# VictoriaMetrics/VictoriaLogs

Measured on NVIDIA H100. Metric: log rows scanned/sec (LogsQL phrase+regex), higher is better.
Workload: dtype u8

## Files before the change

### victorialogs_b200/csrc/vl_engine.cu

```cuda
#include <dlfcn.h>
#include <algorithm>
#include <atomic>
#include <chrono>
#include <thread>
#include <cstdio>
#include <cstdlib>
#include <cstring>
#include <functional>
#include <map>
#include <memory>
#include <mutex>
#include "vl_copier.h"
#include "vl_engine.h"
#include "vl_program.h"
#include "vl_part.h"
#include "vl_mathnum.cuh"

using namespace vl;

namespace vl {
static thread_local std::string g_thread_err;
void set_thread_error(const std::string& s) { g_thread_err = s; }
}

struct vlscan_program {
    Program p;
    struct Image { DevBuf leaves, prepass, regexes, blob, u64s, u32s; DevProgram view; };
    std::map<int, std::unique_ptr<Image>> images;
    std::mutex mu;
    const DevProgram& image(int device, cudaStream_t st) {
        std::lock_guard<std::mutex> g(mu);
        auto it = images.find(device);
        if (it != images.end()) return it->second->view;
        auto im = std::make_unique<Image>();
        auto up = [&](DevBuf& b, const void* src, size_t n) { b.ensure(std::max<size_t>(n, 16)); if (n) VL_CUDA(cudaMemcpyAsync(b.p, src, n, cudaMemcpyHostToDevice, st)); };
        up(im->leaves, p.leaves.data(), p.leaves.size() * sizeof(DevLeaf));
        up(im->prepass, p.prepass.data(), p.prepass.size() * sizeof(DevPrepass));
        up(im->regexes, p.regexes.data(), p.regexes.size() * sizeof(DevRegex));
        up(im->blob, p.blob.data(), p.blob.size());
        up(im->u64s, p.u64s.data(), p.u64s.size() * 8);
        up(im->u32s, p.u32s.data(), p.u32s.size() * 4);
        VL_CUDA(cudaStreamSynchronize(st));
        im->view = DevProgram{im->leaves.as<DevLeaf>(), im->prepass.as<DevPrepass>(), im->regexes.as<DevRegex>(), im->blob.as<uint8_t>(), im->u64s.as<uint64_t>(), im->u32s.as<uint32_t>()};
        auto& ref = *im;
        images[device] = std::move(im);
        return ref.view;
    }
    ~vlscan_program() { for (auto& kv : images) { cudaSetDevice(kv.first); kv.second->leaves.release(); kv.second->prepass.release(); kv.second->regexes.release(); kv.second->blob.release(); kv.second->u64s.release(); kv.second->u32s.release(); } }
};

struct vlscan_host_blocks {
    void* pinned = nullptr; size_t bytes = 0;
    std::vector<vlscan_block> blocks;
    std::vector<vlscan_column> cols;
    std::vector<std::string> fields;
    std::vector<std::vector<uint32_t>> dict_offsets;
    std::vector<std::unique_ptr<std::vector<uint8_t>>> owned;
    std::vector<uint64_t> source;
};
struct vlscan_part { vl::part::PartReader r; };

void* vlscan_ctx::ensure_pinned(size_t n) {
    if (n <= pinned_cap) return pinned;
    if (pinned) cudaFreeHost(pinned);
    pinned = nullptr; pinned_cap = 0;
    VL_CUDA(cudaMallocHost(&pinned, n));
    pinned_cap = n;
    return pinned;
}

namespace {

template <class F> int guarded(vlscan_ctx* ctx, F&& f) {
    try { f(); return 0; }
    catch (const CudaFail& e) { set_thread_error(e.msg); if (ctx) ctx->err = e.msg; return e.code > 0 ? e.code : 1; }
    catch (const BadInput& e) { set_thread_error(e.msg); if (ctx) ctx->err = e.msg; return -1; }
    catch (const ProgError& e) { set_thread_error(e.what()); if (ctx) ctx->err = e.what(); return -2; }
    catch (const std::exception& e) { set_thread_error(e.what()); if (ctx) ctx->err = e.what(); return -3; }
}

struct ZstdWriter {
    size_t (*compress)(void*, size_t, const void*, size_t, int) = nullptr;
    size_t (*bound)(size_t) = nullptr;
    unsigned (*is_error)(size_t) = nullptr;
    bool ok = false;
    ZstdWriter() {
        void* h = dlopen("libzstd.so.1", RTLD_NOW | RTLD_GLOBAL);
        if (!h) return;
        compress = (decltype(compress))dlsym(h, "ZSTD_compress");
        bound = (decltype(bound))dlsym(h, "ZSTD_compressBound");
        is_error = (decltype(is_error))dlsym(h, "ZSTD_isError");
        ok = compress && bound && is_error;
    }
};
ZstdWriter& zstd_writer() { static ZstdWriter z; return z; }

void launch_check(vlscan_ctx* ctx) { ctx->launches++; VL_CUDA(cudaGetLastError()); }
inline unsigned cdiv(uint64_t a, uint64_t b) { return (unsigned)((a + b - 1) / b); }

struct Carve {
    size_t off = 0;
    std::vector<std::function<void(uint8_t*)>> set;
    template <class T> Carve& take(T*& p, uint64_t n) { const size_t o = off; off += (n * sizeof(T) + 15) & ~(size_t)15; set.push_back([&p, o](uint8_t* base) { p = (T*)(base + o); }); return *this; }
    size_t place(DevBuf& buf) { buf.ensure(std::max<size_t>(off, 16)); for (auto& f : set) f(buf.as<uint8_t>()); return off; }
};

}

namespace vl {
void finish_batch_layout(vlscan_ctx* ctx, vlscan_batch* b, const std::vector<uint32_t>& rows) {
    b->nblocks = rows.size();
    b->h_rows = rows;
    b->h_word_off.assign(rows.size() + 1, 0);
    b->rows = 0;
    for (size_t i = 0; i < rows.size(); i++) { b->h_word_off[i + 1] = b->h_word_off[i] + (rows[i] + 63) / 64; b->rows += rows[i]; }
    b->nwords = b->h_word_off.back();
    std::vector<uint32_t> wb(b->nwords);
    std::vector<uint64_t> init(b->nwords);
    for (size_t i = 0; i < rows.size(); i++) {
        for (uint64_t w = b->h_word_off[i]; w < b->h_word_off[i + 1]; w++) { wb[w] = (uint32_t)i; init[w] = ~0ull; }
        uint32_t tail = rows[i] & 63;
        if (tail) init[b->h_word_off[i + 1] - 1] = (~0ull) >> (64 - tail);
    }
    b->blk_rows.ensure(std::max<size_t>(rows.size() * 4, 16));
    b->blk_word_off.ensure((rows.size() + 1) * 8);
    b->word_block.ensure(std::max<size_t>(b->nwords * 4, 16));
    b->init_bitmap.ensure(std::max<size_t>(b->nwords * 8, 16));
    if (!rows.empty()) VL_CUDA(cudaMemcpyAsync(b->blk_rows.p, rows.data(), rows.size() * 4, cudaMemcpyHostToDevice, ctx->stream));
    VL_CUDA(cudaMemcpyAsync(b->blk_word_off.p, b->h_word_off.data(), (rows.size() + 1) * 8, cudaMemcpyHostToDevice, ctx->stream));
    if (b->nwords) {
        VL_CUDA(cudaMemcpyAsync(b->word_block.p, wb.data(), b->nwords * 4, cudaMemcpyHostToDevice, ctx->stream));
        VL_CUDA(cudaMemcpyAsync(b->init_bitmap.p, init.data(), b->nwords * 8, cudaMemcpyHostToDevice, ctx->stream));
    }
    VL_CUDA(cudaStreamSynchronize(ctx->stream));
}
}

static uint64_t collect_values_blocks(const vlscan_block* blocks, uint64_t nblocks, std::vector<ZValuesBlock>& zv, const uint8_t* need = nullptr, uint32_t nfields = 0, std::vector<size_t>* at = nullptr) {
    uint64_t zc = 512;
    if (at) at->assign((size_t)nblocks * nfields, SIZE_MAX);
    for (uint64_t b = 0; b < nblocks; b++)
        for (uint32_t k = 0; k < blocks[b].ncols; k++) {
            const vlscan_column& c = blocks[b].cols[k];
            if (c.kind != VLSCAN_COL_VALUES || c.stage != VLSCAN_STAGE_ONDISK) continue;
            if (need && (c.field >= nfields || !need[b * nfields + c.field])) continue;
            if (at && c.field < nfields && (*at)[b * nfields + c.field] == SIZE_MAX) (*at)[b * nfields + c.field] = zv.size();
            zv.push_back({c.values, (size_t)c.values_len, zc});
            zc += c.values_len;
        }
    return zc;
}
static double now_s() { return std::chrono::duration<double>(std::chrono::steady_clock::now().time_since_epoch()).count(); }

namespace {
struct Upload {
    vlscan_ctx* ctx; vlscan_batch* out; const vlscan_block* blocks; uint64_t nblocks; uint32_t nfields; vlscan_stats* stats;
    const std::vector<char>* need_bloom;
    std::vector<DevColumn>& cols = out->h_cols;
    const bool dbg = getenv("VLSCAN_DEBUG_TIMING") != nullptr; const double t_start = now_s();
    Copier io{ctx};
    std::vector<uint32_t> rows = std::vector<uint32_t>(nblocks);
    std::vector<Piece> pieces;
    std::vector<std::unique_ptr<std::vector<uint8_t>>> owned;
    uint64_t cursor = 16;
    ZstdJob zjob;
    uint64_t regen_cursor = 0;
    struct Ondisk { uint64_t col; uint32_t lens_frame, data_frame; uint64_t lens_rel, data_rel; };
    std::vector<Ondisk> ondisk;
    std::vector<OndiskCol> ocols;
    struct TsFrame { uint64_t block; uint32_t frame; uint64_t rel; };
    std::vector<TsFrame> ts_frames;
    std::vector<DevTimestamps> tsv;
    std::vector<ZValuesBlock> zv; std::vector<ZValuesInfo> zinfo; std::vector<size_t> zv_of; std::vector<uint64_t> ts_zoff; size_t zbad = SIZE_MAX; std::string zmsg;
    uint64_t add_piece(const uint8_t* src, uint64_t len) { uint64_t off = arena_reserve(cursor, len); if (len) pieces.push_back({src, len, off}); return off; }
    template <class F> void walk(bool ts, F&& f) {
        for (uint64_t b = 0; b < nblocks; b++) {
            const vlscan_block& blk = blocks[b];
            if (blk.rows > (8u << 20)) throw BadInput("block rows exceed maxRowsPerBlock (8Mi)");
            rows[b] = (uint32_t)blk.rows;
            if (ts) timestamps(blk, b);
            for (uint32_t k = 0; k < blk.ncols; k++) {
                if (blk.cols[k].field >= nfields) throw BadInput("column refers to a field outside the batch field table");
                f(blk, blk.cols[k], (size_t)b * nfields + blk.cols[k].field);
            }
        }
    }
    void sources(const uint8_t* need, bool ts) {
        uint64_t zc = collect_values_blocks(blocks, nblocks, zv, need, nfields, &zv_of);
        for (const ZValuesBlock& v : zv) if (v.n) io.src.push_back({v.p, v.n, v.zoff});
        ts_zoff.resize(ts ? nblocks : 0);
        for (uint64_t b = 0; b < nblocks && ts; b++) {
            const vlscan_block& blk = blocks[b];
            if (blk.ts_marshal_type != MT_ZSTD_NEAREST_DELTA2 && blk.ts_marshal_type != MT_ZSTD_NEAREST_DELTA) continue;
            if (blk.timestamps_len > vl::part::kMaxTimestampsBlockSize) throw BadInput("timestamps block size cannot exceed 8 MiB");
            ts_zoff[b] = zc;
            if (blk.timestamps_len) io.src.push_back({blk.timestamps, blk.timestamps_len, zc});
            zc += blk.timestamps_len;
        }
        if (!io.src.empty()) { ctx->zsrc.ensure(zc + 512); io.send_sources(ctx->zsrc.as<uint8_t>()); }
        zinfo.resize(zv.size());
        const double t_w = now_s();
        if (!zv.empty()) zjob.add_values_blocks(zv.data(), zv.size(), host_threads(), zinfo.data(), &zbad, &zmsg);
        if (dbg) fprintf(stderr, "[vlscan upload] header walk of %zu values blocks on %d host threads: %.1f ms (after %.1f ms of collecting and enqueueing the copies)\n",
                         zv.size(), host_threads(), 1e3 * (now_s() - t_w), 1e3 * (t_w - t_start));
    }
    template <class F> void header(const vlscan_column& c, size_t i, F&& payload) {
        DevColumn& d = cols[i];
        if (d.kind != COL_MISSING) throw BadInput("duplicate column for one field in a block");
        if (c.kind == VLSCAN_COL_CONST) {
            d.kind = COL_CONST; d.meta_len = (uint32_t)c.const_len; d.meta_off = add_piece(c.const_value, c.const_len);
            return;
        }
        if (c.kind != VLSCAN_COL_VALUES) throw BadInput("unknown column kind");
        if (c.value_type < VT_STRING || c.value_type >= VT_MAX) throw BadInput("unknown valueType");
        d.kind = COL_VALUES; d.vt = c.value_type; d.min_value = c.min_value; d.max_value = c.max_value;
        payload();
        if (c.bloom_len % 8) throw BadInput("cannot unmarshal bloomFilter from src with size not multiple by 8");
        if (need_bloom && !(*need_bloom)[c.field]) { d.bloom_words = 0; d.bloom_off = add_piece(c.bloom, 0); }
        else { d.bloom_words = (uint32_t)(c.bloom_len / 8); d.bloom_off = add_piece(c.bloom, c.bloom_len); }
        if (c.value_type == VT_DICT) {
            if (c.dict_len > 8) throw BadInput("valuesDict may contain max 8 items");
            d.dict_len = c.dict_len;
            uint32_t total = c.dict_len ? c.dict_offsets[c.dict_len] : 0;
            d.meta_len = total;
            if (c.dict_len && c.dict_blob == (const uint8_t*)c.dict_offsets + 4 * (c.dict_len + 1)) {
                d.meta_off = add_piece((const uint8_t*)c.dict_offsets, 4 * (c.dict_len + 1) + total);
            } else {
                auto meta = std::make_unique<std::vector<uint8_t>>();
                meta->resize(4 * (c.dict_len + 1) + total);
                if (c.dict_len) memcpy(meta->data(), c.dict_offsets, 4 * (c.dict_len + 1)); else memset(meta->data(), 0, 4);
                if (total) memcpy(meta->data() + 4 * (c.dict_len + 1), c.dict_blob, total);
                d.meta_off = add_piece(meta->data(), meta->size());
                owned.push_back(std::move(meta));
            }
        }
    }
    void values(const vlscan_block& blk, const vlscan_column& c, size_t ci) {
        DevColumn& d = cols[ci];
        if (c.stage == VLSCAN_STAGE_ONDISK) {
            const size_t z = zv_of[ci];
            if (z >= zbad) throw BadInput(zmsg);
            const uint64_t lens_len = zinfo[z].lens_len, data_len = zinfo[z].data_len;
            if (data_len > 0xFFFFFFFFull) throw BadInput("values block too large");
            const uint64_t lr = arena_reserve(regen_cursor, lens_len + 15), dr = arena_reserve(regen_cursor, data_len);
            d.lens_off = lr + 16; d.data_off = dr; d.data_len = data_len;
            ondisk.push_back({ci, (uint32_t)(2 * z), (uint32_t)(2 * z + 1), lr + 15, dr});
            ocols.push_back({ci, lens_len, blk.rows});
        } else if (c.stage == VLSCAN_STAGE_DECODED) {
            const uint8_t* lens_items = c.lens_items; const uint64_t lens_len = c.lens_items_len, data_len = c.data_len;
            if (lens_len < 1) throw BadInput("cannot unmarshal uint64 block type from empty src");
            uint8_t lt = lens_items[0];
            if (lt > 7) throw BadInput("unexpected uint64 block type");
            uint64_t want = lt < 4 ? (blk.rows << lt) : (1ull << (lt - 4));
            if (lens_len - 1 != want) throw BadInput("unexpected block length for uint items");
            d.lens_type = lt;
            if (lt >= 4) { uint64_t v = 0; for (uint64_t i = 0; i < want; i++) v = (v << 8) | lens_items[1 + i]; if (v > 0xFFFFFFFFull) throw BadInput("row length does not fit 32 bits"); d.lens_const = (uint32_t)v; }
            if (data_len > 0xFFFFFFFFull) throw BadInput("values block too large");
            d.lens_off = add_piece(lens_items + 1, lens_len - 1);
            d.data_off = add_piece(c.data, data_len); d.data_len = data_len;
            d.data_const = (blk.rows >= 2 && lt >= 4 && data_len == d.lens_const) ? 1 : 0;
        } else throw BadInput("unknown values stage");
    }
    void timestamps(const vlscan_block& blk, uint64_t b) {
        if (!blk.ts_marshal_type) return;
        if (blk.ts_marshal_type > MT_NEAREST_DELTA) throw BadInput("unknown MarshalType of a timestamps block");
        if (blk.timestamps_len > vl::part::kMaxTimestampsBlockSize) throw BadInput("timestamps block size cannot exceed 8 MiB");
        if (tsv.empty()) { tsv.resize(nblocks); memset(tsv.data(), 0, nblocks * sizeof(DevTimestamps)); }
        DevTimestamps& t = tsv[b];
        t.first = blk.min_timestamp; t.max = blk.max_timestamp;
        if (blk.ts_marshal_type == MT_ZSTD_NEAREST_DELTA2 || blk.ts_marshal_type == MT_ZSTD_NEAREST_DELTA) {
            uint64_t regen = 0; uint32_t id = 0;
            zjob.add_frame(blk.timestamps, blk.timestamps_len, ts_zoff[b], &regen, &id);
            if (regen > 10ull * blk.rows + 16) throw BadInput("cannot unmarshal timestamps: the decompressed block is larger than its varints can be");
            t.mt = blk.ts_marshal_type == MT_ZSTD_NEAREST_DELTA2 ? MT_NEAREST_DELTA2 : MT_NEAREST_DELTA;
            t.len = (uint32_t)regen;
            ts_frames.push_back({b, id, arena_reserve(regen_cursor, regen)});
        } else {
            t.mt = (uint8_t)blk.ts_marshal_type; t.len = (uint32_t)blk.timestamps_len;
            t.off = add_piece(blk.timestamps, blk.timestamps_len);
        }
    }

    uint64_t commit(DevBuf& region, const std::vector<uint64_t>* patch, bool layout) {
        const uint64_t regen_base = (cursor + kArenaAlign - 1) / kArenaAlign * kArenaAlign;
        for (const Ondisk& o : ondisk) {
            DevColumn& d = cols[o.col];
            d.lens_off += regen_base; d.data_off += regen_base;
            zjob.set_dst(o.lens_frame, regen_base + o.lens_rel); zjob.set_dst(o.data_frame, regen_base + o.data_rel);
        }
        for (const TsFrame& tf : ts_frames) { tsv[tf.block].off = regen_base + tf.rel; zjob.set_dst(tf.frame, regen_base + tf.rel); }
        const bool have_z = !ondisk.empty() || !ts_frames.empty();
        if (have_z) cursor = regen_base + regen_cursor;
        const uint64_t bytes = cursor + kArenaPad;
        const double t_desc = now_s();
        region.ensure(bytes);
        const double t_alloc = now_s();
        uint8_t* cols_base = region.as<uint8_t>();
        std::vector<ColPatch> patches;
        if (patch) {
            const uint64_t delta = (uint64_t)(uintptr_t)region.p - (uint64_t)(uintptr_t)out->arena.p;
            cols_base = out->arena.as<uint8_t>();
            patches.resize(patch->size());
            for (size_t i = 0; i < patch->size(); i++) {
                DevColumn& d = cols[(*patch)[i]];
                d.lens_off += delta; d.data_off += delta;
                patches[i].col = (*patch)[i]; patches[i].c = d;
            }
        }
        cudaStream_t cs = ctx->copy_stream;
        cudaEvent_t ev_cleared = io.events.make(), ev_copied = io.events.make();
        VL_CUDA(cudaMemsetAsync(region.p, 0, bytes, ctx->stream));
        VL_CUDA(cudaEventRecord(ev_cleared, ctx->stream));
        VL_CUDA(cudaStreamWaitEvent(cs, ev_cleared, 0));
        const double t_h2d = dbg ? now_s() : 0;
        double t_zrun = 0;
        if (have_z) {
            zjob.set_group_hook([&](uint64_t src_end) { io.wait_sources(ctx->stream, src_end); });
            zjob.run(ctx, ctx->zsrc.as<uint8_t>(), region.as<uint8_t>());
            io.ship_sources(UINT64_MAX);
            if (dbg) t_zrun = now_s();
        }
        io.copy(pieces, region.as<uint8_t>());
        DevBuf& table = patch ? ctx->patch : out->cols;
        const void* entries = patch ? (const void*)patches.data() : (const void*)cols.data();
        const size_t table_bytes = patch ? patches.size() * sizeof(ColPatch) : cols.size() * sizeof(DevColumn);
        table.ensure(std::max<size_t>(table_bytes, 16));
        if (table_bytes) VL_CUDA(cudaMemcpyAsync(table.p, entries, table_bytes, cudaMemcpyHostToDevice, cs));
        io.h2d += table_bytes;
        if (!patch) out->has_ts = !tsv.empty();
        if (!tsv.empty()) {
            out->ts.ensure(nblocks * sizeof(DevTimestamps));
            VL_CUDA(cudaMemcpyAsync(out->ts.p, tsv.data(), nblocks * sizeof(DevTimestamps), cudaMemcpyHostToDevice, cs));
            io.h2d += nblocks * sizeof(DevTimestamps);
        }
        VL_CUDA(cudaEventRecord(ev_copied, cs));
        if (!patches.empty()) {
            VL_CUDA(cudaStreamWaitEvent(ctx->stream, ev_copied, 0));
            k_patch_cols<<<cdiv(patches.size(), 128), 128, 0, ctx->stream>>>(out->cols.as<DevColumn>(), ctx->patch.as<ColPatch>(), (uint32_t)patches.size());
            launch_check(ctx);
        }
        const double t_enq = dbg ? now_s() : 0;
        if (have_z) {
            VL_CUDA(cudaStreamWaitEvent(ctx->stream, ev_copied, 0));
            ctx->zcols.ensure(16 + ocols.size() * sizeof(OndiskCol));
            VL_CUDA(cudaMemsetAsync(ctx->zcols.p, 0, 16, ctx->stream));
            VL_CUDA(cudaMemcpyAsync(ctx->zcols.as<uint8_t>() + 16, ocols.data(), ocols.size() * sizeof(OndiskCol), cudaMemcpyHostToDevice, ctx->stream));
            if (!ocols.empty()) {
                k_finish_ondisk_cols<<<cdiv(ocols.size(), 128), 128, 0, ctx->stream>>>(cols_base, out->cols.as<DevColumn>(), (const OndiskCol*)(ctx->zcols.as<uint8_t>() + 16),
                                                                                         (uint32_t)ocols.size(), ctx->zcols.as<unsigned long long>());
                launch_check(ctx);
            }
            io.h2d += ocols.size() * sizeof(OndiskCol);
            zjob.check(ctx);
            unsigned long long cst[2] = {0, 0};
            VL_CUDA(cudaMemcpy(cst, ctx->zcols.p, 16, cudaMemcpyDeviceToHost));
            static const char* what[] = {"", "cannot unmarshal uint64 block type from empty src", "unexpected uint64 block type", "unexpected block length for uint items", "row length does not fit 32 bits"};
            if (cst[0]) throw BadInput(what[std::min<unsigned long long>(cst[0], 4)]);
        }
        VL_CUDA(cudaStreamWaitEvent(ctx->stream, ev_copied, 0));
        double t_copy = 0;
        if (dbg) { VL_CUDA(cudaStreamSynchronize(ctx->stream)); t_copy = now_s(); }
        if (nfields) out->note_columns(cols);
        if (layout) finish_batch_layout(ctx, out, rows);
        else VL_CUDA(cudaStreamSynchronize(ctx->stream));
        if (dbg) fprintf(stderr, "[vlscan upload] blocks=%llu arena=%.1f MB h2d=%.1f MB pieces=%zu+%zu pinned=%d: describe %.1f ms, alloc %.1f ms, copy %.1f ms (%.1f GB/s), "
                                 "zstd %llu frames / %llu blocks / %llu sequences: enqueue %.1f ms, decode %.1f ms; layout %.1f ms\n", (unsigned long long)nblocks,
                         bytes / 1e6, io.h2d / 1e6, pieces.size(), io.src.size(), (int)io.all_pinned, 1e3 * (t_desc - t_start), 1e3 * (t_alloc - t_desc), 1e3 * (t_enq - (t_zrun > 0 ? t_zrun : t_h2d)), io.h2d / 1e9 / std::max(t_copy - t_start, 1e-9),
                         (unsigned long long)zjob.frames(), (unsigned long long)zjob.compressed_blocks(), (unsigned long long)zjob.sequences(), 1e3 * (t_zrun > 0 ? t_zrun - t_h2d : 0), 1e3 * (t_copy - t_enq), 1e3 * (now_s() - t_copy));
        if (layout) io.h2d += out->nwords * 12 + nblocks * 12;
        if (stats) stats->h2d_bytes += io.h2d;
        return bytes;
    }
};
}

enum UploadMode { UP_FULL = 0, UP_HEADERS = 1, UP_VALUES = 2, UP_LATE = 3 };
static void do_upload(vlscan_ctx* ctx, const char* const* field_names, const size_t* field_name_lens, uint32_t nfields, const vlscan_block* blocks,
                      uint64_t nblocks, vlscan_batch* out, vlscan_stats* stats, const std::vector<char>* need_bloom = nullptr, UploadMode mode = UP_FULL,
                      const uint8_t* need = nullptr, uint64_t* zframes = nullptr) {
    VL_CUDA(cudaSetDevice(ctx->device));
    if (nblocks > 0xFFFFFFF0ull) throw BadInput("too many blocks in one batch");
    out->device = ctx->device; out->nfields = nfields;
    Upload u{ctx, out, blocks, nblocks, nfields, stats, need_bloom};
    if (mode == UP_FULL || mode == UP_HEADERS) {
        for (uint32_t f = 0; f < nfields; f++) out->field_names.emplace_back(field_names[f], field_name_lens[f]);
        u.cols.assign((size_t)nblocks * std::max<uint32_t>(nfields, 1), DevColumn{});
        memset(u.cols.data(), 0, u.cols.size() * sizeof(DevColumn));
        out->late_used = 0; out->split_hdr = mode == UP_HEADERS;
    } else if (u.cols.size() != (size_t)nblocks * std::max<uint32_t>(nfields, 1) || !need) throw BadInput("internal: values phase of a bloom-first upload without its header phase");
    try {
        switch (mode) {
        case UP_FULL:
            u.sources(nullptr, true);
            u.walk(true, [&](const vlscan_block& blk, const vlscan_column& c, size_t i) { u.header(c, i, [&] { u.values(blk, c, i); }); });
            out->arena_bytes = u.commit(out->arena, nullptr, true);
            out->harena_bytes = 0;
            std::vector<DevColumn>().swap(out->h_cols);
            break;
        case UP_HEADERS:
            u.walk(false, [&](const vlscan_block&, const vlscan_column& c, size_t i) {
                u.header(c, i, [&] {
                    if (c.stage != VLSCAN_STAGE_ONDISK && c.stage != VLSCAN_STAGE_DECODED) throw BadInput("unknown values stage");
                    u.cols[i].values_state = VALUES_DEFERRED;
                });
            });
            out->harena_bytes = u.commit(out->harena, nullptr, true);
            break;
        case UP_VALUES:
            u.sources(need, true);
            u.walk(true, [&](const vlscan_block& blk, const vlscan_column& c, size_t i) {
                if (c.kind != VLSCAN_COL_VALUES) return;
                u.cols[i].values_state = need[i] ? VALUES_STAGED : VALUES_ABSENT;
                if (need[i]) u.values(blk, c, i);
            });
            out->arena_bytes = u.commit(out->arena, nullptr, false);
            break;
        case UP_LATE: {
            std::vector<uint64_t> staged;
            u.sources(need, false);
            u.walk(false, [&](const vlscan_block& blk, const vlscan_column& c, size_t i) {
                if (c.kind != VLSCAN_COL_VALUES || !need[i]) return;
                if (u.cols[i].values_state == VALUES_STAGED) throw BadInput("duplicate column for one field in a block");
                u.cols[i].values_state = VALUES_STAGED;
                u.values(blk, c, i);
                staged.push_back(i);
            });
            if (out->late_used == out->late.size()) out->late.emplace_back();
            u.commit(out->late[out->late_used], &staged, false);
            out->late_used++;
            *zframes += u.zjob.frames();
            break;
        }
        }
    } catch (...) {
        cudaStreamSynchronize(ctx->copy_stream); cudaStreamSynchronize(ctx->stream);
        throw;
    }
}

namespace {
struct ScanRun {
    vlscan_ctx* ctx; const vlscan_program* prog; const vlscan_batch* batch;
    DevProgram P; BatchView B; std::vector<int> field_slot;
    unsigned long long* stats;
    size_t regs_used = 0;

    uint64_t* new_reg() {
        if (regs_used == ctx->regs.size()) ctx->regs.emplace_back();
        DevBuf& r = ctx->regs[regs_used++];
        r.ensure(std::max<size_t>(B.nwords * 8, 16));
        return r.as<uint64_t>();
    }
    void free_reg() { regs_used--; }
    void copy_reg(uint64_t* dst, const uint64_t* src) { if (B.nwords) VL_CUDA(cudaMemcpyAsync(dst, src, B.nwords * 8, cudaMemcpyDeviceToDevice, ctx->stream)); }
    void andnot(uint64_t* a, const uint64_t* b) { if (!B.nwords) return; k_andnot<<<cdiv(B.nwords, 256), 256, 0, ctx->stream>>>(a, b, B.nwords); launch_check(ctx); }
    void prepass(const PNode& nd, uint64_t* reg) {
        if (nd.prepass_count == 0) return;
        std::vector<int> slots(nd.prepass_count);
        for (int e = 0; e < nd.prepass_count; e++) slots[e] = field_slot[prog->p.prepass[nd.prepass_begin + e].field];
        size_t off = slots_cursor; slots_cursor += slots.size();
        ctx->slots.ensure(std::max<size_t>(slots_total * 4, 16));
        VL_CUDA(cudaMemcpyAsync(ctx->slots.as<int>() + off, slots.data(), slots.size() * 4, cudaMemcpyHostToDevice, ctx->stream));
        k_prepass<<<cdiv((uint64_t)B.nblocks * 32, 128), 128, 0, ctx->stream>>>(P, B, (uint32_t)nd.prepass_begin, (uint32_t)nd.prepass_count, ctx->slots.as<int>() + off,
                                                                             nd.kind == F_OR, reg, stats);
        launch_check(ctx);
    }
    size_t slots_cursor = 0, slots_total = 0;

    void leaf(int leaf_idx, uint64_t* reg) {
        const DevLeaf& L = prog->p.leaves[leaf_idx];
        if (L.kind == F_NOOP) return;
        int slot = L.field >= 0 ? field_slot[L.field] : -1;
        uint8_t* action = ctx->action.as<uint8_t>(); uint64_t* payload = ctx->payload.as<uint64_t>(); uint64_t* leaf_bm = ctx->leaf_bm.as<uint64_t>();
        uint32_t* lens_blocks = ctx->lens_blocks.as<uint32_t>(); uint32_t* row_blocks = ctx->row_blocks.as<uint32_t>(); uint32_t* wc = ctx->work_count.as<uint32_t>();
        ScanTile* tiles = ctx->tiles.as<ScanTile>();
        VL_CUDA(cudaMemsetAsync(wc, 0, WC_COUNT * 4, ctx->stream));
        if (L.kind == F_EQ_FIELD || L.kind == F_LE_FIELD) {
            const int slot_b = field_slot[L.field2];
            uint32_t* lens_b = ctx->lens_blocks2.as<uint32_t>();
            k_plan_pair<<<cdiv((uint64_t)B.nblocks * 32, 256), 256, 0, ctx->stream>>>(P, B, (uint32_t)leaf_idx, slot, slot_b, reg, action, payload, lens_blocks, lens_b, row_blocks, wc, stats);
            launch_check(ctx);
            if (B.nwords) {
                const int persistent = ctx->sm_count * 8;
                const uint32_t *ro_a = nullptr, *ro_b = nullptr;
                for (int side = 0; side < 2; side++) {
                    const int sl = side ? slot_b : slot;
                    if (sl < 0) continue;
                    uint8_t* ready = ctx->ready[sl].as<uint8_t>();
                    if (!ctx->ready_cleared[sl]) { VL_CUDA(cudaMemsetAsync(ready, 0, B.nblocks, ctx->stream)); ctx->ready_cleared[sl] = 1; }
                    k_lens_offsets<<<persistent, 256, 0, ctx->stream>>>(B, sl, side ? lens_b : lens_blocks, wc, ctx->row_off8[sl].as<uint32_t>(), ready, stats, side ? WC_LENS2 : WC_LENS); launch_check(ctx);
                    (side ? ro_b : ro_a) = ctx->row_off8[sl].as<uint32_t>();
                }
                k_row_pair<<<persistent, 256, 0, ctx->stream>>>(P, B, (uint32_t)leaf_idx, slot, slot_b, row_blocks, wc, payload, reg, ro_a, ro_b, leaf_bm, stats); launch_check(ctx);
                k_apply_leaf<<<cdiv(B.nwords, 256), 256, 0, ctx->stream>>>(B, action, leaf_bm, reg); launch_check(ctx);
            }
            return;
        }
        k_plan_leaf<<<cdiv(B.nblocks, VL_PLAN_WARPS), VL_PLAN_WARPS * 32, 0, ctx->stream>>>(P, B, (uint32_t)leaf_idx, slot, reg, action, payload, lens_blocks, row_blocks, tiles, wc, stats);
        launch_check(ctx);
        if (slot >= 0 && B.nwords) {
            uint32_t* ro = ctx->row_off8[slot].as<uint32_t>(); uint8_t* ready = ctx->ready[slot].as<uint8_t>();
            if (!ctx->ready_cleared[slot]) { VL_CUDA(cudaMemsetAsync(ready, 0, B.nblocks, ctx->stream)); ctx->ready_cleared[slot] = 1; }
            const int persistent = ctx->sm_count * 8;
            const uint32_t vts = batch->slot_vt_mask.empty() ? ~0u : batch->slot_vt_mask[slot];
            const bool has_string = vts >> VT_STRING & 1, has_dict = vts >> VT_DICT & 1;
            const bool has_numeric = (vts & ~((1u << VT_STRING) | (1u << VT_DICT))) != 0;
            const bool may_scan = L.str_strategy == STR_SCAN && has_string;
            const bool may_row = (has_string && L.str_strategy != STR_ALL) || has_numeric;
            if (may_scan || may_row) { k_lens_offsets<<<persistent, 256, 0, ctx->stream>>>(B, slot, lens_blocks, wc, ro, ready, stats); launch_check(ctx); }
            if (may_scan) {
                VL_CUDA(cudaMemsetAsync(leaf_bm, 0, B.nwords * 8, ctx->stream));
                ScanParams sp; memset(&sp, 0, sizeof sp);
                sp.mode = L.scan_mode; sp.needle_off = L.scan_needle_off; sp.needle_len = L.scan_needle_len; sp.starts_tok = L.starts_tok; sp.ends_tok = L.ends_tok; sp.regex = L.regex;
                const bool masked = fill_scan_patterns(prog->p.blob.data() + L.scan_needle_off, L.scan_needle_len, sp.pat, sp.msk, sp.delta, sp.nd16);
                if (L.scan_mode == SCAN_CONTAINS || L.scan_mode >= SCAN_RX_DOTPLUS) { sp.starts_tok = sp.ends_tok = 0; }
                auto& evp = next_scan_events();
                VL_CUDA(cudaEventRecord(evp.first, ctx->stream));
                if (masked) k_substr_scan<true><<<ctx->sm_count * ctx->scan_occ[1], VL_SCAN_THREADS, 0, ctx->stream>>>(P, B, slot, sp, tiles, wc, ro, leaf_bm);
                else k_substr_scan<false><<<ctx->sm_count * ctx->scan_occ[0], VL_SCAN_THREADS, 0, ctx->stream>>>(P, B, slot, sp, tiles, wc, ro, leaf_bm);
                launch_check(ctx);
                VL_CUDA(cudaEventRecord(evp.second, ctx->stream));
            }
            if (may_row) { k_row_match<<<ctx->sm_count * ctx->row_occ, 256, 0, ctx->stream>>>(P, B, (uint32_t)leaf_idx, slot, row_blocks, wc, action, payload, reg, ro, leaf_bm); launch_check(ctx); }
            if (has_dict || has_numeric) { k_word_match<<<cdiv(B.nwords, 128), 128, 0, ctx->stream>>>(P, B, (uint32_t)leaf_idx, slot, action, payload, reg, leaf_bm, stats); launch_check(ctx); }
        }
        if (L.kind == F_TIME && B.nwords) {
            ctx->ts_vals.ensure(B.nwords * 64 * 8);
            k_time_match<<<ctx->sm_count * 4, 256, 0, ctx->stream>>>(B, (long long)L.aux0, (long long)L.aux1, row_blocks, wc, ctx->ts_vals.as<unsigned long long>(), leaf_bm, stats);
            launch_check(ctx);
        }
        if (B.nwords) { k_apply_leaf<<<cdiv(B.nwords, 256), 256, 0, ctx->stream>>>(B, action, leaf_bm, reg); launch_check(ctx); }
    }
    std::pair<cudaEvent_t, cudaEvent_t>& next_scan_events() {
        if (ctx->scan_events_used == ctx->scan_events.size()) { cudaEvent_t a, b; VL_CUDA(cudaEventCreate(&a)); VL_CUDA(cudaEventCreate(&b)); ctx->scan_events.emplace_back(a, b); }
        return ctx->scan_events[ctx->scan_events_used++];
    }
    void probe_leaf(int leaf_idx, const uint64_t* reg, uint8_t* need) {
        const DevLeaf& L = prog->p.leaves[leaf_idx];
        if (L.kind == F_NOOP || L.kind == F_TIME) return;
        const int slot = L.field >= 0 ? field_slot[L.field] : -1;
        if (L.kind == F_EQ_FIELD || L.kind == F_LE_FIELD) {
            k_plan_pair<<<cdiv((uint64_t)B.nblocks * 32, 256), 256, 0, ctx->stream>>>(P, B, (uint32_t)leaf_idx, slot, field_slot[L.field2], reg, nullptr, nullptr, nullptr, nullptr, nullptr, nullptr, stats, need);
        } else {
            if (slot < 0) return;
            k_plan_leaf<<<cdiv(B.nblocks, VL_PLAN_WARPS), VL_PLAN_WARPS * 32, 0, ctx->stream>>>(P, B, (uint32_t)leaf_idx, slot, reg, nullptr, nullptr, nullptr, nullptr, nullptr, nullptr, stats, need);
        }
        launch_check(ctx);
    }
    void probe_node(int id, uint64_t* reg, uint8_t* need) {
        const PNode& nd = prog->p.nodes[id];
        switch (nd.kind) {
        case F_NOOP: break;
        case F_AND: case F_OR: {
            uint64_t* r = reg;
            if (nd.prepass_count) { r = new_reg(); copy_reg(r, reg); prepass(nd, r); }
            for (int k : nd.kids) probe_node(k, r, need);
            if (nd.prepass_count) free_reg();
            break;
        }
        case F_NOT: probe_node(nd.kids[0], reg, need); break;
        default: probe_leaf(nd.leaf, reg, need);
        }
    }
    void node(int id, uint64_t* reg) {
        const PNode& nd = prog->p.nodes[id];
        switch (nd.kind) {
        case F_NOOP: break;
        case F_AND: prepass(nd, reg); for (int k : nd.kids) node(k, reg); break;
        case F_OR: {
            prepass(nd, reg);
            uint64_t* res = new_reg(); uint64_t* tmp = new_reg();
            copy_reg(res, reg);
            for (int k : nd.kids) { copy_reg(tmp, res); node(k, tmp); andnot(res, tmp); }
            andnot(reg, res);
            free_reg(); free_reg();
            break;
        }
        case F_NOT: { uint64_t* tmp = new_reg(); copy_reg(tmp, reg); node(nd.kids[0], tmp); andnot(reg, tmp); free_reg(); break; }
        default: leaf(nd.leaf, reg);
        }
    }
};
}

static void read_stats(vlscan_ctx* ctx, vlscan_stats* st, bool check_error) {
    unsigned long long h[ST_COUNT];
    VL_CUDA(cudaMemcpyAsync(h, ctx->stats.p, sizeof h, cudaMemcpyDeviceToHost, ctx->stream));
    VL_CUDA(cudaStreamSynchronize(ctx->stream));
    if (check_error && h[ST_ERROR]) {
        static const char* const msg[] = {"", "cannot unmarshal strings: row lengths do not add up to the data length", "too big index for dict value",
                                          "unexpected length for binary representation of a number", "", "", "the filter needs the timestamps of a block that was handed over without them", "cannot unmarshal timestamps",
                                          "internal: a filter reached the values of a column that the bloom-first probe pass had left on the host"};
        throw BadInput(msg[std::min<unsigned long long>(h[ST_ERROR], 8)]);
    }
    if (!st) return;
    st->values_bytes += h[ST_VALUES_BYTES]; st->bloom_probe_bytes += h[ST_BLOOM_BYTES]; st->columns_read += h[ST_COLUMNS_READ];
    st->bitmap_bytes += h[ST_BITMAP_BYTES]; st->rows_matched += h[ST_ROWS_MATCHED]; st->blocks_matched += h[ST_BLOCKS_MATCHED];
    st->scan_kernel_bytes += h[ST_SCAN_BYTES];
    float ms = 0;
    VL_CUDA(cudaEventElapsedTime(&ms, ctx->ev_begin, ctx->ev_end)); st->gpu_ms += ms;
    for (size_t i = 0; i < ctx->scan_events_used; i++) { VL_CUDA(cudaEventElapsedTime(&ms, ctx->scan_events[i].first, ctx->scan_events[i].second)); st->scan_kernel_ms += ms; }
}

static void do_scan(vlscan_ctx* ctx, const vlscan_program* prog, const vlscan_batch* batch, vlscan_stats* stats) {
    VL_CUDA(cudaSetDevice(ctx->device));
    if (batch->device != ctx->device) throw BadInput("batch lives on another device than the ctx");
    ScanRun run{ctx, prog, batch};
    run.P = const_cast<vlscan_program*>(prog)->image(ctx->device, ctx->stream);
    run.B = batch->view();
    const Program& pr = prog->p;
    run.field_slot.assign(pr.fields.size(), -1);
    for (size_t f = 0; f < pr.fields.size(); f++) for (uint32_t s = 0; s < batch->nfields; s++) if (batch->field_names[s] == pr.fields[f]) run.field_slot[f] = (int)s;
    for (auto& nd : pr.nodes) run.slots_total += nd.prepass_count;
    uint64_t nb = std::max<uint64_t>(batch->nblocks, 1), nw = std::max<uint64_t>(batch->nwords, 1);
    ctx->action.ensure(nb); ctx->payload.ensure(nb * 8); ctx->leaf_bm.ensure(nw * 8);
    ctx->lens_blocks.ensure(nb * 4); ctx->lens_blocks2.ensure(nb * 4); ctx->row_blocks.ensure(nb * 4); ctx->work_count.ensure(WC_COUNT * 4);
    {
        uint64_t max_tiles = batch->arena_bytes / VL_TILE_BYTES + nb + 16;
        ctx->tiles.ensure(max_tiles * sizeof(ScanTile));
    }
    ctx->stats.ensure(ST_COUNT * 8); ctx->totals.ensure(32); ctx->counts.ensure(nb * 4);
    if (ctx->row_off8.size() < batch->nfields) { ctx->row_off8.resize(batch->nfields); ctx->ready.resize(batch->nfields); }
    ctx->ready_cleared.assign(batch->nfields, 0);
    for (uint32_t s = 0; s < batch->nfields; s++) { ctx->row_off8[s].ensure(nw * 32); ctx->ready[s].ensure(nb); }
    uint64_t launches0 = ctx->launches;
    ctx->scan_events_used = 0;
    run.stats = ctx->stats.as<unsigned long long>();
    VL_CUDA(cudaEventRecord(ctx->ev_begin, ctx->stream));
    VL_CUDA(cudaMemsetAsync(ctx->stats.p, 0, ST_COUNT * 8, ctx->stream));
    VL_CUDA(cudaMemsetAsync(ctx->totals.p, 0, 32, ctx->stream));
    uint64_t* reg = run.new_reg();
    run.copy_reg(reg, batch->init_bitmap.as<uint64_t>());
    if (batch->nblocks) {
        run.node(pr.root, reg);
        k_finalize<<<cdiv(batch->nblocks, 8), 256, 0, ctx->stream>>>(run.B, reg, ctx->counts.as<uint32_t>(), run.stats, ctx->totals.as<unsigned long long>());
        launch_check(ctx);
    }
    VL_CUDA(cudaEventRecord(ctx->ev_end, ctx->stream));
    ctx->last_batch = batch; ctx->has_result = true; ctx->kept = false; ctx->last_launches = ctx->launches - launches0;
    ctx->last_nblocks = batch->nblocks; ctx->last_nwords = batch->nwords; ctx->last_rows = batch->rows;
    if (stats) {
        read_stats(ctx, stats, true);
        stats->blocks += batch->nblocks; stats->rows += batch->rows; stats->gpu_launches += ctx->launches - launches0;
    }
}

static void do_probe(vlscan_ctx* ctx, const vlscan_program* prog, const vlscan_batch* batch, std::vector<uint8_t>& need) {
    VL_CUDA(cudaSetDevice(ctx->device));
    ScanRun run{ctx, prog, batch};
    run.P = const_cast<vlscan_program*>(prog)->image(ctx->device, ctx->stream);
    run.B = batch->view();
    const Program& pr = prog->p;
    run.field_slot.assign(pr.fields.size(), -1);
    for (size_t f = 0; f < pr.fields.size(); f++) for (uint32_t s = 0; s < batch->nfields; s++) if (batch->field_names[s] == pr.fields[f]) run.field_slot[f] = (int)s;
    for (auto& nd : pr.nodes) run.slots_total += nd.prepass_count;
    const size_t cells = (size_t)batch->nblocks * batch->nfields;
    need.assign(cells, 0);
    if (!cells || !batch->nwords) return;
    ctx->need.ensure(std::max<size_t>(cells, 16)); ctx->stats.ensure(ST_COUNT * 8);
    VL_CUDA(cudaMemsetAsync(ctx->need.p, 0, cells, ctx->stream));
    VL_CUDA(cudaMemsetAsync(ctx->stats.p, 0, ST_COUNT * 8, ctx->stream));
    run.stats = ctx->stats.as<unsigned long long>();
    uint64_t* reg = run.new_reg();
    run.copy_reg(reg, batch->init_bitmap.as<uint64_t>());
    run.probe_node(pr.root, reg, ctx->need.as<uint8_t>());
    VL_CUDA(cudaMemcpyAsync(need.data(), ctx->need.p, cells, cudaMemcpyDeviceToHost, ctx->stream));
    VL_CUDA(cudaStreamSynchronize(ctx->stream));
}

extern "C" {

int vlscan_device_count(void) {
    int n = 0;
    if (cudaGetDeviceCount(&n) != cudaSuccess) { cudaGetLastError(); return 0; }
    return n;
}

vlscan_ctx* vlscan_ctx_create(int device) {
    vlscan_ctx* ctx = new vlscan_ctx();
    int rc = guarded(nullptr, [&] {
        int n = vlscan_device_count();
        if (n <= 0) throw CudaFail("no CUDA device is available: libvlscan has no CPU fallback", 100);
        ctx->device = ((device % n) + n) % n;
        VL_CUDA(cudaSetDevice(ctx->device));
        VL_CUDA(cudaStreamCreateWithFlags(&ctx->stream, cudaStreamNonBlocking));
        VL_CUDA(cudaStreamCreateWithFlags(&ctx->copy_stream, cudaStreamNonBlocking));
        VL_CUDA(cudaEventCreate(&ctx->ev_begin)); VL_CUDA(cudaEventCreate(&ctx->ev_end));
        cudaDeviceProp prop; VL_CUDA(cudaGetDeviceProperties(&prop, ctx->device)); ctx->sm_count = prop.multiProcessorCount;
        VL_CUDA(cudaOccupancyMaxActiveBlocksPerMultiprocessor(&ctx->scan_occ[0], k_substr_scan<false>, VL_SCAN_THREADS, 0));
        VL_CUDA(cudaOccupancyMaxActiveBlocksPerMultiprocessor(&ctx->scan_occ[1], k_substr_scan<true>, VL_SCAN_THREADS, 0));
        for (int& o : ctx->scan_occ) o = std::max(o, 1);
        VL_CUDA(cudaOccupancyMaxActiveBlocksPerMultiprocessor(&ctx->row_occ, k_row_match, 256, 0));
        ctx->row_occ = std::max(ctx->row_occ, 1);
    });
    if (rc) { delete ctx; return nullptr; }
    return ctx;
}
void vlscan_ctx_free(vlscan_ctx* ctx) {
    if (!ctx) return;
    cudaSetDevice(ctx->device);
    if (ctx->copy_stream) cudaStreamSynchronize(ctx->copy_stream);
    if (ctx->stream) cudaStreamSynchronize(ctx->stream);
    for (DevBuf* b : {&ctx->action, &ctx->payload, &ctx->leaf_bm, &ctx->lens_blocks, &ctx->row_blocks, &ctx->work_count, &ctx->stats, &ctx->totals, &ctx->counts, &ctx->slots, &ctx->hit_offs, &ctx->hits, &ctx->tiles, &ctx->lens_blocks2}) b->release();
    for (auto& r : ctx->regs) r.release();
    for (auto& r : ctx->row_off8) r.release();
    for (auto& r : ctx->ready) r.release();
    ctx->zsrc.release(); ctx->zcols.release(); ctx->ztest.release(); ctx->ts_vals.release();
    for (DevBuf* b : {&ctx->hit_block, &ctx->glens, &ctx->goffs, &ctx->gtiles, &ctx->gout, &ctx->gstat, &ctx->hblk, &ctx->htab, &ctx->hgrp, &ctx->lcand, &ctx->ftab, &ctx->patch, &ctx->unstaged}) b->release();
    for (DevBuf& b : ctx->ftxt) b.release();
    zstd_dev_free(ctx->zdev);
    delete ctx->pool;
    if (ctx->pinned) cudaFreeHost(ctx->pinned);
    delete ctx->recycle;
    for (auto& e : ctx->scan_events) { cudaEventDestroy(e.first); cudaEventDestroy(e.second); }
    if (ctx->ev_begin) cudaEventDestroy(ctx->ev_begin);
    if (ctx->ev_end) cudaEventDestroy(ctx->ev_end);
    if (ctx->copy_stream) cudaStreamDestroy(ctx->copy_stream);
    if (ctx->stream) cudaStreamDestroy(ctx->stream);
    delete ctx;
}
const char* vlscan_last_error(const vlscan_ctx* ctx) { return ctx ? ctx->err.c_str() : g_thread_err.c_str(); }
void* vlscan_ctx_stream(const vlscan_ctx* ctx) { return (void*)ctx->stream; }
int vlscan_ctx_sync(vlscan_ctx* ctx) { return guarded(ctx, [&] { VL_CUDA(cudaSetDevice(ctx->device)); VL_CUDA(cudaStreamSynchronize(ctx->stream)); }); }

int vlscan_program_create(const void* tree, size_t tree_len, vlscan_program** out) {
    *out = nullptr;
    auto* pg = new vlscan_program();
    int rc = guarded(nullptr, [&] { ProgramBuilder(tree, tree_len, pg->p).build(); });
    if (rc) { delete pg; return rc; }
    *out = pg;
    return 0;
}
void vlscan_program_free(vlscan_program* prog) { delete prog; }
uint32_t vlscan_program_nfields(const vlscan_program* prog) { return (uint32_t)prog->p.fields.size(); }
const char* vlscan_program_field(const vlscan_program* prog, uint32_t i, size_t* len) { if (i >= prog->p.fields.size()) { *len = 0; return nullptr; } *len = prog->p.fields[i].size(); return prog->p.fields[i].data(); }
int64_t vlscan_program_leaf_tokens(const vlscan_program* prog, uint32_t leaf, char* buf, size_t cap) {
    if (leaf >= prog->p.leaf_tokens.size()) return -1;
    std::string s; for (size_t i = 0; i < prog->p.leaf_tokens[leaf].size(); i++) { if (i) s.push_back('\n'); s += prog->p.leaf_tokens[leaf][i]; }
    if (s.size() > cap) return -1;
    memcpy(buf, s.data(), s.size());
    return (int64_t)s.size();
}

int vlscan_eval_predicate(int kind, const void* value, size_t value_len, const void* arg1, size_t arg1_len, const void* arg2, size_t arg2_len, uint64_t aux0, uint64_t aux1) {
    if (value_len > 0xFFFFFFFFull || arg1_len > 0xFFFFFFFFull || arg2_len > 0xFFFFFFFFull) return -1;
    const uint8_t* v = (const uint8_t*)value; const uint32_t vn = (uint32_t)value_len;
    const uint8_t* a = (const uint8_t*)arg1; const uint32_t an = (uint32_t)arg1_len;
    switch (kind) {
    case F_REGEXP: {
        try { return vl::compile_regex(std::string((const char*)a, an)).match(v, vn) ? 1 : 0; } catch (const vl::RxError& e) { vl::set_thread_error(e.what()); return -2; }
    }
    case 14: return vl::any_case_match(v, vn, a, an, false) ? 1 : 0;
    case 15: return vl::any_case_match(v, vn, a, an, true) ? 1 : 0;
    case 16: return vl::match_sequence(v, vn, vl::PhraseList{a, an}) ? 1 : 0;
    case 17: return vl::match_all_phrases(v, vn, vl::PhraseList{a, an}) ? 1 : 0;
    case 18: return vl::match_any_phrase(v, vn, vl::PhraseList{a, an}) ? 1 : 0;
    }
    if (kind < F_EXACT_PREFIX || kind > F_IPV4_RANGE) return -1;
    return vl::range_predicate(kind, (const uint8_t*)value, (uint32_t)value_len, (const uint8_t*)arg1, (uint32_t)arg1_len, (const uint8_t*)arg2, (uint32_t)arg2_len, aux0, aux1) ? 1 : 0;
}

int64_t vlscan_program_prepass_tokens(const vlscan_program* prog, char* buf, size_t cap) {
    const Program& P = prog->p;
    std::string s;
    for (const PNode& nd : P.nodes) {
        if (nd.kind != F_AND && nd.kind != F_OR) continue;
        s += nd.kind == F_AND ? "A" : "O";
        for (int k = 0; k < nd.prepass_count; k++) {
            const DevPrepass& pp = P.prepass[(size_t)nd.prepass_begin + k];
            s += "\t" + P.fields[pp.field];
            const uint32_t* offs = (const uint32_t*)(P.blob.data() + pp.tok_offs_off);
            for (uint32_t t = 0; t < pp.ntokens; t++) { s += "\x1f"; s.append((const char*)P.blob.data() + pp.tok_blob_off + offs[t], offs[t + 1] - offs[t]); }
        }
        s += "\n";
    }
    if (s.size() > cap) return -1;
    memcpy(buf, s.data(), s.size());
    return (int64_t)s.size();
}

int64_t vlscan_program_in_hashes(const vlscan_program* prog, uint32_t leaf, uint64_t* out, size_t cap) {
    const Program& P = prog->p;
    if (leaf >= P.leaves.size() || P.leaves[leaf].kind != F_IN) return -1;
    const DevLeaf& L = P.leaves[leaf];
    std::vector<uint64_t> v;
    v.push_back(L.nhashes); v.insert(v.end(), P.u64s.begin() + L.hashes_off, P.u64s.begin() + L.hashes_off + L.nhashes);
    if (L.in_skip_sets) v.push_back(UINT64_MAX);
    else {
        v.push_back(L.in_nsets);
        for (uint32_t k = 0; k < L.in_nsets; k++) {
            const uint32_t off = P.u32s[L.in_sets_off + 2 * k], n = P.u32s[L.in_sets_off + 2 * k + 1];
            v.push_back(n); v.insert(v.end(), P.u64s.begin() + off, P.u64s.begin() + off + n);
        }
    }
    if (v.size() > cap) return -1;
    memcpy(out, v.data(), v.size() * 8);
    return (int64_t)v.size();
}

int64_t vlscan_program_in_typed(const vlscan_program* prog, uint32_t leaf, int value_type, uint64_t* out, size_t cap) {
    const Program& P = prog->p;
    if (leaf >= P.leaves.size() || P.leaves[leaf].kind != F_IN || value_type < VT_UINT8 || value_type >= VT_MAX) return -1;
    const DevLeaf& L = P.leaves[leaf];
    const uint32_t n = L.in_typed_cnt[value_type];
    if (n > cap) return -1;
    if (n) memcpy(out, P.u64s.data() + L.in_typed_off[value_type], (size_t)n * 8);
    return (int64_t)n;
}

int vlscan_parse_typed(int value_type, const void* s, size_t len, uint64_t* out) {
    const std::string v((const char*)s, len);
    uint64_t u = 0; int64_t i = 0; double f = 0; uint32_t ip = 0;
    switch (value_type) {
    case VT_UINT8: case VT_UINT16: case VT_UINT32: case VT_UINT64: if (!vl::parse_u64(v, &u)) return 0; *out = u; return 1;
    case VT_INT64: if (!vl::parse_i64(v, &i)) return 0; *out = (uint64_t)i; return 1;
    case VT_FLOAT64: if (!vl::parse_f64_exact(v, &f)) return 0; memcpy(out, &f, 8); return 1;
    case VT_IPV4: if (!vl::parse_ipv4(v, &ip)) return 0; *out = ip; return 1;
    case VT_ISO8601: if (!vl::parse_iso8601(v, &i)) return 0; *out = (uint64_t)i; return 1;
    }
    return -1;
}

double vlscan_parse_math_number(const void* s, size_t len) {
    if (len > 0xFFFFFFFFull) return NAN;
    return vl::mn::parse_math_number((const uint8_t*)s, (uint32_t)len);
}

int vlscan_format_float64(uint64_t ieee_bits, char* buf, size_t cap) {
    uint8_t tmp[VL_FMT_F64_MAX];
    int n = vl::fmt_f64(tmp, ieee_bits);
    if ((size_t)n > cap) return -1;
    memcpy(buf, tmp, (size_t)n);
    return n;
}

int vlscan_batch_upload(vlscan_ctx* ctx, const char* const* field_names, const size_t* field_name_lens, uint32_t nfields, const vlscan_block* blocks,
                        uint64_t nblocks, vlscan_batch** out, vlscan_stats* stats) {
    *out = nullptr;
    auto* b = new vlscan_batch();
    int rc = guarded(ctx, [&] { do_upload(ctx, field_names, field_name_lens, nfields, blocks, nblocks, b, stats); });
    if (rc) { delete b; return rc; }
    *out = b;
    return 0;
}
void vlscan_batch_free(vlscan_batch* batch) { delete batch; }
uint64_t vlscan_batch_nblocks(const vlscan_batch* b) { return b->nblocks; }
uint64_t vlscan_batch_rows(const vlscan_batch* b) { return b->rows; }
uint64_t vlscan_batch_words(const vlscan_batch* b) { return b->nwords; }
uint64_t vlscan_batch_device_bytes(const vlscan_batch* b) { return b->device_bytes(); }

int vlscan_batch_download(vlscan_ctx* ctx, const vlscan_batch* batch, vlscan_host_blocks** out) {
    *out = nullptr;
    auto* hb = new vlscan_host_blocks();
    int rc = guarded(ctx, [&] {
        VL_CUDA(cudaSetDevice(ctx->device));
        if (batch->split_hdr) throw BadInput("a batch staged bloom-first cannot be downloaded");
        hb->bytes = batch->arena_bytes;
        VL_CUDA(cudaMallocHost(&hb->pinned, std::max<size_t>(hb->bytes, 16)));
        std::vector<DevColumn> cols((size_t)batch->nblocks * batch->nfields);
        VL_CUDA(cudaMemcpyAsync(hb->pinned, batch->arena.p, hb->bytes, cudaMemcpyDeviceToHost, ctx->stream));
        if (!cols.empty()) VL_CUDA(cudaMemcpyAsync(cols.data(), batch->cols.p, cols.size() * sizeof(DevColumn), cudaMemcpyDeviceToHost, ctx->stream));
        VL_CUDA(cudaStreamSynchronize(ctx->stream));
        hb->fields = batch->field_names;
        const uint8_t* base = (const uint8_t*)hb->pinned;
        hb->blocks.resize(batch->nblocks);
        hb->cols.reserve(cols.size());
        std::vector<size_t> first(batch->nblocks + 1, 0);
        for (uint64_t b = 0; b < batch->nblocks; b++) {
            first[b] = hb->cols.size();
            for (uint32_t f = 0; f < batch->nfields; f++) {
                const DevColumn& d = cols[(size_t)b * batch->nfields + f];
                if (d.kind == COL_MISSING) continue;
                vlscan_column c; memset(&c, 0, sizeof c);
                c.field = f;
                if (d.kind == COL_CONST) { c.kind = VLSCAN_COL_CONST; c.const_value = base + d.meta_off; c.const_len = d.meta_len; hb->cols.push_back(c); continue; }
                c.kind = VLSCAN_COL_VALUES; c.value_type = d.vt; c.stage = VLSCAN_STAGE_DECODED; c.dict_len = d.dict_len; c.min_value = d.min_value; c.max_value = d.max_value;
                uint64_t items = d.lens_type < 4 ? ((uint64_t)batch->h_rows[b] << d.lens_type) : (1ull << (d.lens_type - 4));
                uint8_t* tb = (uint8_t*)hb->pinned + d.lens_off - 1;
                *tb = d.lens_type;
                c.lens_items = tb; c.lens_items_len = items + 1;
                c.data = base + d.data_off; c.data_len = d.data_len;
                c.bloom = base + d.bloom_off; c.bloom_len = (uint64_t)d.bloom_words * 8;
                if (d.vt == VT_DICT) { c.dict_offsets = (const uint32_t*)(base + d.meta_off); c.dict_blob = base + d.meta_off + 4 * (d.dict_len + 1); }
                hb->cols.push_back(c);
            }
        }
        first[batch->nblocks] = hb->cols.size();
        for (uint64_t b = 0; b < batch->nblocks; b++) { hb->blocks[b].rows = batch->h_rows[b]; hb->blocks[b].ncols = (uint32_t)(first[b + 1] - first[b]); hb->blocks[b].cols = hb->cols.data() + first[b]; }
        if (batch->has_ts && batch->nblocks) {
            std::vector<DevTimestamps> ts(batch->nblocks);
            VL_CUDA(cudaMemcpy(ts.data(), batch->ts.p, ts.size() * sizeof(DevTimestamps), cudaMemcpyDeviceToHost));
            for (uint64_t b = 0; b < batch->nblocks; b++) {
                if (!ts[b].mt) continue;
                vlscan_block& blk = hb->blocks[b];
                blk.ts_marshal_type = ts[b].mt; blk.timestamps = base + ts[b].off; blk.timestamps_len = ts[b].len;
                blk.min_timestamp = ts[b].first; blk.max_timestamp = ts[b].max;
            }
        }
    });
    if (rc) { if (hb->pinned) cudaFreeHost(hb->pinned); delete hb; return rc; }
    *out = hb;
    return 0;
}
static void marshal_bytes_block(std::vector<uint8_t>& dst, const uint8_t* src, size_t n) {
    if (n < 128) { dst.push_back(0); dst.push_back((uint8_t)n); dst.insert(dst.end(), src, src + n); return; }
    ZstdWriter& z = zstd_writer();
    if (!z.ok) throw BadInput("libzstd.so.1 is not available for compressing values blocks");
    int level = n <= 512 ? 1 : n <= 4096 ? 2 : 3;
    size_t cap = z.bound(n), old = dst.size();
    dst.push_back(1);
    dst.resize(old + 1 + 10 + cap);
    size_t got = z.compress(dst.data() + old + 11, cap, src, n, level);
    if (z.is_error(got)) throw BadInput("ZSTD_compress failed");
    uint8_t vu[10]; int k = 0; uint64_t v = got; while (v >= 0x80) { vu[k++] = (uint8_t)(v | 0x80); v >>= 7; } vu[k++] = (uint8_t)v;
    memcpy(dst.data() + old + 1, vu, k);
    memmove(dst.data() + old + 1 + k, dst.data() + old + 11, got);
    dst.resize(old + 1 + k + got);
}

int vlscan_host_blocks_compress(const vlscan_host_blocks* in, int threads, vlscan_host_blocks** out) {
    *out = nullptr;
    auto* hb = new vlscan_host_blocks();
    int rc = guarded(nullptr, [&] {
        const size_t ncols = in->cols.size();
        std::vector<std::vector<uint8_t>> packed(ncols);
        std::atomic<size_t> next{0}; std::atomic<bool> failed{false}; std::string fail_msg; std::mutex mu;
        auto work = [&] {
            for (;;) {
                size_t i0 = next.fetch_add(64); if (i0 >= ncols || failed) return;
                for (size_t i = i0; i < std::min(ncols, i0 + 64); i++) {
                    const vlscan_column& c = in->cols[i];
                    if (c.kind != VLSCAN_COL_VALUES) continue;
                    try {
                        if (c.stage == VLSCAN_STAGE_ONDISK) packed[i].assign(c.values, c.values + c.values_len);
                        else { marshal_bytes_block(packed[i], c.lens_items, c.lens_items_len); marshal_bytes_block(packed[i], c.data, c.data_len); }
                    } catch (const BadInput& e) { std::lock_guard<std::mutex> g(mu); fail_msg = e.msg; failed = true; return; }
                }
            }
        };
        int nt = threads > 0 ? threads : (int)std::max(1u, std::thread::hardware_concurrency());
        std::vector<std::thread> pool; for (int t = 1; t < nt; t++) pool.emplace_back(work);
        work(); for (auto& t : pool) t.join();
        if (failed) throw BadInput(fail_msg);
        uint64_t cursor = 16, vbytes = 0;
        std::vector<uint64_t> off_a(ncols, 0), off_b(ncols, 0), off_v(ncols, 0);
        for (size_t i = 0; i < ncols; i++) {
            const vlscan_column& c = in->cols[i];
            if (c.kind == VLSCAN_COL_CONST) { off_a[i] = arena_reserve(cursor, c.const_len); continue; }
            off_a[i] = arena_reserve(cursor, c.bloom_len);
            if (c.value_type == VT_DICT) off_b[i] = arena_reserve(cursor, 4 * (c.dict_len + 1) + (c.dict_len ? c.dict_offsets[c.dict_len] : 0));
            off_v[i] = vbytes; vbytes += packed[i].size();
        }
        const uint64_t vbase = (cursor + kArenaPad + 63) / 64 * 64;
        hb->bytes = vbase + vbytes + 64;
        VL_CUDA(cudaMallocHost(&hb->pinned, hb->bytes));
        uint8_t* base = (uint8_t*)hb->pinned;
        memset(base, 0, vbase);
        hb->fields = in->fields; hb->cols = in->cols; hb->blocks = in->blocks;
        for (size_t i = 0; i < ncols; i++) {
            vlscan_column& c = hb->cols[i];
            if (c.kind == VLSCAN_COL_CONST) { if (c.const_len) memcpy(base + off_a[i], c.const_value, c.const_len); c.const_value = base + off_a[i]; continue; }
            if (c.bloom_len) memcpy(base + off_a[i], c.bloom, c.bloom_len);
            c.bloom = base + off_a[i];
            if (c.value_type == VT_DICT) {
                uint32_t total = c.dict_len ? c.dict_offsets[c.dict_len] : 0;
                uint8_t* m = base + off_b[i];
                if (c.dict_len) memcpy(m, c.dict_offsets, 4 * (c.dict_len + 1)); else memset(m, 0, 4);
                if (total) memcpy(m + 4 * (c.dict_len + 1), c.dict_blob, total);
                c.dict_offsets = (const uint32_t*)m; c.dict_blob = m + 4 * (c.dict_len + 1);
            }
            memcpy(base + vbase + off_v[i], packed[i].data(), packed[i].size());
            c.stage = VLSCAN_STAGE_ONDISK; c.values = base + vbase + off_v[i]; c.values_len = packed[i].size();
            c.lens_items = nullptr; c.lens_items_len = 0; c.data = nullptr; c.data_len = 0;
            std::vector<uint8_t>().swap(packed[i]);
        }
        size_t k = 0;
        for (size_t b = 0; b < hb->blocks.size(); b++) { hb->blocks[b].cols = hb->cols.data() + k; k += hb->blocks[b].ncols; }
    });
    if (rc) { if (hb->pinned) cudaFreeHost(hb->pinned); delete hb; return rc; }
    *out = hb;
    return 0;
}

int vlscan_zstd_inspect(const void* bytes_block, size_t len, uint64_t out[5]) {
    return guarded(nullptr, [&] {
        ZstdJob job;
        uint64_t regen = 0; uint32_t id = 0;
        size_t used = job.add_bytes_block((const uint8_t*)bytes_block, len, 512, &regen, &id);
        out[0] = used; out[1] = regen; out[2] = job.blocks(); out[3] = job.compressed_blocks(); out[4] = job.sequences();
    });
}

int vlscan_zstd_walk_digest(const vlscan_block* blocks, uint64_t nblocks, int threads, uint64_t out[12]) {
    return guarded(nullptr, [&] {
        std::vector<ZValuesBlock> zv;
        collect_values_blocks(blocks, nblocks, zv);
        std::vector<ZValuesInfo> info(zv.size());
        ZstdJob job; size_t bad = SIZE_MAX; std::string msg;
        const double t0 = now_s();
        if (!zv.empty()) job.add_values_blocks(zv.data(), zv.size(), threads, info.data(), &bad, &msg);
        const double t1 = now_s();
        if (bad != SIZE_MAX) throw BadInput("values block " + std::to_string(bad) + ": " + msg);
        job.prepare();
        const double t2 = now_s();
        job.digest(out);
        uint64_t h = 5; for (const ZValuesInfo& x : info) { h = (h ^ x.lens_len) * 0x9E3779B97F4A7C15ull; h = (h ^ x.data_len) * 0x9E3779B97F4A7C15ull; h ^= h >> 29; }
        out[0] ^= h;
        out[4] = job.frames(); out[5] = job.blocks(); out[6] = job.groups(); out[7] = job.compressed_blocks(); out[8] = job.sequences();
        out[9] = (uint64_t)((t1 - t0) * 1e9); out[10] = (uint64_t)((t2 - t1) * 1e9); out[11] = 0;
    });
}

static void zstd_decompress_frames(vlscan_ctx* ctx, uint32_t nframes, const void* const* frames, const size_t* frame_lens, void* dst, const uint64_t* dst_offsets) {
    {
        VL_CUDA(cudaSetDevice(ctx->device));
        ZstdJob job;
        std::vector<uint8_t> packed(512, 0);
// ... 857 lines not shown
```

### victorialogs_b200/csrc/vl_engine.h

```cpp
#pragma once
#include <cuda_runtime.h>
#include <stdint.h>
#include <algorithm>
#include <string>
#include <vector>
#include "../../include/vlscan.h"
#include "vl_kernels.cuh"
#include "vl_zstd.h"
#include "vl_zstd_walk.h"
#include "vl_hostpool.h"

namespace vl {

void set_thread_error(const std::string& s);
#define VL_CUDA(call)                                                                                                   \
    do {                                                                                                                \
        cudaError_t e__ = (call);                                                                                       \
        if (e__ != cudaSuccess) throw CudaFail(std::string(#call) + ": " + cudaGetErrorString(e__), (int)e__);        \
    } while (0)
struct CudaFail { std::string msg; int code; CudaFail(std::string m, int c) : msg(std::move(m)), code(c) {} };

struct DevBuf {
    void* p = nullptr; size_t cap = 0;
    void ensure(size_t n) {
        if (n <= cap) return;
        if (p) VL_CUDA(cudaFree(p));
        p = nullptr; cap = 0;
        size_t want = n + std::min<size_t>(n / 8, (size_t)256 << 20) + 256;
        VL_CUDA(cudaMalloc(&p, want)); cap = want;
    }
    void release() { if (p) cudaFree(p); p = nullptr; cap = 0; }
    template <class T> T* as() const { return (T*)p; }
};



static const size_t kArenaAlign = 16;
static const size_t kArenaPad = 32;
inline uint64_t arena_reserve(uint64_t& cursor, uint64_t len) {
    uint64_t off = (cursor + kArenaAlign - 1) / kArenaAlign * kArenaAlign;
    cursor = off + len + kArenaPad;
    return off;
}

}

struct vlscan_batch {
    int device = 0;
    uint32_t nfields = 0;
    std::vector<std::string> field_names;
    uint64_t nblocks = 0, nwords = 0, rows = 0;
    uint64_t arena_bytes = 0, harena_bytes = 0;
    vl::DevBuf arena, cols, blk_rows, blk_word_off, word_block, init_bitmap, ts;
    vl::DevBuf harena;
    bool split_hdr = false;
    std::vector<vl::DevColumn> h_cols;
    bool has_ts = false;
    std::vector<uint32_t> h_rows;
    std::vector<uint64_t> h_word_off;
    std::vector<uint32_t> slot_vt_mask;
    std::vector<vl::DevBuf> late;
    size_t late_used = 0;
    struct CellSig { uint64_t len0 = 0, len1 = 0; uint32_t stage = 0; };
    std::vector<CellSig> h_sig;
    std::vector<uint32_t> h_ncols;
    void note_columns(const std::vector<vl::DevColumn>& cols) {
        slot_vt_mask.assign(nfields, 0);
        for (size_t i = 0; i < cols.size(); i++) if (cols[i].kind == vl::COL_VALUES) slot_vt_mask[i % nfields] |= 1u << cols[i].vt;
    }
    vl::BatchView view() const {
        vl::BatchView v;
        v.arena = arena.as<uint8_t>(); v.hdr = split_hdr ? harena.as<uint8_t>() : arena.as<uint8_t>(); v.cols = cols.as<vl::DevColumn>(); v.blk_rows = blk_rows.as<uint32_t>();
        v.blk_word_off = blk_word_off.as<uint64_t>(); v.word_block = word_block.as<uint32_t>();
        v.ts = has_ts ? ts.as<vl::DevTimestamps>() : nullptr;
        v.nblocks = (uint32_t)nblocks; v.nfields = nfields; v.nwords = nwords;
        return v;
    }
    uint64_t device_bytes() const {
        uint64_t n = arena.cap + harena.cap + cols.cap + blk_rows.cap + blk_word_off.cap + word_block.cap + init_bitmap.cap + ts.cap;
        for (const vl::DevBuf& r : late) n += r.cap;
        return n;
    }
    ~vlscan_batch() {
        cudaSetDevice(device); arena.release(); harena.release(); cols.release(); blk_rows.release(); blk_word_off.release(); word_block.release(); init_bitmap.release(); ts.release();
        for (vl::DevBuf& r : late) r.release();
    }
};

struct vlscan_ctx {
    int device = 0;
    cudaStream_t stream = nullptr;
    cudaStream_t copy_stream = nullptr;
    std::string err;
    uint64_t launches = 0;
    vl::DevBuf action, payload, leaf_bm, lens_blocks, work_count, stats, totals, counts, slots, tiles;
    vl::DevBuf lens_blocks2;
    vl::DevBuf row_blocks;
    vl::DevBuf hit_offs, hits;
    std::vector<vl::DevBuf> regs;
    std::vector<vl::DevBuf> row_off8;
    std::vector<vl::DevBuf> ready;
    std::vector<char> ready_cleared;
    vl::DevBuf hit_block, glens, goffs, gtiles, gout, gstat;
    vl::DevBuf ts_vals;
    vl::DevBuf hblk, htab, hgrp;
    vl::DevBuf lcand;
    vl::DevBuf ftab;
    std::vector<vl::DevBuf> ftxt;
    vl::DevBuf need;
    const void* bf_prog = nullptr; int bf_skip = 0;
    vl::DevBuf zsrc, zcols, ztest;
    vl::ZstdDev* zdev = nullptr;
    void* pinned = nullptr; size_t pinned_cap = 0;
    vl::HostPool* pool = nullptr;
    cudaEvent_t ev_begin = nullptr, ev_end = nullptr;
    std::vector<std::pair<cudaEvent_t, cudaEvent_t>> scan_events; size_t scan_events_used = 0;
    const vlscan_batch* last_batch = nullptr;
    uint64_t last_nblocks = 0, last_nwords = 0, last_rows = 0;
    vlscan_batch* recycle = nullptr;
    bool kept = false;
    vl::DevBuf patch, unstaged;
    bool has_result = false;
    uint64_t last_launches = 0;
    int sm_count = 132;
    int scan_occ[2] = {1, 1};
    int row_occ = 1;
    void* ensure_pinned(size_t n);
};

namespace vl {
void finish_batch_layout(vlscan_ctx* ctx, vlscan_batch* b, const std::vector<uint32_t>& rows);
}
```

### victorialogs_b200/csrc/vl_kernels.cuh

```cuda
#pragma once
#include <cuda_runtime.h>
#include <stdint.h>
#include "vl_hd.cuh"
#include "vl_anycase.cuh"
#include "vl_mathnum.cuh"
#include "vl_types.h"

namespace vl {

struct DevProgram {
    const DevLeaf* leaves; const DevPrepass* prepass; const DevRegex* regexes;
    const uint8_t* blob; const uint64_t* u64s; const uint32_t* u32s;
};

enum { ST_VALUES_BYTES = 0, ST_BLOOM_BYTES, ST_COLUMNS_READ, ST_BITMAP_BYTES, ST_ROWS_MATCHED, ST_BLOCKS_MATCHED, ST_ERROR, ST_SCAN_BYTES, ST_COUNT };
enum { ERR_NONE = 0, ERR_LENS_MISMATCH = 1, ERR_DICT_INDEX = 2, ERR_BAD_WIDTH = 3, ERR_NO_TIMESTAMPS = 6, ERR_BAD_TIMESTAMPS = 7, ERR_VALUES_ABSENT = 8,
       ERR_TS_HEADER = 9 };

struct BatchView {
    const uint8_t* arena;
    const uint8_t* hdr;
    const DevColumn* cols;
    const uint32_t* blk_rows;
    const uint64_t* blk_word_off;
    const uint32_t* word_block;
    const DevTimestamps* ts;
    uint32_t nblocks, nfields;
    uint64_t nwords;
};

static __device__ __forceinline__ uint32_t lane_id() { return threadIdx.x & 31; }
#define VL_SHORT_ROW_BYTES 48u
static __device__ __forceinline__ uint32_t width_of_vt(uint32_t vt) {
    switch (vt) { case VT_DICT: case VT_UINT8: return 1; case VT_UINT16: return 2; case VT_UINT32: case VT_IPV4: return 4; case VT_UINT64: case VT_FLOAT64: case VT_ISO8601: case VT_INT64: return 8; }
    return 0;
}
static __device__ __forceinline__ uint64_t lens_stored_bytes(const DevColumn& c, uint32_t rows) {
    return 1 + (c.lens_type < 4 ? ((uint64_t)rows << c.lens_type) : (1ull << (c.lens_type - 4)));
}
static __device__ __forceinline__ bool cell_needs_offsets(const DevColumn& c) { return c.kind == COL_VALUES && c.lens_type < 4 && !c.data_const; }
static __device__ __forceinline__ uint32_t row_len(const DevColumn& c, const uint8_t* lens, uint32_t r) {
    switch (c.lens_type) {
    case 0: return lens[r];
    case 1: return ld_be16(lens + 2 * (uint64_t)r);
    case 2: return ld_be32(lens + 4 * (uint64_t)r);
    case 3: return (uint32_t)ld_be64(lens + 8 * (uint64_t)r);
    default: return c.lens_const;
    }
}
static __device__ __forceinline__ uint64_t load_fixed_be(const uint8_t* p, uint32_t w) {
    switch (w) { case 1: return p[0]; case 2: return ld_be16(p); case 4: return ld_be32(p); default: return ld_be64(p); }
}
static __device__ __forceinline__ int64_t unzigzag64(uint64_t u) { return (int64_t)(u >> 1) ^ -(int64_t)(u & 1); }

static __device__ __forceinline__ uint32_t rx_class(const DevRegex& R, const uint8_t* blob, int32_t r) {
    if (r < 128) return blob[R.ascii_off + r];
    const int32_t* b = (const int32_t*)(blob + R.bounds_off);
    int lo = 0, hi = (int)R.nclasses - 1;
    while (lo < hi) { int mid = (lo + hi + 1) >> 1; if (b[mid] <= r) lo = mid; else hi = mid - 1; }
    return (uint32_t)lo;
}
static __device__ bool dfa_run(const DevRegex& R, const uint8_t* blob, const uint8_t* s, uint32_t n) {
    const uint16_t* T = (const uint16_t*)(blob + R.trans_off);
    uint32_t st = 0;
    for (uint32_t i = 0; i < n;) {
        int w; int32_t r = s[i];
        if (r < 0x80) w = 1; else r = decode_rune(s + i, n - i, &w);
        i += w;
        uint32_t e = T[st * R.nclasses + rx_class(R, blob, r)];
        if (e & 0x8000) return true;
        st = e & 0x7FFF;
        if (st == 0x7FFF) return false;
    }
    return blob[R.accept_off + st] != 0;
}
static __device__ bool regex_match(const DevRegex& R, const uint8_t* blob, const uint8_t* s, uint32_t n) {
    const uint8_t* pre = blob + R.prefix_off; uint32_t pl = R.prefix_len;
    const uint8_t* sub = blob + R.sub_off; uint32_t sl = R.sub_len;
    if (R.only_prefix) return pl == 0 || find_bytes(s, n, pre, pl, 0) >= 0;
    if (pl == 0) {
        if (R.dot_star) return true;
        if (R.dot_plus) return n > 0;
        if (R.sub_kind == 1) return find_bytes(s, n, sub, sl, 0) >= 0;
        if (R.sub_kind == 2) { int k = find_bytes(s, n, sub, sl, 0); return k > 0 && (uint32_t)k + sl < n; }
        return dfa_run(R, blob, s, n);
    }
    int k = find_bytes(s, n, pre, pl, 0);
    if (k < 0) return false;
    uint32_t rem = (uint32_t)k + pl;
    if (R.dot_star) return true;
    if (R.dot_plus) return n > rem;
    if (R.sub_kind == 1) return find_bytes(s + rem, n - rem, sub, sl, 0) >= 0;
    if (R.sub_kind == 2) { int m = find_bytes(s + rem, n - rem, sub, sl, 0); return m > 0 && (uint32_t)m + sl < n - rem; }
    if (R.tail_len) return find_bytes(s + rem, n - rem, blob + R.tail_off, R.tail_len, 0) >= 0;
    for (;;) {
        if (dfa_run(R, blob, s + rem, n - rem)) return true;
        k = find_bytes(s, n, pre, pl, (uint32_t)k + 1);
        if (k < 0) return false;
        rem = (uint32_t)k + pl;
    }
}

static __device__ bool in_contains_string(const DevLeaf& L, const uint8_t* blob, const uint8_t* s, uint32_t n) {
    const uint32_t* offs = (const uint32_t*)(blob + L.in_offs_off);
    const uint8_t* base = blob + L.in_blob_off;
    for (uint32_t i = 0; i < L.in_count; i++) { uint32_t a = offs[i], b = offs[i + 1]; if (b - a == n && bytes_equal(base + a, n, s, n)) return true; }
    return false;
}
static __device__ __forceinline__ bool in_contains_typed(const DevLeaf& L, const uint64_t* u64s, uint32_t vt, uint64_t v) {
    const uint64_t* set = u64s + L.in_typed_off[vt];
    int lo = 0, hi = (int)L.in_typed_cnt[vt] - 1;
    while (lo <= hi) { int mid = (lo + hi) >> 1; uint64_t x = set[mid]; if (x == v) return true; if (x < v) lo = mid + 1; else hi = mid - 1; }
    return false;
}

static __device__ bool leaf_match_string(const DevProgram& P, const DevLeaf& L, const uint8_t* s, uint32_t n) {
    const uint8_t* nd = P.blob + L.needle_off;
    switch (L.kind) {
    case F_PHRASE: return match_phrase(s, n, nd, L.needle_len);
    case F_PREFIX: return match_prefix(s, n, nd, L.needle_len);
    case F_EXACT: return bytes_equal(s, n, nd, L.needle_len);
    case F_IN: return in_contains_string(L, P.blob, s, n);
    case F_REGEXP: return regex_match(P.regexes[L.regex], P.blob, s, n);
    case F_EXACT_PREFIX: case F_LEN_RANGE: case F_STRING_RANGE: case F_IPV4_RANGE:
        return range_predicate(L.kind, s, n, nd, L.needle_len, P.blob + L.needle2_off, L.needle2_len, L.aux0, L.aux1);
    case F_VALUE_TYPE: return false;
    case F_ANY_CASE_PHRASE: return any_case_match(s, n, nd, L.needle_len, false);
    case F_ANY_CASE_PREFIX: return any_case_match(s, n, nd, L.needle_len, true);
    case F_SEQUENCE: return match_sequence(s, n, PhraseList{P.blob + L.list_off, L.list_len});
    case F_CONTAINS_ALL: return match_all_phrases(s, n, PhraseList{P.blob + L.list_off, L.list_len});
    case F_CONTAINS_ANY: return match_any_phrase(s, n, PhraseList{P.blob + L.list_off, L.list_len});
    case F_RANGE: {
        const double f = mn::parse_math_number(s, n);
        return f >= __longlong_as_double((long long)L.rng_fmin) && f <= __longlong_as_double((long long)L.rng_fmax);
    }
    }
    return true;
}
static __device__ bool leaf_match_typed_text(const DevProgram& P, const DevLeaf& L, uint32_t vt, const uint8_t* s, uint32_t n) {
    if (L.kind == F_ANY_CASE_PHRASE || L.kind == F_ANY_CASE_PREFIX) {
        const uint8_t* nd = P.blob + (vt == VT_ISO8601 ? L.needle2_off : L.needle_off); const uint32_t nl = vt == VT_ISO8601 ? L.needle2_len : L.needle_len;
        return L.kind == F_ANY_CASE_PHRASE ? match_phrase(s, n, nd, nl) : match_prefix(s, n, nd, nl);
    }
    return leaf_match_string(P, L, s, n);
}

static __device__ int encoded_to_string(uint32_t vt, uint64_t raw, uint8_t* buf) {
    switch (vt) {
    case VT_UINT8: case VT_UINT16: case VT_UINT32: case VT_UINT64: return fmt_u64(buf, raw);
    case VT_INT64: return fmt_i64(buf, unzigzag64(raw));
    case VT_IPV4: return fmt_ipv4(buf, (uint32_t)raw);
    case VT_ISO8601: return fmt_iso8601(buf, (int64_t)raw);
    }
    return -1;
}

static __device__ __noinline__ bool leaf_match_f64(const DevProgram& P, const DevLeaf& L, uint64_t raw) {
    uint8_t buf[VL_FMT_F64_MAX];
    int n = fmt_f64(buf, raw);
    return leaf_match_typed_text(P, L, VT_FLOAT64, buf, (uint32_t)n);
}

static __device__ bool bloom_contains_all_warp(const uint8_t* bloom_be, uint32_t nwords, const uint64_t* hashes, uint32_t nh) {
    if (nwords == 0) return true;
    uint64_t maxbits = (uint64_t)nwords * 64;
    bool ok = true;
    for (uint32_t i = lane_id(); i < nh; i += 32) {
        uint64_t idx = hashes[i] % maxbits;
        uint64_t w = ld_be64(bloom_be + (idx >> 6) * 8);
        if (!((w >> (idx & 63)) & 1)) ok = false;
    }
    return __all_sync(0xffffffffu, ok);
}

static __device__ __forceinline__ bool block_alive_warp(const uint64_t* __restrict__ reg, const BatchView& B, uint32_t b) {
    const uint64_t lo = B.blk_word_off[b], hi = B.blk_word_off[b + 1];
    bool any = false;
    for (uint64_t w = lo + lane_id(); w < hi; w += 32) any |= reg[w] != 0;
    return __any_sync(0xffffffffu, any);
}
static __device__ __forceinline__ uint32_t block_ones_warp(const uint64_t* __restrict__ reg, const BatchView& B, uint32_t b) {
    const uint64_t lo = B.blk_word_off[b], hi = B.blk_word_off[b + 1];
    uint32_t n = 0;
    for (uint64_t w = lo + lane_id(); w < hi; w += 32) n += __popcll(reg[w]);
#pragma unroll
    for (int d = 16; d; d >>= 1) n += __shfl_xor_sync(0xffffffffu, n, d);
    return n;
}
static __global__ void k_andnot(uint64_t* __restrict__ a, const uint64_t* __restrict__ b, uint64_t n) {
    uint64_t i = (uint64_t)blockIdx.x * blockDim.x + threadIdx.x;
    if (i < n) a[i] &= ~b[i];
}

static __global__ void k_prepass(DevProgram P, BatchView B, uint32_t pp_begin, uint32_t pp_count, const int* __restrict__ slots ,
                          int is_or, uint64_t* __restrict__ reg, unsigned long long* __restrict__ stats) {
    uint32_t b = (blockIdx.x * blockDim.x + threadIdx.x) >> 5;
    if (b >= B.nblocks || !block_alive_warp(reg, B, b)) return;
    bool pass = is_or ? false : true;
    unsigned long long bloom_bytes = 0;
    for (uint32_t e = 0; e < pp_count; e++) {
        const DevPrepass& pp = P.prepass[pp_begin + e];
        int slot = slots[e];
        const DevColumn* c = slot >= 0 ? &B.cols[(uint64_t)b * B.nfields + slot] : nullptr;
        bool ok;
        bool skip = false;
        if (c && c->kind == COL_CONST) {
            const uint32_t* to = (const uint32_t*)(P.blob + pp.tok_offs_off);
            const uint8_t* v = B.hdr + c->meta_off;
            ok = true;
            for (uint32_t t = 0; t < pp.ntokens && ok; t++) ok = match_phrase(v, c->meta_len, P.blob + pp.tok_blob_off + to[t], to[t + 1] - to[t]);
        } else if (!c || c->kind == COL_MISSING) {
            ok = false; skip = true;
        } else if (c->vt == VT_DICT) {
            const uint32_t* dof = (const uint32_t*)(B.hdr + c->meta_off);
            const uint8_t* dv = B.hdr + c->meta_off + 4 * (c->dict_len + 1);
            const uint32_t* to = (const uint32_t*)(P.blob + pp.tok_offs_off);
            ok = true;
            for (uint32_t t = 0; t < pp.ntokens && ok; t++) {
                bool found = false;
                for (uint32_t d = 0; d < c->dict_len && !found; d++) found = match_phrase(dv + dof[d], dof[d + 1] - dof[d], P.blob + pp.tok_blob_off + to[t], to[t + 1] - to[t]);
                ok = found;
            }
        } else {
            bloom_bytes += 8ull * pp.nhashes;
            ok = bloom_contains_all_warp(B.hdr + c->bloom_off, c->bloom_words, P.u64s + pp.hashes_off, pp.nhashes);
        }
        if (is_or) { if (!skip && ok) { pass = true; break; } }
        else if (!ok) { pass = false; break; }
    }
    if (is_or && pp_count == 0) pass = true;
    if (lane_id() == 0 && bloom_bytes) atomicAdd(&stats[ST_BLOOM_BYTES], bloom_bytes);
    if (!pass) for (uint64_t w = B.blk_word_off[b] + lane_id(); w < B.blk_word_off[b + 1]; w += 32) reg[w] = 0;
}

#define VL_PLAN_WARPS 8
enum { WC_LENS = 0, WC_TILES = 1, WC_ROW = 2, WC_LENS2 = 3, WC_COUNT = 4 };
#define VL_TILE_BYTES 65536u
struct __align__(16) ScanTile {
    uint64_t off;
    uint32_t bytes;
    uint32_t block;
};
static __global__ void __launch_bounds__(VL_PLAN_WARPS * 32) k_plan_leaf(DevProgram P, BatchView B, uint32_t leaf_idx, int slot, const uint64_t* __restrict__ reg,
                            uint8_t* __restrict__ action, uint64_t* __restrict__ payload, uint32_t* __restrict__ lens_blocks, uint32_t* __restrict__ row_blocks,
                            ScanTile* __restrict__ tiles, uint32_t* __restrict__ work_count,
                            unsigned long long* __restrict__ stats, uint8_t* __restrict__ need = nullptr) {
    __shared__ uint32_t s_cnt[VL_PLAN_WARPS][3], s_off[VL_PLAN_WARPS][3];
    __shared__ unsigned long long s_stat[VL_PLAN_WARPS][4];
    const uint32_t warp = threadIdx.x >> 5;
    const uint32_t b = blockIdx.x * VL_PLAN_WARPS + warp;
    const DevLeaf& L = P.leaves[leaf_idx];
    uint8_t act = ACT_NONE; uint64_t pay = 0;
    unsigned long long bloom_bytes = 0, values_bytes = 0, scan_bytes = 0, scan_off = 0; int err = 0;
    uint32_t need_lens = 0, need_row = 0, ntiles = 0;
    const bool valid = b < B.nblocks;
    const uint32_t ones = valid ? block_ones_warp(reg, B, b) : 0;
    const bool alive = ones != 0;
    if (alive && L.kind == F_NOOP) act = ACT_ALL;
    else if (alive) {
    act = ACT_ALL;
    uint32_t rows = B.blk_rows[b];
    const DevColumn* c = slot >= 0 ? &B.cols[(uint64_t)b * B.nfields + slot] : nullptr;
    const uint8_t* nd = P.blob + L.needle_off; uint32_t nl = L.needle_len;
    if ((L.kind == F_IN && L.in_count == 0) || L.always_none) act = ACT_NONE;
    else if (L.kind == F_TIME) {
        const int64_t mn = (int64_t)L.aux0, mx = (int64_t)L.aux1;
        if (!B.ts || B.ts[b].mt == 0) { act = ACT_NONE; err = ERR_NO_TIMESTAMPS; }
        else if (mn > B.ts[b].max || mx < B.ts[b].first) act = ACT_NONE;
        else if (mn <= B.ts[b].first && mx >= B.ts[b].max) act = ACT_ALL;
        else { act = ACT_TIME; need_row = 1; }
    }
    else if (c && c->kind == COL_CONST) {
        if (L.kind == F_VALUE_TYPE) act = L.aux0 == VTYPE_CONST ? ACT_ALL : ACT_NONE;
        else act = leaf_match_string(P, L, B.hdr + c->meta_off, c->meta_len) ? ACT_ALL : ACT_NONE;
    } else if (!c || c->kind == COL_MISSING) {
        switch (L.kind) {
        case F_PHRASE: case F_EXACT: case F_EXACT_PREFIX: act = nl == 0 ? ACT_ALL : ACT_NONE; break;
        case F_PREFIX: act = ACT_NONE; break;
        case F_IN: act = L.in_has_empty ? ACT_ALL : ACT_NONE; break;
        case F_REGEXP: act = regex_match(P.regexes[L.regex], P.blob, nullptr, 0) ? ACT_ALL : ACT_NONE; break;
        case F_LEN_RANGE: act = L.aux0 == 0 ? ACT_ALL : ACT_NONE; break;
        case F_STRING_RANGE: act = (nl == 0 && L.needle2_len > 0) ? ACT_ALL : ACT_NONE; break;
        case F_IPV4_RANGE: case F_VALUE_TYPE: case F_RANGE: act = ACT_NONE; break;
        case F_ANY_CASE_PHRASE: act = nl == 0 ? ACT_ALL : ACT_NONE; break;
        case F_ANY_CASE_PREFIX: act = ACT_NONE; break;
        case F_SEQUENCE: case F_CONTAINS_ALL: case F_CONTAINS_ANY: act = leaf_match_string(P, L, nullptr, 0) ? ACT_ALL : ACT_NONE; break;
        }
    } else if (L.kind == F_VALUE_TYPE) {
        act = L.aux0 == c->vt ? ACT_ALL : ACT_NONE;
    } else if (c->vt == VT_DICT) {
        const uint32_t* dof = (const uint32_t*)(B.hdr + c->meta_off);
        const uint8_t* dv = B.hdr + c->meta_off + 4 * (c->dict_len + 1);
        uint32_t mask = 0;
        for (uint32_t d = 0; d < c->dict_len; d++) if (leaf_match_string(P, L, dv + dof[d], dof[d + 1] - dof[d])) mask |= 1u << d;
        if (mask == 0) act = ACT_NONE; else { act = ACT_DICT; pay = mask; }
    } else {
        uint32_t vt = c->vt;
        const uint8_t* bloom = B.hdr + c->bloom_off;
        auto probe = [&](const uint64_t* h, uint32_t nh) -> bool {
            if (nh == 0) return true;
            bloom_bytes += 8ull * nh;
            return bloom_contains_all_warp(bloom, c->bloom_words, h, nh);
        };
        const uint64_t* H = P.u64s + L.hashes_off; uint32_t nH = L.nhashes;
        if (vt == VT_STRING) {
            bool ok = true;
            if (L.kind == F_IN) {
                ok = probe(H, L.nhashes);
                if (ok && !(L.in_skip_sets || (uint64_t)L.in_nsets > 10ull * rows)) {
                    bool any = false;
                    const uint32_t* sets = P.u32s + L.in_sets_off;
                    for (uint32_t s = 0; s < L.in_nsets && !any; s++) { bloom_bytes += 8ull * sets[2 * s + 1]; any = bloom_contains_all_warp(bloom, c->bloom_words, P.u64s + sets[2 * s], sets[2 * s + 1]); }
                    ok = any;
                }
            } else if (L.kind == F_CONTAINS_ANY) {
                ok = probe(H, L.nhashes);
                if (ok) {
                    bool any = false;
                    const uint32_t* sets = P.u32s + L.in_sets_off;
                    for (uint32_t s = 0; s < L.in_nsets; s++) { bloom_bytes += 8ull * sets[2 * s + 1]; any |= bloom_contains_all_warp(bloom, c->bloom_words, P.u64s + sets[2 * s], sets[2 * s + 1]); }
                    ok = any;
                }
            } else if (L.kind == F_ANY_CASE_PHRASE || L.kind == F_ANY_CASE_PREFIX || L.kind == F_RANGE) ok = true;
            else ok = probe(H, L.nhashes);
            if (!ok) act = ACT_NONE;
            else if (need) { act = ACT_ROW; values_bytes = 1; }
            else if (c->data_const) act = leaf_match_string(P, L, B.arena + c->data_off, (uint32_t)c->data_len) ? ACT_ALL : ACT_NONE, values_bytes = 1;
            else {
                act = L.str_strategy == STR_SCAN ? ACT_SCAN : L.str_strategy == STR_ALL ? ACT_ALL : ACT_ROW; values_bytes = 1;
                if (act == ACT_SCAN && c->data_len < (uint64_t)VL_SHORT_ROW_BYTES * rows) act = ACT_ROW;
                if (act == ACT_SCAN && (uint64_t)ones * 16 < rows) act = ACT_ROW;
            }
        } else {
            uint32_t w = width_of_vt(vt);
            bool fixed_ok = c->lens_type >= 4 && c->lens_const == w && c->data_len == (uint64_t)rows * w && !c->data_const;
            const TypedNeedle& tn = L.typed[vt];
            uint32_t kind = L.kind;
            if (kind == F_ANY_CASE_PHRASE || kind == F_ANY_CASE_PREFIX) {
                kind = kind == F_ANY_CASE_PHRASE ? F_PHRASE : F_PREFIX;
                if (vt == VT_ISO8601) { H = P.u64s + L.hashes2_off; nH = L.nhashes2; nd = P.blob + L.needle2_off; nl = L.needle2_len; }
            }
            auto in_range = [&]() -> bool {
                switch (vt) {
                case VT_UINT8: case VT_UINT16: case VT_UINT32: case VT_UINT64: case VT_IPV4: return tn.val >= c->min_value && tn.val <= c->max_value;
                case VT_INT64: case VT_ISO8601: return tn.sval >= (int64_t)c->min_value && tn.sval <= (int64_t)c->max_value;
                case VT_FLOAT64: { double f = __longlong_as_double((long long)tn.val), mn = __longlong_as_double((long long)c->min_value), mx = __longlong_as_double((long long)c->max_value); return !(f < mn) && !(f > mx); }
                }
                return false;
            };
            auto exact_path = [&]() {
                if (!tn.ok || !in_range()) { act = ACT_NONE; return; }
                if (!probe(H, nH)) { act = ACT_NONE; return; }
                act = fixed_ok ? ACT_FIXED_EQ : ACT_ROW_EQ; pay = tn.val;
            };
            auto tostring_path = [&](bool use_bloom) {
                if (use_bloom && !probe(H, nH)) { act = ACT_NONE; return; }
                act = ACT_ROW;
            };
            const bool is_uintN = vt == VT_UINT8 || vt == VT_UINT16 || vt == VT_UINT32 || vt == VT_UINT64;
            switch (kind) {
            case F_EXACT: exact_path(); break;
            case F_PHRASE:
                if (vt == VT_FLOAT64) { if (!L.f64_phrase_gate) act = ACT_NONE; else if (L.f64_exact_form) exact_path(); else tostring_path(true); }
                else if (vt == VT_IPV4 || vt == VT_ISO8601) { if (tn.ok) exact_path(); else tostring_path(true); }
                else exact_path();
                break;
            case F_PREFIX:
                if (nl == 0) act = ACT_ALL;
                else if (vt == VT_UINT8 || vt == VT_UINT16 || vt == VT_UINT32 || vt == VT_UINT64) { if (!tn.ok || tn.val > c->max_value) act = ACT_NONE; else tostring_path(false); }
                else if (vt == VT_INT64) { bool dash = nl == 1 && nd[0] == '-'; if (!dash && (!tn.ok || !in_range())) act = ACT_NONE; else tostring_path(false); }
                else if (vt == VT_FLOAT64) { if (!L.f64_prefix_gate) act = ACT_NONE; else tostring_path(true); }
                else tostring_path(true);
                break;
            case F_REGEXP: tostring_path(true); break;
            case F_IN:
                if (L.in_typed_cnt[vt] == 0) act = ACT_NONE;
                else {
                    bool ok = probe(H, L.nhashes);
                    if (ok && !(L.in_skip_sets || (uint64_t)L.in_nsets > 10ull * rows)) {
                        bool any = false;
                        const uint32_t* sets = P.u32s + L.in_sets_off;
                        for (uint32_t s = 0; s < L.in_nsets && !any; s++) { bloom_bytes += 8ull * sets[2 * s + 1]; any = bloom_contains_all_warp(bloom, c->bloom_words, P.u64s + sets[2 * s], sets[2 * s + 1]); }
                        ok = any;
                    }
                    act = !ok ? ACT_NONE : fixed_ok ? ACT_FIXED_IN : ACT_ROW_IN;
                }
                break;
            case F_SEQUENCE:
                if (is_uintN || vt == VT_INT64) { if (L.in_count > 1) act = ACT_NONE; else exact_path(); }
                else if (vt == VT_FLOAT64) tostring_path(true);
                else if (L.in_count == 1 && tn.ok) exact_path();
                else tostring_path(true);
                break;
            case F_CONTAINS_ALL:
                if (is_uintN) {
                    const uint32_t n_values = (uint32_t)L.aux0;
                    if (n_values == 0) act = ACT_ALL;
                    else if (n_values != 1 || L.in_typed_cnt[vt] != 1) act = ACT_NONE;
                    else if (!probe(H, nH)) act = ACT_NONE;
                    else { act = fixed_ok ? ACT_FIXED_EQ : ACT_ROW_EQ; pay = P.u64s[L.in_typed_off[vt]]; }
                } else tostring_path(true);
                break;
            case F_CONTAINS_ANY:
                if (is_uintN) {
                    if (L.in_typed_cnt[vt] == 0) act = ACT_NONE;
                    else {
                        bool ok = probe(H, nH);
                        if (ok && !(L.in_skip_sets || (uint64_t)L.in_nsets > 10ull * rows)) {
                            bool any = false;
                            const uint32_t* sets = P.u32s + L.in_sets_off;
                            for (uint32_t s = 0; s < L.in_nsets && !any; s++) { bloom_bytes += 8ull * sets[2 * s + 1]; any = bloom_contains_all_warp(bloom, c->bloom_words, P.u64s + sets[2 * s], sets[2 * s + 1]); }
                            ok = any;
                        }
                        act = !ok ? ACT_NONE : fixed_ok ? ACT_FIXED_IN : ACT_ROW_IN;
                    }
                } else {
                    bool ok = probe(H, nH);
                    if (ok) {
                        bool any = false;
                        const uint32_t* sets = P.u32s + L.in_sets_off;
                        for (uint32_t s = 0; s < L.in_nsets; s++) { bloom_bytes += 8ull * sets[2 * s + 1]; any |= bloom_contains_all_warp(bloom, c->bloom_words, P.u64s + sets[2 * s], sets[2 * s + 1]); }
                        ok = any;
                    }
                    act = ok ? ACT_ROW : ACT_NONE;
                }
                break;
            case F_RANGE: {
                const double fmn = __longlong_as_double((long long)L.rng_fmin), fmx = __longlong_as_double((long long)L.rng_fmax);
                if (is_uintN) act = (fmx < 0 || L.rng_ulo > c->max_value || L.rng_uhi < c->min_value) ? ACT_NONE : ACT_ROW;
                else if (vt == VT_INT64) act = (L.rng_ilo > (int64_t)c->max_value || L.rng_ihi < (int64_t)c->min_value) ? ACT_NONE : ACT_ROW;
                else if (vt == VT_FLOAT64) act = (fmn > __longlong_as_double((long long)c->max_value) || fmx < __longlong_as_double((long long)c->min_value)) ? ACT_NONE : ACT_ROW;
                else if (vt == VT_IPV4) act = (c->min_value > (uint64_t)L.rng_iphi || c->max_value < (uint64_t)L.rng_iplo) ? ACT_NONE : ACT_ROW;
                else act = (fmx < 0 || L.rng_ilo > (int64_t)c->max_value || L.rng_ihi < (int64_t)c->min_value) ? ACT_NONE : ACT_ROW;
                break;
            }
            case F_EXACT_PREFIX: {
                const bool is_uint = vt == VT_UINT8 || vt == VT_UINT16 || vt == VT_UINT32 || vt == VT_UINT64;
                if (nl == 0) act = ACT_ALL;
                else if (is_uint) act = (L.nhashes > 0 || !tn.ok || tn.val > c->max_value) ? ACT_NONE : ACT_ROW;
                else if (vt == VT_INT64) {
                    bool dash = nl == 1 && nd[0] == '-';
                    if (L.nhashes > 0) act = ACT_NONE;
                    else if (!dash && (!tn.ok || tn.sval > (int64_t)c->max_value || tn.sval < (int64_t)c->min_value)) act = ACT_NONE;
                    else act = ACT_ROW;
                }
                else if (vt == VT_FLOAT64) act = (L.nhashes > 2 * 6 || !probe(H, L.nhashes)) ? ACT_NONE : ACT_ROW;
                else if (vt == VT_IPV4) act = (!(L.gates & GATE_DIGIT_PREFIX) || L.nhashes > 3 * 6 || !probe(H, L.nhashes)) ? ACT_NONE : ACT_ROW;
                else act = (!(L.gates & GATE_DIGIT_PREFIX) || !probe(H, L.nhashes)) ? ACT_NONE : ACT_ROW;
                break;
            }
            case F_LEN_RANGE: {
                const uint64_t mn = L.aux0, mx = L.aux1;
                uint8_t tmp[24];
                if (vt == VT_UINT8 || vt == VT_UINT16 || vt == VT_UINT32 || vt == VT_UINT64) {
                    const uint64_t maxd = vt == VT_UINT8 ? 3 : vt == VT_UINT16 ? 5 : vt == VT_UINT32 ? 10 : 20;
                    if (mn > maxd || mx == 0) act = ACT_NONE;
                    else if (mx < (uint64_t)fmt_u64(tmp, c->min_value) || mn > (uint64_t)fmt_u64(tmp, c->max_value)) act = ACT_NONE;
                    else act = ACT_ROW;
                } else if (vt == VT_INT64) {
                    if (mn > 21 || mx == 0) act = ACT_NONE;
                    else { int a = fmt_i64(tmp, (int64_t)c->min_value), b2 = fmt_i64(tmp, (int64_t)c->max_value); act = (uint64_t)(a > b2 ? a : b2) < mn ? ACT_NONE : ACT_ROW; }
                } else if (vt == VT_FLOAT64) act = (mn > 24 || mx == 0) ? ACT_NONE : ACT_ROW;
                else if (vt == VT_IPV4) act = (mn > 15 || mx < 7) ? ACT_NONE : ACT_ROW;
                else act = (mn > 24 || mx < 24) ? ACT_NONE : ACT_ALL;
                break;
            }
            case F_STRING_RANGE:
                if (vt == VT_INT64) act = (L.gates & GATE_SR_INT) ? ACT_ROW : ACT_NONE;
                else if (vt == VT_FLOAT64) act = (L.gates & GATE_SR_FLOAT) ? ACT_ROW : ACT_NONE;
                else act = (L.gates & GATE_SR_UINT) ? ACT_ROW : ACT_NONE;
                break;
            case F_IPV4_RANGE:
                if (vt != VT_IPV4) act = ACT_NONE;
                else act = (c->min_value > L.aux1 || c->max_value < L.aux0) ? ACT_NONE : ACT_ROW;
                break;
            }
        }
        if (act >= ACT_DICT || values_bytes) values_bytes = lens_stored_bytes(*c, rows) + c->data_len;
    }
    if (c && c->kind == COL_VALUES && c->vt == VT_DICT && act == ACT_DICT) values_bytes = lens_stored_bytes(*c, rows) + c->data_len;
    if (need) {
        if (c && c->kind == COL_VALUES && (values_bytes || act >= ACT_DICT) && lane_id() == 0) need[(uint64_t)b * B.nfields + slot] = 1;
        act = ACT_NONE; values_bytes = 0; bloom_bytes = 0; err = 0;
    } else if (c && c->kind == COL_VALUES && c->values_state != VALUES_STAGED && (values_bytes || act >= ACT_DICT)) {
        act = ACT_NONE; values_bytes = 0; err = ERR_VALUES_ABSENT;
    }
    if (c && c->kind == COL_VALUES && (act == ACT_SCAN || act >= ACT_ROW)) {
        need_lens = 1;
        if (act == ACT_SCAN) { ntiles = (uint32_t)((c->data_len + VL_TILE_BYTES - 1) / VL_TILE_BYTES); scan_bytes = c->data_len; scan_off = c->data_off; }
        else need_row = 1;
    }
    }
    if (need) return;
    if (lane_id() == 0) {
        if (valid) { action[b] = act; payload[b] = pay; }
        if (err) atomicMax(&stats[ST_ERROR], (unsigned long long)err);
        s_cnt[warp][0] = need_lens; s_cnt[warp][1] = ntiles; s_cnt[warp][2] = need_row;
        s_stat[warp][0] = bloom_bytes; s_stat[warp][1] = values_bytes; s_stat[warp][2] = values_bytes ? 1 : 0; s_stat[warp][3] = scan_bytes;
    }
    __syncthreads();
    if (threadIdx.x < 3) {
        uint32_t tot = 0;
        for (int w = 0; w < VL_PLAN_WARPS; w++) { s_off[w][threadIdx.x] = tot; tot += s_cnt[w][threadIdx.x]; }
        const uint32_t base = tot ? atomicAdd(&work_count[threadIdx.x], tot) : 0;
        for (int w = 0; w < VL_PLAN_WARPS; w++) s_off[w][threadIdx.x] += base;
    } else if (threadIdx.x >= 32 && threadIdx.x < 36) {
        const int k = threadIdx.x - 32;
        unsigned long long tot = 0;
        for (int w = 0; w < VL_PLAN_WARPS; w++) tot += s_stat[w][k];
        if (tot) atomicAdd(&stats[k == 0 ? ST_BLOOM_BYTES : k == 1 ? ST_VALUES_BYTES : k == 2 ? ST_COLUMNS_READ : ST_SCAN_BYTES], tot);
    }
    __syncthreads();
    if (need_lens && lane_id() == 0) lens_blocks[s_off[warp][0]] = b;
    if (need_row && lane_id() == 0) row_blocks[s_off[warp][2]] = b;
    for (uint32_t k = lane_id(); k < ntiles; k += 32) {
        const uint32_t t0 = k * VL_TILE_BYTES;
        tiles[s_off[warp][1] + k] = ScanTile{scan_off + t0, (uint32_t)min(scan_bytes - t0, (unsigned long long)VL_TILE_BYTES), b};
    }
}

struct OndiskCol { uint64_t col; uint64_t lens_total; uint64_t rows; };
static __global__ void k_finish_ondisk_cols(const uint8_t* __restrict__ arena, DevColumn* __restrict__ cols, const OndiskCol* __restrict__ oc, uint32_t n,
                                            unsigned long long* __restrict__ status) {
    uint32_t i = blockIdx.x * blockDim.x + threadIdx.x;
    if (i >= n) return;
    DevColumn& c = cols[oc[i].col];
    const uint64_t total = oc[i].lens_total, rows = oc[i].rows;
    unsigned err = 0;
    if (total < 1) err = 1;
    else {
        const uint8_t* p = arena + c.lens_off - 1;
        uint32_t lt = p[0];
        if (lt > 7) err = 2;
        else {
            uint64_t want = lt < 4 ? (rows << lt) : (1ull << (lt - 4));
            if (total - 1 != want) err = 3;
            else {
                c.lens_type = (uint8_t)lt;
                if (lt >= 4) {
                    uint64_t v = 0; for (uint64_t k = 0; k < want; k++) v = (v << 8) | p[1 + k];
                    if (v > 0xFFFFFFFFull) err = 4;
                    else { c.lens_const = (uint32_t)v; c.data_const = (rows >= 2 && c.data_len == v) ? 1 : 0; }
                }
            }
        }
    }
    if (err) atomicMax(&status[0], (unsigned long long)err);
}
struct ColPatch { uint64_t col; DevColumn c; };
static __global__ void k_patch_cols(DevColumn* __restrict__ cols, const ColPatch* __restrict__ p, uint32_t n) {
    const uint32_t i = blockIdx.x * blockDim.x + threadIdx.x;
    if (i < n) cols[p[i].col] = p[i].c;
}
static __global__ void k_unstaged_count(BatchView B, const uint32_t* __restrict__ marks, int slot, unsigned long long* __restrict__ count) {
    const uint32_t b = blockIdx.x * blockDim.x + threadIdx.x;
    if (b >= B.nblocks || marks[b] == 0) return;
    const DevColumn& c = B.cols[(uint64_t)b * B.nfields + slot];
    if (c.kind == COL_VALUES && c.values_state != VALUES_STAGED) atomicAdd(count, 1ull);
}

static __global__ void k_lens_offsets(BatchView B, int slot, const uint32_t* __restrict__ lens_blocks, const uint32_t* __restrict__ work_count,
                               uint32_t* __restrict__ row_off8, uint8_t* __restrict__ ready, unsigned long long* __restrict__ stats, int wc_idx = WC_LENS) {
    const uint32_t nwork = work_count[wc_idx];
    const uint32_t warps = (gridDim.x * blockDim.x) >> 5, lane = lane_id();
    for (uint32_t j = (blockIdx.x * blockDim.x + threadIdx.x) >> 5; j < nwork; j += warps) {
        const uint32_t b = lens_blocks[j];
        if (ready[b]) continue;
        const DevColumn& c = B.cols[(uint64_t)b * B.nfields + slot];
        if (c.values_state != VALUES_STAGED) {
            if (lane == 0) atomicMax(&stats[ST_ERROR], (unsigned long long)ERR_VALUES_ABSENT);
            continue;
        }
        const uint32_t rows = B.blk_rows[b];
        const uint64_t w0 = B.blk_word_off[b]; const uint32_t nw = (uint32_t)(B.blk_word_off[b + 1] - w0);
        const uint8_t* lens = B.arena + c.lens_off;
        if (c.lens_type >= 4) {
            if (lane == 0) {
                if ((unsigned long long)rows * c.lens_const != c.data_len) atomicMax(&stats[ST_ERROR], (unsigned long long)ERR_LENS_MISMATCH);
                ready[b] = 1;
            }
            continue;
        }
        unsigned long long carry = 0;
        for (uint32_t base = 0; base < nw; base += 32) {
            const uint32_t w = base + lane;
            uint32_t g[8] = {0, 0, 0, 0, 0, 0, 0, 0};
            unsigned long long sum = 0;
            if (w < nw) {
                const uint32_t r0 = w * 64, r1 = min(rows, r0 + 64);
                if (c.lens_type == 0) {
                    if (r1 - r0 == 64) {
                        const uint4* v = (const uint4*)(lens + r0);
#pragma unroll
                        for (int q = 0; q < 4; q++) { uint4 x = v[q]; g[2 * q] = __vsadu4(x.x, 0) + __vsadu4(x.y, 0); g[2 * q + 1] = __vsadu4(x.z, 0) + __vsadu4(x.w, 0); }
                    } else for (uint32_t r = r0; r < r1; r++) g[(r - r0) >> 3] += lens[r];
#pragma unroll
                    for (int q = 0; q < 8; q++) sum += g[q];
                } else {
                    unsigned long long g64[8] = {0, 0, 0, 0, 0, 0, 0, 0};
                    for (uint32_t r = r0; r < r1; r++) g64[(r - r0) >> 3] += c.lens_type == 3 ? ld_be64(lens + 8 * (uint64_t)r) : (unsigned long long)row_len(c, lens, r);
#pragma unroll
                    for (int q = 0; q < 8; q++) { sum += g64[q]; g[q] = (uint32_t)min(g64[q], 0xFFFFFFFFull); }
                    if (sum > 0xFFFFFFFFull) sum = 0x100000000ull;
                }
            }
            unsigned long long incl = sum;
#pragma unroll
            for (int d = 1; d < 32; d <<= 1) { unsigned long long t = __shfl_up_sync(0xffffffffu, incl, d); if (lane >= d) incl += t; }
            const unsigned long long excl = carry + incl - sum;
            if (w < nw) {
                uint32_t o = (uint32_t)min(excl, 0xFFFFFFFFull);
                uint4 a, bq;
                a.x = o; o += g[0]; a.y = o; o += g[1]; a.z = o; o += g[2]; a.w = o; o += g[3];
                bq.x = o; o += g[4]; bq.y = o; o += g[5]; bq.z = o; o += g[6]; bq.w = o;
                uint4* dst = (uint4*)(row_off8 + ((w0 + w) << 3));
                dst[0] = a; dst[1] = bq;
            }
            carry += __shfl_sync(0xffffffffu, incl, 31);
        }
        if (lane == 0) {
            if (carry != c.data_len) atomicMax(&stats[ST_ERROR], (unsigned long long)ERR_LENS_MISMATCH);
            ready[b] = 1;
        }
    }
}

struct ScanParams {
    uint32_t mode;
    uint32_t needle_off, needle_len;
    uint32_t pat[4], msk[4];
    int32_t delta[4];
    uint32_t nd16[4];
    uint8_t starts_tok, ends_tok;
    int32_t regex;
};

static __device__ __forceinline__ uint32_t ld_u32_unaligned(const uint8_t* p) {
    const uint32_t* a = (const uint32_t*)((uintptr_t)p & ~(uintptr_t)3);
    return __funnelshift_r(a[0], a[1], 8 * (uint32_t)((uintptr_t)p & 3));
}

static __device__ __forceinline__ void scan_verify_lane(const DevProgram& P, const BatchView& B, const DevColumn& c, const ScanParams& sp, uint32_t b,
                                                     const uint32_t* __restrict__ row_off8, uint32_t pos, uint64_t* __restrict__ leaf_bm) {
    const uint8_t* data = B.arena + c.data_off;
    const uint32_t L = sp.needle_len, n = (uint32_t)c.data_len;
    const uint32_t lens_type = c.lens_type, lens_const = c.lens_const;
    const uint8_t* lens = B.arena + c.lens_off;
    const uint32_t rows = B.blk_rows[b];
    const uint64_t w0 = B.blk_word_off[b];
    if ((uint64_t)pos + L > n) return;
    {
        const uint32_t head = L < 16 ? L : 16;
#pragma unroll
        for (uint32_t k = 0; k < 16; k += 4) {
            if (k >= head) break;
            const uint32_t m = head - k >= 4 ? 0xFFFFFFFFu : (1u << (8 * (head - k))) - 1;
            if ((ld_u32_unaligned(data + pos + k) ^ sp.nd16[k >> 2]) & m) return;
        }
        const uint8_t* nd = P.blob + sp.needle_off;
        for (uint32_t k = 16; k < L; k++) if (data[pos + k] != nd[k]) return;
    }
    uint32_t r, off, len;
    if (lens_type >= 4) {
        len = lens_const;
        if (len == 0) return;
        r = pos / len; off = r * len;
        if (r >= rows) return;
    } else {
        const uint32_t* ro = row_off8 + (w0 << 3);
        const uint32_t n8 = (rows + 7) >> 3;
        uint32_t lo, hi;
        {
            const uint32_t g = min((uint32_t)(__uint2float_rz(pos) * __fdividef(__uint2float_rz(n8), __uint2float_rz(n))), n8 - 1);
            lo = g ? g - 1 : 0; hi = min(g + 1, n8 - 1);
            if (!(ro[lo] <= pos && (hi + 1 >= n8 || ro[hi + 1] > pos))) { lo = 0; hi = n8 - 1; }
        }
        while (lo < hi) { const uint32_t mid = (lo + hi + 1) >> 1; if (ro[mid] <= pos) lo = mid; else hi = mid - 1; }
        const uint32_t r0 = lo * 8, kmax = min(8u, rows - r0);
        uint32_t o = ro[lo];
        r = r0; off = o; len = 0;
        if (lens_type == 0) {
            const uint2 lw = *(const uint2*)(lens + r0);
            const uint64_t l8 = ((uint64_t)lw.y << 32) | lw.x;
            for (uint32_t k = 0; k < kmax && o <= pos; k++) { const uint32_t l = (uint32_t)(l8 >> (8 * k)) & 0xFF; r = r0 + k; off = o; len = l; o += l; }
        } else {
            for (uint32_t k = 0; k < kmax && o <= pos; k++) { const uint32_t l = row_len(c, lens, r0 + k); r = r0 + k; off = o; len = l; o += l; }
        }
        if (pos < off || pos - off >= len) return;
    }
    if ((uint64_t)off + len > n) return;
    if (pos + L > off + len) return;
    const uint8_t* s = data + off; const uint32_t p = pos - off;
    bool hit;
    switch (sp.mode) {
    case SCAN_PHRASE: hit = phrase_boundaries_ok(s, len, p, L, sp.starts_tok, sp.ends_tok); break;
    case SCAN_PREFIX: hit = phrase_boundaries_ok(s, len, p, L, sp.starts_tok, false); break;
    case SCAN_CONTAINS: hit = true; break;
    case SCAN_RX_DOTPLUS: hit = p + L < len; break;
    case SCAN_RX_TAIL: {
        const DevRegex& R = P.regexes[sp.regex];
        hit = find_bytes(s, p, P.blob + R.prefix_off, R.prefix_len, 0) >= 0;
        break;
    }
    default: {
        const DevRegex& R = P.regexes[sp.regex];
        if (R.tail_len) hit = find_bytes(s + p + L, len - p - L, P.blob + R.tail_off, R.tail_len, 0) >= 0;
        else hit = dfa_run(R, P.blob, s + p + L, len - p - L);
        break;
    }
    }
    if (hit) atomicOr((unsigned long long*)&leaf_bm[w0 + (r >> 6)], 1ull << (r & 63));
}

#define VL_SCAN_THREADS 256
#define VL_SCAN_CTAS 4
#define VL_SCAN_UNROLL 4
#define VL_SCAN_ROUNDS 4
#define VL_SCAN_STAGES 2
#define VL_SCAN_ROUND_BYTES (VL_SCAN_THREADS * 16)
#define VL_SCAN_QSTRIDE (VL_TILE_BYTES / VL_SCAN_UNROLL)
static_assert(VL_TILE_BYTES == VL_SCAN_ROUND_BYTES * VL_SCAN_UNROLL * VL_SCAN_ROUNDS, "tile size");
static_assert(VL_SCAN_ROUNDS % VL_SCAN_STAGES == 0 && VL_SCAN_STAGES >= 2, "every round of a tile uses the same register stage in every tile");

template <bool MASKED>
static __device__ __forceinline__ uint32_t scan_word_hits(uint32_t w, const ScanParams& sp) {
    if (MASKED) return (uint32_t)((w & sp.msk[0]) == sp.pat[0]) | (uint32_t)((w & sp.msk[1]) == sp.pat[1]) << 1 | (uint32_t)((w & sp.msk[2]) == sp.pat[2]) << 2 | (uint32_t)((w & sp.msk[3]) == sp.pat[3]) << 3;
    return (uint32_t)(w == sp.pat[0]) | (uint32_t)(w == sp.pat[1]) << 1 | (uint32_t)(w == sp.pat[2]) << 2 | (uint32_t)(w == sp.pat[3]) << 3;
}

template <bool MASKED>
static __device__ __forceinline__ uint32_t scan_vector_hit(const uint4& v, const ScanParams& sp) {
    uint32_t h;
    if (MASKED) {
        asm("{\n\t.reg .pred p;\n\t.reg .b32 t;\n\t"
            "lop3.b32 t, %1, %5, %9, 0x28;\n\tsetp.eq.u32 p, t, 0;\n\t"
            "lop3.b32 t, %1, %6, %10, 0x28;\n\tsetp.eq.or.u32 p, t, 0, p;\n\t"
            "lop3.b32 t, %1, %7, %11, 0x28;\n\tsetp.eq.or.u32 p, t, 0, p;\n\t"
            "lop3.b32 t, %1, %8, %12, 0x28;\n\tsetp.eq.or.u32 p, t, 0, p;\n\t"
            "lop3.b32 t, %2, %5, %9, 0x28;\n\tsetp.eq.or.u32 p, t, 0, p;\n\t"
            "lop3.b32 t, %2, %6, %10, 0x28;\n\tsetp.eq.or.u32 p, t, 0, p;\n\t"
            "lop3.b32 t, %2, %7, %11, 0x28;\n\tsetp.eq.or.u32 p, t, 0, p;\n\t"
            "lop3.b32 t, %2, %8, %12, 0x28;\n\tsetp.eq.or.u32 p, t, 0, p;\n\t"
            "lop3.b32 t, %3, %5, %9, 0x28;\n\tsetp.eq.or.u32 p, t, 0, p;\n\t"
            "lop3.b32 t, %3, %6, %10, 0x28;\n\tsetp.eq.or.u32 p, t, 0, p;\n\t"
            "lop3.b32 t, %3, %7, %11, 0x28;\n\tsetp.eq.or.u32 p, t, 0, p;\n\t"
            "lop3.b32 t, %3, %8, %12, 0x28;\n\tsetp.eq.or.u32 p, t, 0, p;\n\t"
            "lop3.b32 t, %4, %5, %9, 0x28;\n\tsetp.eq.or.u32 p, t, 0, p;\n\t"
            "lop3.b32 t, %4, %6, %10, 0x28;\n\tsetp.eq.or.u32 p, t, 0, p;\n\t"
            "lop3.b32 t, %4, %7, %11, 0x28;\n\tsetp.eq.or.u32 p, t, 0, p;\n\t"
            "lop3.b32 t, %4, %8, %12, 0x28;\n\tsetp.eq.or.u32 p, t, 0, p;\n\t"
            "selp.u32 %0, 1, 0, p;\n\t}"
            : "=r"(h)
            : "r"(v.x), "r"(v.y), "r"(v.z), "r"(v.w), "r"(sp.pat[0]), "r"(sp.pat[1]), "r"(sp.pat[2]), "r"(sp.pat[3]), "r"(sp.msk[0]), "r"(sp.msk[1]), "r"(sp.msk[2]), "r"(sp.msk[3]));
    } else {
        asm("{\n\t.reg .pred p;\n\t"
            "setp.eq.u32 p, %1, %5;\n\tsetp.eq.or.u32 p, %1, %6, p;\n\tsetp.eq.or.u32 p, %1, %7, p;\n\tsetp.eq.or.u32 p, %1, %8, p;\n\t"
            "setp.eq.or.u32 p, %2, %5, p;\n\tsetp.eq.or.u32 p, %2, %6, p;\n\tsetp.eq.or.u32 p, %2, %7, p;\n\tsetp.eq.or.u32 p, %2, %8, p;\n\t"
            "setp.eq.or.u32 p, %3, %5, p;\n\tsetp.eq.or.u32 p, %3, %6, p;\n\tsetp.eq.or.u32 p, %3, %7, p;\n\tsetp.eq.or.u32 p, %3, %8, p;\n\t"
            "setp.eq.or.u32 p, %4, %5, p;\n\tsetp.eq.or.u32 p, %4, %6, p;\n\tsetp.eq.or.u32 p, %4, %7, p;\n\tsetp.eq.or.u32 p, %4, %8, p;\n\t"
            "selp.u32 %0, 1, 0, p;\n\t}"
            : "=r"(h)
            : "r"(v.x), "r"(v.y), "r"(v.z), "r"(v.w), "r"(sp.pat[0]), "r"(sp.pat[1]), "r"(sp.pat[2]), "r"(sp.pat[3]));
    }
    return h;
}

#define VL_SCAN_QCAP 2048
#define VL_SCAN_QFLUSH 192
struct ScanCand { uint32_t block, pos; };

template <bool MASKED>
static __device__ __forceinline__ void scan_vector(const DevProgram& P, const BatchView& B, const DevColumn& c, const ScanParams& sp, uint32_t b,
                                                    const uint32_t* __restrict__ row_off8, uint32_t pos, uint64_t* __restrict__ leaf_bm) {
    const uint32_t n = (uint32_t)c.data_len;
    const uint4 v = pos < n ? __ldg((const uint4*)(B.arena + c.data_off + pos)) : make_uint4(0, 0, 0, 0);
    uint32_t m = scan_word_hits<MASKED>(v.x, sp) | scan_word_hits<MASKED>(v.y, sp) << 4 | scan_word_hits<MASKED>(v.z, sp) << 8 | scan_word_hits<MASKED>(v.w, sp) << 12;
    while (m) {
        const int j = __ffs((int)m) - 1; m &= m - 1;
        const int64_t q = (int64_t)pos + (j & ~3) + sp.delta[j & 3];
        if (q < 0 || q + (int64_t)sp.needle_len > (int64_t)n) continue;
        scan_verify_lane(P, B, c, sp, b, row_off8, (uint32_t)q, leaf_bm);
    }
}

static __device__ __forceinline__ void scan_load_round(uint4 (&v)[VL_SCAN_UNROLL], const BatchView& B, const ScanTile& tl, int round) {
    const uint32_t base = (uint32_t)round * VL_SCAN_ROUND_BYTES + threadIdx.x * 16;
    const uint8_t* __restrict__ ptr = B.arena + tl.off + base;
    if ((uint32_t)(round + 1) * VL_SCAN_ROUND_BYTES + (VL_SCAN_UNROLL - 1) * VL_SCAN_QSTRIDE <= tl.bytes) {
#pragma unroll
        for (int u = 0; u < VL_SCAN_UNROLL; u++) v[u] = __ldg((const uint4*)(ptr + u * VL_SCAN_QSTRIDE));
    } else {
#pragma unroll
        for (int u = 0; u < VL_SCAN_UNROLL; u++) v[u] = base + u * VL_SCAN_QSTRIDE < tl.bytes ? __ldg((const uint4*)(ptr + u * VL_SCAN_QSTRIDE)) : make_uint4(0, 0, 0, 0);
    }
}

template <bool MASKED>
static __device__ __forceinline__ bool scan_round(const uint4 (&v)[VL_SCAN_UNROLL], const ScanParams& sp, uint32_t b, uint32_t pos, ScanCand* s_q, uint32_t* s_cnt) {
    static_assert(VL_SCAN_UNROLL == 4, "one ballot per vector index below");
    uint32_t hits = 0;
#pragma unroll
    for (int u = 0; u < VL_SCAN_UNROLL; u++) hits |= scan_vector_hit<MASKED>(v[u], sp) << u;
    if (!__any_sync(0xffffffffu, hits != 0)) return false;
    const uint32_t lane = threadIdx.x & 31;
    const uint32_t b0 = __ballot_sync(0xffffffffu, hits & 1), b1 = __ballot_sync(0xffffffffu, hits & 2), b2 = __ballot_sync(0xffffffffu, hits & 4), b3 = __ballot_sync(0xffffffffu, hits & 8);
    const uint32_t n0 = __popc(b0), n1 = n0 + __popc(b1), n2 = n1 + __popc(b2), n3 = n2 + __popc(b3);
    uint32_t at0 = 0;
    if (lane == 0) at0 = atomicAdd(s_cnt, n3);
    at0 = __shfl_sync(0xffffffffu, at0, 0);
    const uint32_t below = (1u << lane) - 1u;
    const uint32_t bal[4] = {b0, b1, b2, b3}, first[4] = {at0, at0 + n0, at0 + n1, at0 + n2};
    bool overflow = false;
#pragma unroll
    for (int u = 0; u < VL_SCAN_UNROLL; u++) {
        if (!(hits >> u & 1)) continue;
        const uint32_t at = first[u] + __popc(bal[u] & below);
        if (at < VL_SCAN_QCAP) s_q[at] = ScanCand{b, pos + u * VL_SCAN_QSTRIDE}; else overflow = true;
    }
    return overflow;
}

template <bool MASKED>
static __device__ __noinline__ void scan_tile_inplace(const DevProgram& P, const BatchView& B, int slot, const ScanParams& sp, const ScanTile tl,
                                                      const uint32_t* __restrict__ row_off8, uint64_t* __restrict__ leaf_bm) {
    const DevColumn& c = B.cols[(uint64_t)tl.block * B.nfields + slot];
    const uint32_t tile0 = (uint32_t)(tl.off - c.data_off);
    for (uint32_t p = threadIdx.x * 16; p < tl.bytes; p += VL_SCAN_ROUND_BYTES) scan_vector<MASKED>(P, B, c, sp, tl.block, row_off8, tile0 + p, leaf_bm);
}
template <bool MASKED>
static __device__ __noinline__ void scan_drain(const DevProgram& P, const BatchView& B, int slot, const ScanParams& sp, const uint32_t* __restrict__ row_off8,
                                               uint64_t* __restrict__ leaf_bm, const ScanCand* s_q, uint32_t count) {
    for (uint32_t i = threadIdx.x; i < count; i += blockDim.x) {
        const ScanCand e = s_q[i];
        const DevColumn& c = B.cols[(uint64_t)e.block * B.nfields + slot];
        scan_vector<MASKED>(P, B, c, sp, e.block, row_off8, e.pos - (uint32_t)c.data_off, leaf_bm);
    }
}

static __device__ __forceinline__ ScanTile scan_tile_at(const ScanTile* __restrict__ tiles, uint32_t t, uint32_t ntiles) {
    if (t >= ntiles) return ScanTile{0, 0, 0};
    const uint4 r = __ldg((const uint4*)(tiles + t));
    return ScanTile{(uint64_t)r.y << 32 | r.x, r.z, r.w};
}

template <bool MASKED>
static __global__ void __launch_bounds__(VL_SCAN_THREADS, VL_SCAN_CTAS) k_substr_scan(const __grid_constant__ DevProgram P, const __grid_constant__ BatchView B, int slot, const __grid_constant__ ScanParams sp,
                                                                                      const ScanTile* __restrict__ tiles, const uint32_t* __restrict__ work_count,
                                                                                      const uint32_t* __restrict__ row_off8, uint64_t* __restrict__ leaf_bm) {
    __shared__ ScanCand s_q[VL_SCAN_QCAP];
    __shared__ uint32_t s_cnt, s_t, s_ntiles;
    __shared__ ScanTile s_next;
    if (threadIdx.x == 0) s_cnt = 0;
    __syncthreads();
    uint32_t ntiles = work_count[WC_TILES];
    ScanTile cur = scan_tile_at(tiles, blockIdx.x, ntiles), next = scan_tile_at(tiles, blockIdx.x + gridDim.x, ntiles);
    uint4 v[VL_SCAN_STAGES][VL_SCAN_UNROLL];
#pragma unroll
    for (int s = 0; s < VL_SCAN_STAGES - 1; s++) scan_load_round(v[s], B, cur, s);
    for (uint32_t t = blockIdx.x; t < ntiles; t += gridDim.x) {
        bool overflow = false;
#pragma unroll
        for (int r = 0; r < VL_SCAN_ROUNDS; r++) {
            const int ahead = r + VL_SCAN_STAGES - 1;
            if (ahead < VL_SCAN_ROUNDS) scan_load_round(v[ahead % VL_SCAN_STAGES], B, cur, ahead);
            else scan_load_round(v[ahead % VL_SCAN_STAGES], B, next, ahead - VL_SCAN_ROUNDS);
            overflow |= scan_round<MASKED>(v[r % VL_SCAN_STAGES], sp, cur.block, (uint32_t)cur.off + (uint32_t)r * VL_SCAN_ROUND_BYTES + threadIdx.x * 16, s_q, &s_cnt);
        }
        if (__syncthreads_or((threadIdx.x == 0 && s_cnt >= VL_SCAN_QFLUSH) || overflow)) {
            if (threadIdx.x == 0) { s_t = t; s_ntiles = ntiles; s_next = next; }
            if (__syncthreads_or(overflow)) scan_tile_inplace<MASKED>(P, B, slot, sp, cur, row_off8, leaf_bm);
            scan_drain<MASKED>(P, B, slot, sp, row_off8, leaf_bm, s_q, min(s_cnt, (uint32_t)VL_SCAN_QCAP));
            __syncthreads();
            if (threadIdx.x == 0) s_cnt = 0;
            t = s_t; ntiles = s_ntiles; next = s_next;
            __syncthreads();
#pragma unroll
            for (int s = 0; s < VL_SCAN_STAGES - 1; s++) scan_load_round(v[s], B, next, s);
        }
        cur = next;
        next = scan_tile_at(tiles, t + 2 * gridDim.x, ntiles);
    }
    __syncthreads();
    scan_drain<MASKED>(P, B, slot, sp, row_off8, leaf_bm, s_q, min(s_cnt, (uint32_t)VL_SCAN_QCAP));
}

static __global__ void k_word_match(DevProgram P, BatchView B, uint32_t leaf_idx, int slot, const uint8_t* __restrict__ action, const uint64_t* __restrict__ payload, const uint64_t* __restrict__ reg,
                             uint64_t* __restrict__ leaf_bm, unsigned long long* __restrict__ stats) {
    uint64_t gw = (uint64_t)blockIdx.x * blockDim.x + threadIdx.x;
    if (gw >= B.nwords) return;
    uint32_t b = B.word_block[gw];
    uint8_t act = action[b];
    if (act != ACT_DICT && act != ACT_FIXED_EQ && act != ACT_FIXED_IN) return;
    if (!reg[gw]) { leaf_bm[gw] = 0; return; }
    const DevColumn& c = B.cols[(uint64_t)b * B.nfields + slot];
    const DevLeaf& L = P.leaves[leaf_idx];
    uint32_t rows = B.blk_rows[b];
    uint32_t r0 = (uint32_t)(gw - B.blk_word_off[b]) * 64, r1 = min(rows, r0 + 64);
    const uint8_t* data = B.arena + c.data_off;
    uint64_t bits = 0, pay = payload[b];
    if (act == ACT_DICT) {
        bool bad = false;
        if (r1 - r0 == 64 && ((c.data_off + r0) & 15) == 0) {
            const uint4* v = (const uint4*)(data + r0);
#pragma unroll
            for (int q = 0; q < 4; q++) {
                uint4 x = __ldg(v + q); uint32_t ww[4] = {x.x, x.y, x.z, x.w};
#pragma unroll
                for (int i = 0; i < 4; i++)
#pragma unroll
                    for (int j = 0; j < 4; j++) { uint32_t id = (ww[i] >> (8 * j)) & 0xFF; bad |= id >= c.dict_len; bits |= (uint64_t)((pay >> (id & 7)) & 1) << (q * 16 + i * 4 + j); }
            }
        } else for (uint32_t r = r0; r < r1; r++) { uint32_t id = data[r]; bad |= id >= c.dict_len; bits |= (uint64_t)((pay >> (id & 7)) & 1) << (r - r0); }
        if (bad) atomicMax(&stats[ST_ERROR], (unsigned long long)ERR_DICT_INDEX);
    } else {
        uint32_t w = width_of_vt(c.vt);
        for (uint32_t r = r0; r < r1; r++) {
            uint64_t v = load_fixed_be(data + (uint64_t)r * w, w);
            bool hit = act == ACT_FIXED_EQ ? v == pay : in_contains_typed(L, P.u64s, c.vt, v);
            bits |= (uint64_t)hit << (r - r0);
        }
    }
    leaf_bm[gw] = bits;
}

static __global__ void __launch_bounds__(256, 4) k_row_match(DevProgram P, BatchView B, uint32_t leaf_idx, int slot, const uint32_t* __restrict__ work_blocks,
                                   const uint32_t* __restrict__ work_count, const uint8_t* __restrict__ action, const uint64_t* __restrict__ payload, const uint64_t* __restrict__ reg,
                                   const uint32_t* __restrict__ row_off8, uint64_t* __restrict__ leaf_bm) {
  if (work_count[WC_ROW] == 0) return;
  const DevLeaf& L = P.leaves[leaf_idx];
  const uint64_t nwarps = (uint64_t)gridDim.x * (blockDim.x >> 5), warp = (uint64_t)blockIdx.x * (blockDim.x >> 5) + (threadIdx.x >> 5);
  for (uint64_t base = warp * 32; base < B.nwords; base += nwarps * 32) {
    uint64_t live_l = 0; uint32_t b_l = 0;
    if (base + lane_id() < B.nwords) {
        live_l = reg[base + lane_id()];
        if (live_l) { b_l = B.word_block[base + lane_id()]; const uint8_t a = action[b_l]; if (a < ACT_ROW || a > ACT_ROW_IN) live_l = 0; }
    }
    uint32_t todo = __ballot_sync(0xffffffffu, live_l != 0);
   while (todo) {
    const int src = __ffs((int)todo) - 1; todo &= todo - 1;
    const uint64_t gw = base + (uint32_t)src;
    const uint64_t live = __shfl_sync(0xffffffffu, live_l, src);
    const uint32_t b = __shfl_sync(0xffffffffu, b_l, src);
    const DevColumn& c = B.cols[(uint64_t)b * B.nfields + slot];
    const uint32_t rows = B.blk_rows[b];
    const uint8_t act = action[b]; const uint64_t pay = payload[b];
    const uint64_t w_lo = B.blk_word_off[b];
    uint32_t r0 = (uint32_t)(gw - w_lo) * 64;
    const uint8_t* data = B.arena + c.data_off;
    const uint8_t* lens = B.arena + c.lens_off;
    uint32_t la = 0, lb = 0;
    uint32_t ra = r0 + lane_id(), rb = r0 + 32 + lane_id();
    if (ra < rows) la = row_len(c, lens, ra);
    if (rb < rows) lb = row_len(c, lens, rb);
    uint32_t ia = la, ib = lb;
#pragma unroll
    for (int d = 1; d < 32; d <<= 1) { uint32_t t = __shfl_up_sync(0xffffffffu, ia, d), u = __shfl_up_sync(0xffffffffu, ib, d); if (lane_id() >= d) { ia += t; ib += u; } }
    uint32_t tot_a = __shfl_sync(0xffffffffu, ia, 31);
    uint64_t base = c.lens_type >= 4 ? (uint64_t)r0 * c.lens_const : row_off8[gw << 3];
    uint64_t oa = base + ia - la, ob = base + tot_a + ib - lb;
    if (c.data_const) { oa = ob = 0; la = lb = (uint32_t)c.data_len; }
    bool ha = false, hb = false;
    uint32_t vt = c.vt;
    auto eval = [&](uint64_t off, uint32_t len) -> bool {
        if (off + len > c.data_len) return false;
        const uint8_t* s = data + off;
        if (vt == VT_STRING) return leaf_match_string(P, L, s, len);
        uint32_t w = width_of_vt(vt);
        if (len != w) return false;
        uint64_t raw = load_fixed_be(s, w);
        if (act == ACT_ROW_EQ) return raw == pay;
        if (act == ACT_ROW_IN) return in_contains_typed(L, P.u64s, vt, raw);
        if (L.kind == F_IPV4_RANGE) return raw >= L.aux0 && raw <= L.aux1;
        if (L.kind == F_RANGE) {
            switch (vt) {
            case VT_UINT8: case VT_UINT16: case VT_UINT32: case VT_UINT64: return raw >= L.rng_ulo && raw <= L.rng_uhi;
            case VT_INT64: { const int64_t v = unzigzag64(raw); return v >= L.rng_ilo && v <= L.rng_ihi; }
            case VT_FLOAT64: { const double f = __longlong_as_double((long long)raw); return f >= __longlong_as_double((long long)L.rng_fmin) && f <= __longlong_as_double((long long)L.rng_fmax); }
            case VT_IPV4: return raw >= L.rng_iplo && raw <= L.rng_iphi;
            default: return (int64_t)raw >= L.rng_ilo && (int64_t)raw <= L.rng_ihi;
            }
        }
        if (vt == VT_FLOAT64) return leaf_match_f64(P, L, raw);
        uint8_t buf[32];
        int n = encoded_to_string(vt, raw, buf);
        if (n < 0) return false;
        return leaf_match_typed_text(P, L, vt, buf, (uint32_t)n);
    };
    if (ra < rows && (live >> lane_id() & 1)) ha = eval(oa, la);
    if (rb < rows && (live >> (32 + lane_id()) & 1)) hb = eval(ob, lb);
    uint32_t lo = __ballot_sync(0xffffffffu, ha), hi = __ballot_sync(0xffffffffu, hb);
    if (lane_id() == 0) leaf_bm[gw] = ((uint64_t)hi << 32) | lo;
   }
  }
}

static __global__ void k_apply_leaf(BatchView B, const uint8_t* __restrict__ action, const uint64_t* __restrict__ leaf_bm, uint64_t* __restrict__ reg) {
    uint64_t gw = (uint64_t)blockIdx.x * blockDim.x + threadIdx.x;
    if (gw >= B.nwords) return;
    uint8_t act = action[B.word_block[gw]];
    if (act == ACT_ALL) return;
    reg[gw] = act == ACT_NONE ? 0 : (reg[gw] & leaf_bm[gw]);
}

static __global__ void __launch_bounds__(256) k_finalize(BatchView B, const uint64_t* __restrict__ reg, uint32_t* __restrict__ counts, unsigned long long* __restrict__ stats,
                           unsigned long long* __restrict__ totals4) {
    __shared__ unsigned long long s_acc[8][4];
    const uint32_t warp = threadIdx.x >> 5;
    const uint32_t b = blockIdx.x * 8 + warp;
    unsigned long long rows = 0, matched = 0, blocks = 0, bm_bytes = 0;
    if (b < B.nblocks) {
        uint64_t lo = B.blk_word_off[b], hi = B.blk_word_off[b + 1];
        uint32_t n = 0;
        for (uint64_t w = lo + lane_id(); w < hi; w += 32) n += __popcll(reg[w]);
#pragma unroll
        for (int d = 16; d; d >>= 1) n += __shfl_xor_sync(0xffffffffu, n, d);
        if (lane_id() == 0) counts[b] = n;
        rows = B.blk_rows[b];
        if (n) { matched = n; blocks = 1; bm_bytes = 8ull * (hi - lo); }
    }
    if (lane_id() == 0) { s_acc[warp][0] = rows; s_acc[warp][1] = matched; s_acc[warp][2] = blocks; s_acc[warp][3] = bm_bytes; }
    __syncthreads();
    if (threadIdx.x < 4) {
        unsigned long long t = 0;
        for (int w = 0; w < 8; w++) t += s_acc[w][threadIdx.x];
        if (t) {
            if (threadIdx.x == 0) atomicAdd(&totals4[0], t);
            else if (threadIdx.x == 1) { atomicAdd(&stats[ST_ROWS_MATCHED], t); atomicAdd(&totals4[1], t); }
            else if (threadIdx.x == 2) { atomicAdd(&stats[ST_BLOCKS_MATCHED], t); atomicAdd(&totals4[2], t); }
            else atomicAdd(&stats[ST_BITMAP_BYTES], t);
        }
    }
}

template <typename T>
static __global__ void k_scan_cta(const T* in, uint32_t n, uint64_t* offs, uint64_t* total) {
    __shared__ uint64_t s[1024];
    __shared__ uint64_t carry;
    if (threadIdx.x == 0) carry = 0;
    __syncthreads();
    for (uint32_t base = 0; base < n; base += blockDim.x) {
        const uint32_t i = base + threadIdx.x;
        const uint64_t v = i < n ? in[i] : 0;
        s[threadIdx.x] = v;
        __syncthreads();
        for (uint32_t d = 1; d < blockDim.x; d <<= 1) { uint64_t a = threadIdx.x >= d ? s[threadIdx.x - d] : 0; __syncthreads(); s[threadIdx.x] += a; __syncthreads(); }
        if (i < n) offs[i] = carry + s[threadIdx.x] - v;
        __syncthreads();
        if (threadIdx.x == blockDim.x - 1) carry += s[threadIdx.x];
        __syncthreads();
    }
    if (threadIdx.x == 0) *total = carry;
}

static __device__ unsigned long long cta_incl_scan_u64(unsigned long long v, unsigned long long* s_warp, unsigned long long* s_carry) {
    unsigned long long incl = v;
#pragma unroll
    for (int d = 1; d < 32; d <<= 1) { unsigned long long t = __shfl_up_sync(0xffffffffu, incl, d); if (lane_id() >= d) incl += t; }
    const uint32_t wid = threadIdx.x >> 5, nw = blockDim.x >> 5;
    if (lane_id() == 31) s_warp[wid] = incl;
    __syncthreads();
    unsigned long long pre = *s_carry;
    for (uint32_t k = 0; k < wid; k++) pre += s_warp[k];
    unsigned long long tot = 0;
    for (uint32_t k = 0; k < nw; k++) tot += s_warp[k];
    __syncthreads();
    if (threadIdx.x == 0) *s_carry += tot;
    __syncthreads();
    return pre + incl;
}
static __device__ bool ts_decode_block(const BatchView& B, uint32_t b, unsigned long long* __restrict__ vals) {
    __shared__ unsigned long long s_warp[32];
    __shared__ unsigned long long s_carry;
    __shared__ uint32_t s_cnt[32];
    __shared__ uint32_t s_ccarry;
    __shared__ int s_bad;
    const DevTimestamps t = B.ts[b];
    const uint32_t R = B.blk_rows[b], len = t.len;
    const uint8_t* raw = B.arena + t.off;
    const unsigned long long first = (unsigned long long)t.first;
    if (threadIdx.x == 0) { s_bad = 0; s_ccarry = 0; s_carry = 0; }
    __syncthreads();
    if (t.mt == MT_CONST) {
        for (uint32_t r = threadIdx.x; r < R; r += blockDim.x) vals[r] = first;
        return len == 0;
    }
    if (t.mt == MT_DELTA_CONST) {
        unsigned long long u = 0; bool ok = len >= 1 && len <= 10;
        if (ok) { for (uint32_t k = 0; k < len; k++) { const uint8_t c = raw[k]; if ((k + 1 < len) != (c >= 0x80)) ok = false; u |= (unsigned long long)(c & 0x7F) << (7 * k); } if (len == 10 && raw[9] > 1) ok = false; }
        const unsigned long long d = (u >> 1) ^ (0ull - (u & 1));
        for (uint32_t r = threadIdx.x; r < R; r += blockDim.x) vals[r] = first + (unsigned long long)r * d;
        return ok;
    }
    if (t.mt != MT_NEAREST_DELTA && t.mt != MT_NEAREST_DELTA2) return false;
    const uint32_t min_rows = t.mt == MT_NEAREST_DELTA2 ? 2u : 1u;
    if (R < min_rows) return false;
    const uint32_t need = R - 1;
    for (uint32_t base = 0; base < len; base += blockDim.x) {
        const uint32_t i = base + threadIdx.x;
        const uint8_t c = i < len ? raw[i] : 0x80;
        const bool is_end = i < len && c < 0x80;
        const uint32_t m = __ballot_sync(0xffffffffu, is_end);
        if (lane_id() == 0) s_cnt[threadIdx.x >> 5] = __popc(m);
        __syncthreads();
        uint32_t k = s_ccarry + __popc(m & ((1u << lane_id()) - 1));
        for (uint32_t w = 0; w < (threadIdx.x >> 5); w++) k += s_cnt[w];
        if (is_end) {
            uint32_t s0 = i, n = 1;
            while (s0 > 0 && raw[s0 - 1] >= 0x80 && n <= 10) { s0--; n++; }
            unsigned long long u = 0;
            for (uint32_t q = 0; q < n && q < 10; q++) u |= (unsigned long long)(raw[s0 + q] & 0x7F) << (7 * q);
            if (n > 10 || (n == 10 && c > 1) || k >= need) s_bad = 1;
            else vals[1 + k] = (u >> 1) ^ (0ull - (u & 1));
        }
        __syncthreads();
        if (threadIdx.x == 0) { uint32_t tot = 0; for (uint32_t w = 0; w < (blockDim.x >> 5); w++) tot += s_cnt[w]; s_ccarry += tot; }
        __syncthreads();
    }
    if (threadIdx.x == 0 && (s_ccarry != need || (len > 0 && raw[len - 1] >= 0x80))) s_bad = 1;
    __syncthreads();
    if (s_bad) return false;
    for (int pass = t.mt == MT_NEAREST_DELTA2 ? 0 : 1; pass < 2; pass++) {
        if (threadIdx.x == 0) s_carry = pass == 1 ? first : 0;
        __syncthreads();
        for (uint32_t base = 0; base < need; base += blockDim.x) {
            const uint32_t i = base + threadIdx.x;
            const unsigned long long v = i < need ? vals[1 + i] : 0;
            const unsigned long long sum = cta_incl_scan_u64(v, s_warp, &s_carry);
            if (i < need) vals[1 + i] = sum;
        }
        __syncthreads();
    }
    if (threadIdx.x == 0) vals[0] = first;
    __syncthreads();
    return true;
}

static __global__ void __launch_bounds__(256) k_time_match(BatchView B, long long mn, long long mx, const uint32_t* __restrict__ row_blocks, const uint32_t* __restrict__ work_count,
                                                            unsigned long long* __restrict__ ts_vals, uint64_t* __restrict__ leaf_bm, unsigned long long* __restrict__ stats) {
    const uint32_t nwork = work_count[WC_ROW];
    for (uint32_t j = blockIdx.x; j < nwork; j += gridDim.x) {
        const uint32_t b = row_blocks[j], R = B.blk_rows[b];
        const uint64_t w0 = B.blk_word_off[b];
        unsigned long long* vals = ts_vals + w0 * 64;
        const bool ok = ts_decode_block(B, b, vals);
        if (!ok && threadIdx.x == 0) atomicMax(&stats[ST_ERROR], (unsigned long long)ERR_BAD_TIMESTAMPS);
        const uint32_t rows_padded = (R + 63) / 64 * 64;
        for (uint32_t base = 0; base < rows_padded; base += blockDim.x) {
            const uint32_t r = base + threadIdx.x;
            const long long v = r < R ? (long long)vals[r] : 0;
            const uint32_t m = __ballot_sync(0xffffffffu, ok && r < R && v >= mn && v <= mx);
            if (lane_id() == 0 && r < rows_padded) ((uint32_t*)(leaf_bm + w0))[r >> 5] = m;
        }
        __syncthreads();
    }
}

static __global__ void k_hits_compact(BatchView B, const uint64_t* __restrict__ reg, const uint64_t* __restrict__ offs, uint32_t* __restrict__ hits, uint32_t* __restrict__ hit_block, uint64_t cap) {
    uint32_t b = (blockIdx.x * blockDim.x + threadIdx.x) >> 5;
    if (b >= B.nblocks) return;
    uint64_t lo = B.blk_word_off[b], hi = B.blk_word_off[b + 1];
    uint64_t out = offs[b];
    for (uint64_t w0 = lo; w0 < hi; w0 += 32) {
        uint64_t w = w0 + lane_id();
        uint64_t bits = w < hi ? reg[w] : 0;
        uint32_t n = __popcll(bits), incl = n;
#pragma unroll
        for (int d = 1; d < 32; d <<= 1) { uint32_t t = __shfl_up_sync(0xffffffffu, incl, d); if (lane_id() >= d) incl += t; }
        uint64_t pos = out + incl - n;
        uint32_t rbase = (uint32_t)(w - lo) * 64;
        while (bits) { int k = __ffsll((long long)bits) - 1; bits &= bits - 1; if (pos < cap) { hits[pos] = rbase + k; hit_block[pos] = b; } pos++; }
        out += __shfl_sync(0xffffffffu, incl, 31);
    }
}
static __global__ void k_hit_blocks_list(BatchView B, const uint32_t* __restrict__ counts, int slot, int mode, uint32_t* __restrict__ list, uint32_t* __restrict__ work_count) {
    const uint32_t b = blockIdx.x * blockDim.x + threadIdx.x;
    if (b >= B.nblocks || counts[b] == 0) return;
    if (mode == 0) {
        if (slot < 0 || !cell_needs_offsets(B.cols[(uint64_t)b * B.nfields + slot])) return;
        list[atomicAdd(&work_count[WC_LENS], 1u)] = b;
    } else list[atomicAdd(&work_count[WC_ROW], 1u)] = b;
}
static __global__ void __launch_bounds__(256) k_ts_decode_list(BatchView B, const uint32_t* __restrict__ row_blocks, const uint32_t* __restrict__ work_count,
                                                                unsigned long long* __restrict__ ts_vals, unsigned long long* __restrict__ stats) {
    const uint32_t nwork = work_count[WC_ROW];
    for (uint32_t j = blockIdx.x; j < nwork; j += gridDim.x) {
        const uint32_t b = row_blocks[j];
        const bool ok = B.ts && B.ts[b].mt && ts_decode_block(B, b, ts_vals + B.blk_word_off[b] * 64);
        if (!ok && threadIdx.x == 0) atomicMax(&stats[ST_ERROR], (unsigned long long)(B.ts && B.ts[b].mt ? ERR_BAD_TIMESTAMPS : ERR_NO_TIMESTAMPS));
        __syncthreads();
    }
}
static __global__ void k_gather_ts(BatchView B, const uint32_t* __restrict__ hits, const uint32_t* __restrict__ hit_block, uint64_t nhits, const unsigned long long* __restrict__ ts_vals,
                                   long long* __restrict__ out) {
    const uint64_t h = (uint64_t)blockIdx.x * blockDim.x + threadIdx.x;
    if (h < nhits) out[h] = (long long)ts_vals[B.blk_word_off[hit_block[h]] * 64 + hits[h]];
}
static __device__ __forceinline__ bool cell_typed(const DevColumn* c) { return c && c->kind == COL_VALUES && c->vt != VT_STRING && c->vt != VT_DICT; }
static __device__ __forceinline__ const DevColumn* cell_at(const BatchView& B, int slot, uint32_t b) { return slot >= 0 ? &B.cols[(uint64_t)b * B.nfields + slot] : nullptr; }
static __device__ __forceinline__ void report_error(unsigned long long* stats, uint32_t err) { if (err) atomicMax(&stats[ST_ERROR], (unsigned long long)err); }
static __device__ __forceinline__ uint32_t cell_raw(const BatchView& B, const DevColumn& c, uint32_t b, uint32_t r, const uint32_t* __restrict__ row_off8, const uint8_t** p, uint32_t* n) {
    if (c.values_state != VALUES_STAGED) return ERR_VALUES_ABSENT;
    uint64_t off = 0; uint32_t len;
    if (c.data_const) len = (uint32_t)c.data_len;
    else if (c.lens_type >= 4) { len = c.lens_const; off = (uint64_t)r * len; }
    else {
        const uint8_t* lens = B.arena + c.lens_off;
        uint32_t o = row_off8[(B.blk_word_off[b] << 3) + (r >> 3)];
        for (uint32_t q = r & ~7u; q < r; q++) o += row_len(c, lens, q);
        off = o; len = row_len(c, lens, r);
    }
    if (off + len > c.data_len) return ERR_LENS_MISMATCH;
    *p = B.arena + c.data_off + off; *n = len;
    return ERR_NONE;
}
static __device__ __forceinline__ uint32_t cell_text_raw(const BatchView& B, const DevColumn* c, uint32_t b, uint32_t r, const uint32_t* __restrict__ row_off8, const uint8_t** p,
                                                         uint32_t* n) {
    const uint8_t* src = nullptr; uint32_t len = 0, err = ERR_NONE;
    if (c && c->kind == COL_CONST) { src = B.hdr + c->meta_off; len = c->meta_len; }
    else if (c && c->kind == COL_VALUES) {
        err = cell_raw(B, *c, b, r, row_off8, &src, &len);
        if (!err && c->vt != VT_STRING && len != width_of_vt(c->vt)) err = ERR_BAD_WIDTH;
        if (!err && c->vt == VT_DICT) {
            const uint32_t id = src[0];
            if (id >= c->dict_len) err = ERR_DICT_INDEX;
            else { const uint32_t* dof = (const uint32_t*)(B.hdr + c->meta_off); src = B.hdr + c->meta_off + 4 * (c->dict_len + 1) + dof[id]; len = dof[id + 1] - dof[id]; }
        }
        if (err) len = 0;
    }
    *p = src; *n = len;
    return err;
}
static __device__ __noinline__ uint32_t cell_text(const BatchView& B, const DevColumn* c, uint32_t b, uint32_t r, const uint32_t* __restrict__ row_off8, uint8_t* buf, const uint8_t** p, uint32_t* n) {
    const uint32_t err = cell_text_raw(B, c, b, r, row_off8, p, n);
    if (!err && cell_typed(c)) {
        const uint64_t raw = load_fixed_be(*p, *n);
        const int k = c->vt == VT_FLOAT64 ? fmt_f64(buf, raw) : encoded_to_string(c->vt, raw, buf);
        *p = buf; *n = k > 0 ? (uint32_t)k : 0;
    }
    return err;
}
static __device__ __forceinline__ const uint8_t* plain_dict_ids(const BatchView& B, const DevColumn& c, uint32_t rows) {
    const bool plain = c.kind == COL_VALUES && c.vt == VT_DICT && c.values_state == VALUES_STAGED && c.lens_type >= 4 && c.lens_const == 1 && c.data_len == rows && !c.data_const;
    return plain ? B.arena + c.data_off : nullptr;
}
static __global__ void k_gather_values(BatchView B, int slot, const uint32_t* __restrict__ hits, const uint32_t* __restrict__ hit_block, uint64_t nhits, const uint32_t* __restrict__ row_off8,
                                       int pass, uint32_t* __restrict__ lens_out, const uint64_t* __restrict__ offs, uint8_t* __restrict__ out, unsigned long long* __restrict__ stats) {
    const uint64_t h = (uint64_t)blockIdx.x * blockDim.x + threadIdx.x;
    if (h >= nhits) return;
    uint8_t buf[VL_FMT_F64_MAX];
    const uint8_t* src; uint32_t len;
    const uint32_t b = hit_block[h];
    report_error(stats, cell_text(B, cell_at(B, slot, b), b, hits[h], row_off8, buf, &src, &len));
    if (pass == 0) { lens_out[h] = len; return; }
    uint8_t* d = out + offs[h];
    for (uint32_t k = 0; k < len; k++) d[k] = src[k];
}
#define VL_SCAN_TILE 2048
static __global__ void __launch_bounds__(256) k_scan_tiles(const uint32_t* __restrict__ v, uint64_t n, unsigned long long* __restrict__ tile_sums, unsigned long long* __restrict__ offs, int pass) {
    __shared__ unsigned long long s_w[8];
    const uint64_t base = (uint64_t)blockIdx.x * VL_SCAN_TILE + (uint64_t)threadIdx.x * 8;
    unsigned long long x[8], sum = 0;
#pragma unroll
    for (int k = 0; k < 8; k++) { x[k] = base + k < n ? v[base + k] : 0; sum += x[k]; }
    unsigned long long incl = sum;
#pragma unroll
    for (int d = 1; d < 32; d <<= 1) { unsigned long long t = __shfl_up_sync(0xffffffffu, incl, d); if (lane_id() >= d) incl += t; }
    if (lane_id() == 31) s_w[threadIdx.x >> 5] = incl;
    __syncthreads();
    unsigned long long pre = 0, tot = 0;
    for (uint32_t k = 0; k < 8; k++) { if (k < (threadIdx.x >> 5)) pre += s_w[k]; tot += s_w[k]; }
    if (pass == 0) { if (threadIdx.x == 0) tile_sums[blockIdx.x] = tot; return; }
    unsigned long long o = tile_sums[blockIdx.x] + pre + incl - sum;
#pragma unroll
    for (int k = 0; k < 8; k++) { if (base + k < n) offs[base + k] = o; o += x[k]; }
}

static __device__ bool le_values_string(const uint8_t* a, uint32_t an, const uint8_t* b2, uint32_t bn, bool excl) {
    const double fa = mn::parse_math_number(a, an);
    if (fa == fa) { const double fb = mn::parse_math_number(b2, bn); if (fb == fb) return excl ? fa < fb : fa <= fb; }
    const uint32_t m = an < bn ? an : bn;
    int cmp = 0;
    for (uint32_t i = 0; i < m && !cmp; i++) cmp = (int)a[i] - (int)b2[i];
    if (!cmp) cmp = an < bn ? -1 : an > bn ? 1 : 0;
    return excl ? cmp < 0 : cmp <= 0;
}
static __global__ void __launch_bounds__(256) k_plan_pair(DevProgram P, BatchView B, uint32_t leaf_idx, int slot_a, int slot_b, const uint64_t* __restrict__ reg, uint8_t* __restrict__ action,
                                                           uint64_t* __restrict__ payload, uint32_t* __restrict__ lens_a, uint32_t* __restrict__ lens_b, uint32_t* __restrict__ row_blocks,
                                                           uint32_t* __restrict__ work_count, unsigned long long* __restrict__ stats, uint8_t* __restrict__ need = nullptr) {
    const uint32_t b = (blockIdx.x * blockDim.x + threadIdx.x) >> 5;
    if (b >= B.nblocks) return;
    const DevLeaf& L = P.leaves[leaf_idx];
    const bool alive = block_alive_warp(reg, B, b);
    if (lane_id() != 0) return;
    uint8_t act = ACT_NONE; uint64_t mode = PAIR_STRINGS;
    if (alive && !L.always_none) {
        const bool le = L.kind == F_LE_FIELD, excl = L.pair_excl != 0;
        const DevColumn* ca = slot_a >= 0 ? &B.cols[(uint64_t)b * B.nfields + slot_a] : nullptr;
        const DevColumn* cb = slot_b >= 0 ? &B.cols[(uint64_t)b * B.nfields + slot_b] : nullptr;
        const int ka = ca ? ca->kind : COL_MISSING, kb = cb ? cb->kind : COL_MISSING;
        const bool consta = ka == COL_CONST && ca->meta_len > 0, constb = kb == COL_CONST && cb->meta_len > 0;
        const bool vala = ka == COL_VALUES, valb = kb == COL_VALUES;
        if (consta && constb) {
            const uint8_t* x = B.hdr + ca->meta_off; const uint8_t* y = B.hdr + cb->meta_off;
            const bool m = le ? le_values_string(x, ca->meta_len, y, cb->meta_len, excl) : bytes_equal(x, ca->meta_len, y, cb->meta_len);
            act = m ? ACT_ALL : ACT_NONE;
        } else if (consta || constb) act = ACT_PAIR;
        else if (!vala && !valb) act = (le && excl) ? ACT_NONE : ACT_ALL;
        else if (!vala || !valb) act = ACT_PAIR;
        else if (ca->vt != cb->vt || ca->vt == VT_STRING) act = ACT_PAIR;
        else { act = ACT_PAIR; mode = ca->vt == VT_DICT ? PAIR_DICT : PAIR_BINARY; }
        if (act == ACT_PAIR && need) {
            if (vala) need[(uint64_t)b * B.nfields + slot_a] = 1;
            if (valb) need[(uint64_t)b * B.nfields + slot_b] = 1;
            return;
        }
        if (act == ACT_PAIR && ((vala && ca->values_state != VALUES_STAGED) || (valb && cb->values_state != VALUES_STAGED))) {
// ... 575 lines not shown
```

Before: 21.71 billion.

## Fold last leaf apply into finalize, fuse lens offsets into plan, dynamic scan tile claiming

The final leaf's k_apply_leaf is folded into a combined k_finish kernel that applies the leaf bitmap and counts bits in one pass. When the root is a single leaf, it writes directly into the register from the init bitmap, which skips the leaf_bm memset and copy. The separate k_lens_offsets launch is removed: plan_leaf now computes row offsets per block inline. The substring scan moves from static strided tile assignment to an atomic work-claim counter for load balancing. An optional env-gated per-op event trace and CTA completion timestamps are added for profiling.

```diff
diff --git a/victorialogs_b200/csrc/vl_engine.cu b/victorialogs_b200/csrc/vl_engine.cu
--- a/victorialogs_b200/csrc/vl_engine.cu
+++ b/victorialogs_b200/csrc/vl_engine.cu
@@ -96,6 +96,7 @@
 ZstdWriter& zstd_writer() { static ZstdWriter z; return z; }
 
 void launch_check(vlscan_ctx* ctx) { ctx->launches++; VL_CUDA(cudaGetLastError()); }
+const char* trace_path() { static const char* p = [] { const char* e = getenv("VLSCAN_STEP_TRACE"); return e && *e ? e : nullptr; }(); return p; }
 inline unsigned cdiv(uint64_t a, uint64_t b) { return (unsigned)((a + b - 1) / b); }
 
 struct Carve {
@@ -452,8 +453,8 @@
         return r.as<uint64_t>();
     }
     void free_reg() { regs_used--; }
-    void copy_reg(uint64_t* dst, const uint64_t* src) { if (B.nwords) VL_CUDA(cudaMemcpyAsync(dst, src, B.nwords * 8, cudaMemcpyDeviceToDevice, ctx->stream)); }
-    void andnot(uint64_t* a, const uint64_t* b) { if (!B.nwords) return; k_andnot<<<cdiv(B.nwords, 256), 256, 0, ctx->stream>>>(a, b, B.nwords); launch_check(ctx); }
+    void copy_reg(uint64_t* dst, const uint64_t* src) { if (B.nwords) op("copy reg", [&] { VL_CUDA(cudaMemcpyAsync(dst, src, B.nwords * 8, cudaMemcpyDeviceToDevice, ctx->stream)); }); }
+    void andnot(uint64_t* a, const uint64_t* b) { if (B.nwords) op("k_andnot", [&] { k_andnot<<<cdiv(B.nwords, 256), 256, 0, ctx->stream>>>(a, b, B.nwords); launch_check(ctx); }); }
     void prepass(const PNode& nd, uint64_t* reg) {
         if (nd.prepass_count == 0) return;
         std::vector<int> slots(nd.prepass_count);
@@ -461,25 +462,45 @@
         size_t off = slots_cursor; slots_cursor += slots.size();
         ctx->slots.ensure(std::max<size_t>(slots_total * 4, 16));
         VL_CUDA(cudaMemcpyAsync(ctx->slots.as<int>() + off, slots.data(), slots.size() * 4, cudaMemcpyHostToDevice, ctx->stream));
-        k_prepass<<<cdiv((uint64_t)B.nblocks * 32, 128), 128, 0, ctx->stream>>>(P, B, (uint32_t)nd.prepass_begin, (uint32_t)nd.prepass_count, ctx->slots.as<int>() + off,
-                                                                             nd.kind == F_OR, reg, stats);
-        launch_check(ctx);
+        op("k_prepass", [&] {
+            k_prepass<<<cdiv((uint64_t)B.nblocks * 32, 128), 128, 0, ctx->stream>>>(P, B, (uint32_t)nd.prepass_begin, (uint32_t)nd.prepass_count, ctx->slots.as<int>() + off,
+                                                                                 nd.kind == F_OR, reg, stats);
+            launch_check(ctx);
+        });
     }
     size_t slots_cursor = 0, slots_total = 0;
 
-    void leaf(int leaf_idx, uint64_t* reg) {
+    bool root_leaf = false;
+    enum { FOLD_NONE, FOLD_LEAF_BM, FOLD_INIT } fold = FOLD_NONE;
+    bool trace_on = false;
+    template <class F> void op(const char* name, F&& f) {
+        if (!trace_on) { f(); return; }
+        if (ctx->trace_used == ctx->trace.size()) {
+            vlscan_ctx::TraceOp t{nullptr, nullptr, nullptr};
+            VL_CUDA(cudaEventCreate(&t.before)); VL_CUDA(cudaEventCreate(&t.after));
+            ctx->trace.push_back(t);
+        }
+        vlscan_ctx::TraceOp& t = ctx->trace[ctx->trace_used++];
+        t.name = name;
+        VL_CUDA(cudaEventRecord(t.before, ctx->stream)); f(); VL_CUDA(cudaEventRecord(t.after, ctx->stream));
+    }
+    void apply(uint64_t* reg, bool last) {
+        if (last) { fold = root_leaf ? FOLD_INIT : FOLD_LEAF_BM; return; }
+        if (B.nwords) op("k_apply_leaf", [&] { k_apply_leaf<<<cdiv(B.nwords, 256), 256, 0, ctx->stream>>>(B, ctx->action.as<uint8_t>(), ctx->leaf_bm.as<uint64_t>(), reg); launch_check(ctx); });
+    }
+
+    void leaf(int leaf_idx, uint64_t* reg, bool last) {
         const DevLeaf& L = prog->p.leaves[leaf_idx];
         if (L.kind == F_NOOP) return;
         int slot = L.field >= 0 ? field_slot[L.field] : -1;
         uint8_t* action = ctx->action.as<uint8_t>(); uint64_t* payload = ctx->payload.as<uint64_t>(); uint64_t* leaf_bm = ctx->leaf_bm.as<uint64_t>();
         uint32_t* lens_blocks = ctx->lens_blocks.as<uint32_t>(); uint32_t* row_blocks = ctx->row_blocks.as<uint32_t>(); uint32_t* wc = ctx->work_count.as<uint32_t>();
         ScanTile* tiles = ctx->tiles.as<ScanTile>();
-        VL_CUDA(cudaMemsetAsync(wc, 0, WC_COUNT * 4, ctx->stream));
+        op("memset work_count", [&] { VL_CUDA(cudaMemsetAsync(wc, 0, WC_COUNT * 4, ctx->stream)); });
         if (L.kind == F_EQ_FIELD || L.kind == F_LE_FIELD) {
             const int slot_b = field_slot[L.field2];
             uint32_t* lens_b = ctx->lens_blocks2.as<uint32_t>();
-            k_plan_pair<<<cdiv((uint64_t)B.nblocks * 32, 256), 256, 0, ctx->stream>>>(P, B, (uint32_t)leaf_idx, slot, slot_b, reg, action, payload, lens_blocks, lens_b, row_blocks, wc, stats);
-            launch_check(ctx);
+            op("k_plan_pair", [&] { k_plan_pair<<<cdiv((uint64_t)B.nblocks * 32, 256), 256, 0, ctx->stream>>>(P, B, (uint32_t)leaf_idx, slot, slot_b, reg, action, payload, lens_blocks, lens_b, row_blocks, wc, stats); launch_check(ctx); });
             if (B.nwords) {
                 const int persistent = ctx->sm_count * 8;
                 const uint32_t *ro_a = nullptr, *ro_b = nullptr;
@@ -487,49 +508,56 @@
                     const int sl = side ? slot_b : slot;
                     if (sl < 0) continue;
                     uint8_t* ready = ctx->ready[sl].as<uint8_t>();
-                    if (!ctx->ready_cleared[sl]) { VL_CUDA(cudaMemsetAsync(ready, 0, B.nblocks, ctx->stream)); ctx->ready_cleared[sl] = 1; }
-                    k_lens_offsets<<<persistent, 256, 0, ctx->stream>>>(B, sl, side ? lens_b : lens_blocks, wc, ctx->row_off8[sl].as<uint32_t>(), ready, stats, side ? WC_LENS2 : WC_LENS); launch_check(ctx);
+                    if (!ctx->ready_cleared[sl]) { op("memset ready", [&] { VL_CUDA(cudaMemsetAsync(ready, 0, B.nblocks, ctx->stream)); }); ctx->ready_cleared[sl] = 1; }
+                    op("k_lens_offsets", [&] { k_lens_offsets<<<persistent, 256, 0, ctx->stream>>>(B, sl, side ? lens_b : lens_blocks, wc, ctx->row_off8[sl].as<uint32_t>(), ready, stats, side ? WC_LENS2 : WC_LENS); launch_check(ctx); });
                     (side ? ro_b : ro_a) = ctx->row_off8[sl].as<uint32_t>();
                 }
-                k_row_pair<<<persistent, 256, 0, ctx->stream>>>(P, B, (uint32_t)leaf_idx, slot, slot_b, row_blocks, wc, payload, reg, ro_a, ro_b, leaf_bm, stats); launch_check(ctx);
-                k_apply_leaf<<<cdiv(B.nwords, 256), 256, 0, ctx->stream>>>(B, action, leaf_bm, reg); launch_check(ctx);
+                op("k_row_pair", [&] { k_row_pair<<<persistent, 256, 0, ctx->stream>>>(P, B, (uint32_t)leaf_idx, slot, slot_b, row_blocks, wc, payload, reg, ro_a, ro_b, leaf_bm, stats); launch_check(ctx); });
             }
+            apply(reg, last);
             return;
         }
-        k_plan_leaf<<<cdiv(B.nblocks, VL_PLAN_WARPS), VL_PLAN_WARPS * 32, 0, ctx->stream>>>(P, B, (uint32_t)leaf_idx, slot, reg, action, payload, lens_blocks, row_blocks, tiles, wc, stats);
-        launch_check(ctx);
+        const uint64_t* live = root_leaf ? batch->init_bitmap.as<uint64_t>() : reg;
+        uint64_t* out = root_leaf ? reg : leaf_bm;
+        if (root_leaf && B.nwords) op("memset reg", [&] { VL_CUDA(cudaMemsetAsync(reg, 0, B.nwords * 8, ctx->stream)); });
+        uint32_t* ro = slot >= 0 ? ctx->row_off8[slot].as<uint32_t>() : nullptr; uint8_t* ready = slot >= 0 ? ctx->ready[slot].as<uint8_t>() : nullptr;
+        if (slot >= 0 && !ctx->ready_cleared[slot]) { op("memset ready", [&] { VL_CUDA(cudaMemsetAsync(ready, 0, B.nblocks, ctx->stream)); }); ctx->ready_cleared[slot] = 1; }
+        op("k_plan_leaf", [&] {
+            k_plan_leaf<<<cdiv(B.nblocks, VL_PLAN_WARPS), VL_PLAN_WARPS * 32, 0, ctx->stream>>>(P, B, (uint32_t)leaf_idx, slot, root_leaf ? nullptr : reg, action, payload, ro, ready, row_blocks, tiles, wc, stats);
+            launch_check(ctx);
+        });
         if (slot >= 0 && B.nwords) {
-            uint32_t* ro = ctx->row_off8[slot].as<uint32_t>(); uint8_t* ready = ctx->ready[slot].as<uint8_t>();
-            if (!ctx->ready_cleared[slot]) { VL_CUDA(cudaMemsetAsync(ready, 0, B.nblocks, ctx->stream)); ctx->ready_cleared[slot] = 1; }
-            const int persistent = ctx->sm_count * 8;
             const uint32_t vts = batch->slot_vt_mask.empty() ? ~0u : batch->slot_vt_mask[slot];
             const bool has_string = vts >> VT_STRING & 1, has_dict = vts >> VT_DICT & 1;
             const bool has_numeric = (vts & ~((1u << VT_STRING) | (1u << VT_DICT))) != 0;
             const bool may_scan = L.str_strategy == STR_SCAN && has_string;
             const bool may_row = (has_string && L.str_strategy != STR_ALL) || has_numeric;
-            if (may_scan || may_row) { k_lens_offsets<<<persistent, 256, 0, ctx->stream>>>(B, slot, lens_blocks, wc, ro, ready, stats); launch_check(ctx); }
             if (may_scan) {
-                VL_CUDA(cudaMemsetAsync(leaf_bm, 0, B.nwords * 8, ctx->stream));
+                if (!root_leaf) op("memset leaf_bm", [&] { VL_CUDA(cudaMemsetAsync(leaf_bm, 0, B.nwords * 8, ctx->stream)); });
                 ScanParams sp; memset(&sp, 0, sizeof sp);
                 sp.mode = L.scan_mode; sp.needle_off = L.scan_needle_off; sp.needle_len = L.scan_needle_len; sp.starts_tok = L.starts_tok; sp.ends_tok = L.ends_tok; sp.regex = L.regex;
                 const bool masked = fill_scan_patterns(prog->p.blob.data() + L.scan_needle_off, L.scan_needle_len, sp.pat, sp.msk, sp.delta, sp.nd16);
                 if (L.scan_mode == SCAN_CONTAINS || L.scan_mode >= SCAN_RX_DOTPLUS) { sp.starts_tok = sp.ends_tok = 0; }
+                const int grid = ctx->sm_count * ctx->scan_occ[masked ? 1 : 0];
+                unsigned long long* cta_done = nullptr;
+                if (trace_on) { ctx->cta_done.ensure((size_t)grid * 8); cta_done = ctx->cta_done.as<unsigned long long>(); ctx->cta_done_n = (uint32_t)grid; }
                 auto& evp = next_scan_events();
                 VL_CUDA(cudaEventRecord(evp.first, ctx->stream));
-                if (masked) k_substr_scan<true><<<ctx->sm_count * ctx->scan_occ[1], VL_SCAN_THREADS, 0, ctx->stream>>>(P, B, slot, sp, tiles, wc, ro, leaf_bm);
-                else k_substr_scan<false><<<ctx->sm_count * ctx->scan_occ[0], VL_SCAN_THREADS, 0, ctx->stream>>>(P, B, slot, sp, tiles, wc, ro, leaf_bm);
-                launch_check(ctx);
+                op("k_substr_scan", [&] {
+                    if (masked) k_substr_scan<true><<<grid, VL_SCAN_THREADS, 0, ctx->stream>>>(P, B, slot, sp, tiles, wc, ro, out, cta_done);
+                    else k_substr_scan<false><<<grid, VL_SCAN_THREADS, 0, ctx->stream>>>(P, B, slot, sp, tiles, wc, ro, out, cta_done);
+                    launch_check(ctx);
+                });
                 VL_CUDA(cudaEventRecord(evp.second, ctx->stream));
             }
-            if (may_row) { k_row_match<<<ctx->sm_count * ctx->row_occ, 256, 0, ctx->stream>>>(P, B, (uint32_t)leaf_idx, slot, row_blocks, wc, action, payload, reg, ro, leaf_bm); launch_check(ctx); }
-            if (has_dict || has_numeric) { k_word_match<<<cdiv(B.nwords, 128), 128, 0, ctx->stream>>>(P, B, (uint32_t)leaf_idx, slot, action, payload, reg, leaf_bm, stats); launch_check(ctx); }
+            if (may_row) op("k_row_match", [&] { k_row_match<<<ctx->sm_count * ctx->row_occ, 256, 0, ctx->stream>>>(P, B, (uint32_t)leaf_idx, slot, row_blocks, wc, action, payload, live, ro, out); launch_check(ctx); });
+            if (has_dict || has_numeric) op("k_word_match", [&] { k_word_match<<<cdiv(B.nwords, 128), 128, 0, ctx->stream>>>(P, B, (uint32_t)leaf_idx, slot, action, payload, live, out, stats); launch_check(ctx); });
         }
         if (L.kind == F_TIME && B.nwords) {
             ctx->ts_vals.ensure(B.nwords * 64 * 8);
-            k_time_match<<<ctx->sm_count * 4, 256, 0, ctx->stream>>>(B, (long long)L.aux0, (long long)L.aux1, row_blocks, wc, ctx->ts_vals.as<unsigned long long>(), leaf_bm, stats);
-            launch_check(ctx);
-        }
-        if (B.nwords) { k_apply_leaf<<<cdiv(B.nwords, 256), 256, 0, ctx->stream>>>(B, action, leaf_bm, reg); launch_check(ctx); }
+            op("k_time_match", [&] { k_time_match<<<ctx->sm_count * 4, 256, 0, ctx->stream>>>(B, (long long)L.aux0, (long long)L.aux1, row_blocks, wc, ctx->ts_vals.as<unsigned long long>(), out, stats); launch_check(ctx); });
+        }
+        apply(reg, last);
     }
     std::pair<cudaEvent_t, cudaEvent_t>& next_scan_events() {
         if (ctx->scan_events_used == ctx->scan_events.size()) { cudaEvent_t a, b; VL_CUDA(cudaEventCreate(&a)); VL_CUDA(cudaEventCreate(&b)); ctx->scan_events.emplace_back(a, b); }
@@ -543,7 +571,7 @@
             k_plan_pair<<<cdiv((uint64_t)B.nblocks * 32, 256), 256, 0, ctx->stream>>>(P, B, (uint32_t)leaf_idx, slot, field_slot[L.field2], reg, nullptr, nullptr, nullptr, nullptr, nullptr, nullptr, stats, need);
         } else {
             if (slot < 0) return;
-            k_plan_leaf<<<cdiv(B.nblocks, VL_PLAN_WARPS), VL_PLAN_WARPS * 32, 0, ctx->stream>>>(P, B, (uint32_t)leaf_idx, slot, reg, nullptr, nullptr, nullptr, nullptr, nullptr, nullptr, stats, need);
+            k_plan_leaf<<<cdiv(B.nblocks, VL_PLAN_WARPS), VL_PLAN_WARPS * 32, 0, ctx->stream>>>(P, B, (uint32_t)leaf_idx, slot, reg, nullptr, nullptr, nullptr, nullptr, nullptr, nullptr, nullptr, stats, need);
         }
         launch_check(ctx);
     }
@@ -562,31 +590,55 @@
         default: probe_leaf(nd.leaf, reg, need);
         }
     }
-    void node(int id, uint64_t* reg) {
+    void node(int id, uint64_t* reg, bool last) {
         const PNode& nd = prog->p.nodes[id];
         switch (nd.kind) {
         case F_NOOP: break;
-        case F_AND: prepass(nd, reg); for (int k : nd.kids) node(k, reg); break;
+        case F_AND: prepass(nd, reg); for (size_t i = 0; i < nd.kids.size(); i++) node(nd.kids[i], reg, last && i + 1 == nd.kids.size()); break;
         case F_OR: {
             prepass(nd, reg);
             uint64_t* res = new_reg(); uint64_t* tmp = new_reg();
             copy_reg(res, reg);
-            for (int k : nd.kids) { copy_reg(tmp, res); node(k, tmp); andnot(res, tmp); }
+            for (int k : nd.kids) { copy_reg(tmp, res); node(k, tmp, false); andnot(res, tmp); }
             andnot(reg, res);
             free_reg(); free_reg();
             break;
         }
-        case F_NOT: { uint64_t* tmp = new_reg(); copy_reg(tmp, reg); node(nd.kids[0], tmp); andnot(reg, tmp); free_reg(); break; }
-        default: leaf(nd.leaf, reg);
+        case F_NOT: { uint64_t* tmp = new_reg(); copy_reg(tmp, reg); node(nd.kids[0], tmp, false); andnot(reg, tmp); free_reg(); break; }
+        default: leaf(nd.leaf, reg, last);
         }
     }
 };
+}
+
+static void write_trace(vlscan_ctx* ctx) {
+    if (!trace_path() || !ctx->trace_used) return;
+    std::string s = "{\"ops\": [";
+    char buf[160];
+    for (size_t i = 0; i < ctx->trace_used; i++) {
+        float a = 0, b = 0;
+        VL_CUDA(cudaEventElapsedTime(&a, ctx->ev_begin, ctx->trace[i].before)); VL_CUDA(cudaEventElapsedTime(&b, ctx->ev_begin, ctx->trace[i].after));
+        snprintf(buf, sizeof buf, "%s[\"%s\", %.4f, %.4f]", i ? ", " : "", ctx->trace[i].name, a, b);
+        s += buf;
+    }
+    s += "]";
+    if (ctx->cta_done_n) {
+        std::vector<unsigned long long> t(ctx->cta_done_n);
+        VL_CUDA(cudaMemcpy(t.data(), ctx->cta_done.p, t.size() * 8, cudaMemcpyDeviceToHost));
+        std::sort(t.begin(), t.end());
+        snprintf(buf, sizeof buf, ", \"scan_cta_done_ms\": [0, %.4f, %.4f], \"scan_ctas\": %u", (t[t.size() / 2] - t[0]) / 1e6, (t.back() - t[0]) / 1e6, ctx->cta_done_n);
+        s += buf;
+    }
+    s += "}\n";
+    ctx->trace_used = 0; ctx->cta_done_n = 0;
+    if (FILE* f = fopen(trace_path(), "a")) { fputs(s.c_str(), f); fclose(f); }
 }
 
 static void read_stats(vlscan_ctx* ctx, vlscan_stats* st, bool check_error) {
     unsigned long long h[ST_COUNT];
     VL_CUDA(cudaMemcpyAsync(h, ctx->stats.p, sizeof h, cudaMemcpyDeviceToHost, ctx->stream));
     VL_CUDA(cudaStreamSynchronize(ctx->stream));
+    write_trace(ctx);
     if (check_error && h[ST_ERROR]) {
         static const char* const msg[] = {"", "cannot unmarshal strings: row lengths do not add up to the data length", "too big index for dict value",
                                           "unexpected length for binary representation of a number", "", "", "the filter needs the timestamps of a block that was handed over without them", "cannot unmarshal timestamps",
@@ -625,16 +677,27 @@
     for (uint32_t s = 0; s < batch->nfields; s++) { ctx->row_off8[s].ensure(nw * 32); ctx->ready[s].ensure(nb); }
     uint64_t launches0 = ctx->launches;
     ctx->scan_events_used = 0;
+    ctx->trace_used = 0; ctx->cta_done_n = 0;
+    run.trace_on = trace_path() != nullptr;
     run.stats = ctx->stats.as<unsigned long long>();
     VL_CUDA(cudaEventRecord(ctx->ev_begin, ctx->stream));
-    VL_CUDA(cudaMemsetAsync(ctx->stats.p, 0, ST_COUNT * 8, ctx->stream));
-    VL_CUDA(cudaMemsetAsync(ctx->totals.p, 0, 32, ctx->stream));
+    run.op("memset stats", [&] { VL_CUDA(cudaMemsetAsync(ctx->stats.p, 0, ST_COUNT * 8, ctx->stream)); VL_CUDA(cudaMemsetAsync(ctx->totals.p, 0, 32, ctx->stream)); });
+    const bool generic = getenv("VLSCAN_GENERIC_LEAF") != nullptr;
+    const PNode& root = pr.nodes[pr.root];
+    const bool root_is_leaf = root.kind != F_NOOP && root.kind != F_AND && root.kind != F_OR && root.kind != F_NOT;
+    const uint32_t root_kind = root_is_leaf ? pr.leaves[root.leaf].kind : F_NOOP;
+    run.root_leaf = !generic && batch->nblocks && root_is_leaf && root_kind != F_NOOP && root_kind != F_EQ_FIELD && root_kind != F_LE_FIELD;
     uint64_t* reg = run.new_reg();
-    run.copy_reg(reg, batch->init_bitmap.as<uint64_t>());
+    if (!run.root_leaf) run.copy_reg(reg, batch->init_bitmap.as<uint64_t>());
     if (batch->nblocks) {
-        run.node(pr.root, reg);
-        k_finalize<<<cdiv(batch->nblocks, 8), 256, 0, ctx->stream>>>(run.B, reg, ctx->counts.as<uint32_t>(), run.stats, ctx->totals.as<unsigned long long>());
-        launch_check(ctx);
+        run.node(pr.root, reg, !generic);
+        const bool fold = run.fold != ScanRun::FOLD_NONE;
+        run.op("k_finish", [&] {
+            k_finish<<<cdiv(batch->nblocks, 8), 256, 0, ctx->stream>>>(run.B, fold ? ctx->action.as<uint8_t>() : nullptr, ctx->leaf_bm.as<uint64_t>(),
+                                                                     run.fold == ScanRun::FOLD_INIT ? batch->init_bitmap.as<uint64_t>() : nullptr, reg,
+                                                                     ctx->counts.as<uint32_t>(), run.stats, ctx->totals.as<unsigned long long>());
+            launch_check(ctx);
+        });
     }
     VL_CUDA(cudaEventRecord(ctx->ev_end, ctx->stream));
     ctx->last_batch = batch; ctx->has_result = true; ctx->kept = false; ctx->last_launches = ctx->launches - launches0;
@@ -713,6 +776,8 @@
     if (ctx->pinned) cudaFreeHost(ctx->pinned);
     delete ctx->recycle;
     for (auto& e : ctx->scan_events) { cudaEventDestroy(e.first); cudaEventDestroy(e.second); }
+    for (auto& t : ctx->trace) { cudaEventDestroy(t.before); cudaEventDestroy(t.after); }
+    ctx->cta_done.release();
     if (ctx->ev_begin) cudaEventDestroy(ctx->ev_begin);
     if (ctx->ev_end) cudaEventDestroy(ctx->ev_end);
     if (ctx->copy_stream) cudaStreamDestroy(ctx->copy_stream);
diff --git a/victorialogs_b200/csrc/vl_engine.h b/victorialogs_b200/csrc/vl_engine.h
--- a/victorialogs_b200/csrc/vl_engine.h
+++ b/victorialogs_b200/csrc/vl_engine.h
@@ -115,6 +115,9 @@
     vl::HostPool* pool = nullptr;
     cudaEvent_t ev_begin = nullptr, ev_end = nullptr;
     std::vector<std::pair<cudaEvent_t, cudaEvent_t>> scan_events; size_t scan_events_used = 0;
+    struct TraceOp { const char* name; cudaEvent_t before, after; };
+    std::vector<TraceOp> trace; size_t trace_used = 0;
+    vl::DevBuf cta_done; uint32_t cta_done_n = 0;
     const vlscan_batch* last_batch = nullptr;
     uint64_t last_nblocks = 0, last_nwords = 0, last_rows = 0;
     vlscan_batch* recycle = nullptr;
diff --git a/victorialogs_b200/csrc/vl_kernels.cuh b/victorialogs_b200/csrc/vl_kernels.cuh
--- a/victorialogs_b200/csrc/vl_kernels.cuh
+++ b/victorialogs_b200/csrc/vl_kernels.cuh
@@ -234,27 +234,85 @@
 }
 
 #define VL_PLAN_WARPS 8
-enum { WC_LENS = 0, WC_TILES = 1, WC_ROW = 2, WC_LENS2 = 3, WC_COUNT = 4 };
+enum { WC_LENS = 0, WC_TILES = 1, WC_ROW = 2, WC_LENS2 = 3, WC_TILE_CLAIM = 4, WC_COUNT = 5 };
 #define VL_TILE_BYTES 65536u
 struct __align__(16) ScanTile {
     uint64_t off;
     uint32_t bytes;
     uint32_t block;
 };
+
+static __device__ __noinline__ void lens_offsets_block(const BatchView& B, const DevColumn& c, uint32_t b, uint32_t* __restrict__ row_off8,
+                                                       uint8_t* __restrict__ ready, unsigned long long* __restrict__ stats) {
+    const uint32_t lane = lane_id();
+    const uint32_t rows = B.blk_rows[b];
+    const uint64_t w0 = B.blk_word_off[b]; const uint32_t nw = (uint32_t)(B.blk_word_off[b + 1] - w0);
+    const uint8_t* lens = B.arena + c.lens_off;
+    if (c.lens_type >= 4) {
+        if (lane == 0) {
+            if ((unsigned long long)rows * c.lens_const != c.data_len) atomicMax(&stats[ST_ERROR], (unsigned long long)ERR_LENS_MISMATCH);
+            ready[b] = 1;
+        }
+        return;
+    }
+    unsigned long long carry = 0;
+    for (uint32_t base = 0; base < nw; base += 32) {
+        const uint32_t w = base + lane;
+        uint32_t g[8] = {0, 0, 0, 0, 0, 0, 0, 0};
+        unsigned long long sum = 0;
+        if (w < nw) {
+            const uint32_t r0 = w * 64, r1 = min(rows, r0 + 64);
+            if (c.lens_type == 0) {
+                if (r1 - r0 == 64) {
+                    const uint4* v = (const uint4*)(lens + r0);
+#pragma unroll
+                    for (int q = 0; q < 4; q++) { uint4 x = v[q]; g[2 * q] = __vsadu4(x.x, 0) + __vsadu4(x.y, 0); g[2 * q + 1] = __vsadu4(x.z, 0) + __vsadu4(x.w, 0); }
+                } else for (uint32_t r = r0; r < r1; r++) g[(r - r0) >> 3] += lens[r];
+#pragma unroll
+                for (int q = 0; q < 8; q++) sum += g[q];
+            } else {
+                unsigned long long g64[8] = {0, 0, 0, 0, 0, 0, 0, 0};
+                for (uint32_t r = r0; r < r1; r++) g64[(r - r0) >> 3] += c.lens_type == 3 ? ld_be64(lens + 8 * (uint64_t)r) : (unsigned long long)row_len(c, lens, r);
+#pragma unroll
+                for (int q = 0; q < 8; q++) { sum += g64[q]; g[q] = (uint32_t)min(g64[q], 0xFFFFFFFFull); }
+                if (sum > 0xFFFFFFFFull) sum = 0x100000000ull;
+            }
+        }
+        unsigned long long incl = sum;
+#pragma unroll
+        for (int d = 1; d < 32; d <<= 1) { unsigned long long t = __shfl_up_sync(0xffffffffu, incl, d); if (lane >= d) incl += t; }
+        const unsigned long long excl = carry + incl - sum;
+        if (w < nw) {
+            uint32_t o = (uint32_t)min(excl, 0xFFFFFFFFull);
+            uint4 a, bq;
+            a.x = o; o += g[0]; a.y = o; o += g[1]; a.z = o; o += g[2]; a.w = o; o += g[3];
+            bq.x = o; o += g[4]; bq.y = o; o += g[5]; bq.z = o; o += g[6]; bq.w = o;
+            uint4* dst = (uint4*)(row_off8 + ((w0 + w) << 3));
+            dst[0] = a; dst[1] = bq;
+        }
+        carry += __shfl_sync(0xffffffffu, incl, 31);
+    }
+    if (lane == 0) {
+        if (carry != c.data_len) atomicMax(&stats[ST_ERROR], (unsigned long long)ERR_LENS_MISMATCH);
+        ready[b] = 1;
+    }
+}
+
 static __global__ void __launch_bounds__(VL_PLAN_WARPS * 32) k_plan_leaf(DevProgram P, BatchView B, uint32_t leaf_idx, int slot, const uint64_t* __restrict__ reg,
-                            uint8_t* __restrict__ action, uint64_t* __restrict__ payload, uint32_t* __restrict__ lens_blocks, uint32_t* __restrict__ row_blocks,
-                            ScanTile* __restrict__ tiles, uint32_t* __restrict__ work_count,
+                            uint8_t* __restrict__ action, uint64_t* __restrict__ payload, uint32_t* __restrict__ row_off8, uint8_t* __restrict__ ready,
+                            uint32_t* __restrict__ row_blocks, ScanTile* __restrict__ tiles, uint32_t* __restrict__ work_count,
                             unsigned long long* __restrict__ stats, uint8_t* __restrict__ need = nullptr) {
-    __shared__ uint32_t s_cnt[VL_PLAN_WARPS][3], s_off[VL_PLAN_WARPS][3];
+    __shared__ uint32_t s_cnt[VL_PLAN_WARPS][2], s_off[VL_PLAN_WARPS][2];
     __shared__ unsigned long long s_stat[VL_PLAN_WARPS][4];
     const uint32_t warp = threadIdx.x >> 5;
     const uint32_t b = blockIdx.x * VL_PLAN_WARPS + warp;
     const DevLeaf& L = P.leaves[leaf_idx];
     uint8_t act = ACT_NONE; uint64_t pay = 0;
     unsigned long long bloom_bytes = 0, values_bytes = 0, scan_bytes = 0, scan_off = 0; int err = 0;
-    uint32_t need_lens = 0, need_row = 0, ntiles = 0;
+    uint32_t need_row = 0, ntiles = 0;
+    const DevColumn* lens_col = nullptr;
     const bool valid = b < B.nblocks;
-    const uint32_t ones = valid ? block_ones_warp(reg, B, b) : 0;
+    const uint32_t ones = !valid ? 0 : reg ? block_ones_warp(reg, B, b) : B.blk_rows[b];
     const bool alive = ones != 0;
     if (alive && L.kind == F_NOOP) act = ACT_ALL;
     else if (alive) {
@@ -486,7 +544,7 @@
         act = ACT_NONE; values_bytes = 0; err = ERR_VALUES_ABSENT;
     }
     if (c && c->kind == COL_VALUES && (act == ACT_SCAN || act >= ACT_ROW)) {
-        need_lens = 1;
+        lens_col = c;
         if (act == ACT_SCAN) { ntiles = (uint32_t)((c->data_len + VL_TILE_BYTES - 1) / VL_TILE_BYTES); scan_bytes = c->data_len; scan_off = c->data_off; }
         else need_row = 1;
     }
@@ -495,14 +553,14 @@
     if (lane_id() == 0) {
         if (valid) { action[b] = act; payload[b] = pay; }
         if (err) atomicMax(&stats[ST_ERROR], (unsigned long long)err);
-        s_cnt[warp][0] = need_lens; s_cnt[warp][1] = ntiles; s_cnt[warp][2] = need_row;
+        s_cnt[warp][0] = ntiles; s_cnt[warp][1] = need_row;
         s_stat[warp][0] = bloom_bytes; s_stat[warp][1] = values_bytes; s_stat[warp][2] = values_bytes ? 1 : 0; s_stat[warp][3] = scan_bytes;
     }
     __syncthreads();
-    if (threadIdx.x < 3) {
+    if (threadIdx.x < 2) {
         uint32_t tot = 0;
         for (int w = 0; w < VL_PLAN_WARPS; w++) { s_off[w][threadIdx.x] = tot; tot += s_cnt[w][threadIdx.x]; }
-        const uint32_t base = tot ? atomicAdd(&work_count[threadIdx.x], tot) : 0;
+        const uint32_t base = tot ? atomicAdd(&work_count[threadIdx.x ? WC_ROW : WC_TILES], tot) : 0;
         for (int w = 0; w < VL_PLAN_WARPS; w++) s_off[w][threadIdx.x] += base;
     } else if (threadIdx.x >= 32 && threadIdx.x < 36) {
         const int k = threadIdx.x - 32;
@@ -511,12 +569,12 @@
         if (tot) atomicAdd(&stats[k == 0 ? ST_BLOOM_BYTES : k == 1 ? ST_VALUES_BYTES : k == 2 ? ST_COLUMNS_READ : ST_SCAN_BYTES], tot);
     }
     __syncthreads();
-    if (need_lens && lane_id() == 0) lens_blocks[s_off[warp][0]] = b;
-    if (need_row && lane_id() == 0) row_blocks[s_off[warp][2]] = b;
+    if (need_row && lane_id() == 0) row_blocks[s_off[warp][1]] = b;
     for (uint32_t k = lane_id(); k < ntiles; k += 32) {
         const uint32_t t0 = k * VL_TILE_BYTES;
-        tiles[s_off[warp][1] + k] = ScanTile{scan_off + t0, (uint32_t)min(scan_bytes - t0, (unsigned long long)VL_TILE_BYTES), b};
-    }
+        tiles[s_off[warp][0] + k] = ScanTile{scan_off + t0, (uint32_t)min(scan_bytes - t0, (unsigned long long)VL_TILE_BYTES), b};
+    }
+    if (lens_col && !ready[b]) lens_offsets_block(B, *lens_col, b, row_off8, ready, stats);
 }
 
 struct OndiskCol { uint64_t col; uint64_t lens_total; uint64_t rows; };
@@ -571,57 +629,7 @@
             if (lane == 0) atomicMax(&stats[ST_ERROR], (unsigned long long)ERR_VALUES_ABSENT);
             continue;
         }
-        const uint32_t rows = B.blk_rows[b];
-        const uint64_t w0 = B.blk_word_off[b]; const uint32_t nw = (uint32_t)(B.blk_word_off[b + 1] - w0);
-        const uint8_t* lens = B.arena + c.lens_off;
-        if (c.lens_type >= 4) {
-            if (lane == 0) {
-                if ((unsigned long long)rows * c.lens_const != c.data_len) atomicMax(&stats[ST_ERROR], (unsigned long long)ERR_LENS_MISMATCH);
-                ready[b] = 1;
-            }
-            continue;
-        }
-        unsigned long long carry = 0;
-        for (uint32_t base = 0; base < nw; base += 32) {
-            const uint32_t w = base + lane;
-            uint32_t g[8] = {0, 0, 0, 0, 0, 0, 0, 0};
-            unsigned long long sum = 0;
-            if (w < nw) {
-                const uint32_t r0 = w * 64, r1 = min(rows, r0 + 64);
-                if (c.lens_type == 0) {
-                    if (r1 - r0 == 64) {
-                        const uint4* v = (const uint4*)(lens + r0);
-#pragma unroll
-                        for (int q = 0; q < 4; q++) { uint4 x = v[q]; g[2 * q] = __vsadu4(x.x, 0) + __vsadu4(x.y, 0); g[2 * q + 1] = __vsadu4(x.z, 0) + __vsadu4(x.w, 0); }
-                    } else for (uint32_t r = r0; r < r1; r++) g[(r - r0) >> 3] += lens[r];
-#pragma unroll
-                    for (int q = 0; q < 8; q++) sum += g[q];
-                } else {
-                    unsigned long long g64[8] = {0, 0, 0, 0, 0, 0, 0, 0};
-                    for (uint32_t r = r0; r < r1; r++) g64[(r - r0) >> 3] += c.lens_type == 3 ? ld_be64(lens + 8 * (uint64_t)r) : (unsigned long long)row_len(c, lens, r);
-#pragma unroll
-                    for (int q = 0; q < 8; q++) { sum += g64[q]; g[q] = (uint32_t)min(g64[q], 0xFFFFFFFFull); }
-                    if (sum > 0xFFFFFFFFull) sum = 0x100000000ull;
-                }
-            }
-            unsigned long long incl = sum;
-#pragma unroll
-            for (int d = 1; d < 32; d <<= 1) { unsigned long long t = __shfl_up_sync(0xffffffffu, incl, d); if (lane >= d) incl += t; }
-            const unsigned long long excl = carry + incl - sum;
-            if (w < nw) {
-                uint32_t o = (uint32_t)min(excl, 0xFFFFFFFFull);
-                uint4 a, bq;
-                a.x = o; o += g[0]; a.y = o; o += g[1]; a.z = o; o += g[2]; a.w = o; o += g[3];
-                bq.x = o; o += g[4]; bq.y = o; o += g[5]; bq.z = o; o += g[6]; bq.w = o;
-                uint4* dst = (uint4*)(row_off8 + ((w0 + w) << 3));
-                dst[0] = a; dst[1] = bq;
-            }
-            carry += __shfl_sync(0xffffffffu, incl, 31);
-        }
-        if (lane == 0) {
-            if (carry != c.data_len) atomicMax(&stats[ST_ERROR], (unsigned long long)ERR_LENS_MISMATCH);
-            ready[b] = 1;
-        }
+        lens_offsets_block(B, c, b, row_off8, ready, stats);
     }
 }
 
@@ -845,10 +853,11 @@
 
 template <bool MASKED>
 static __global__ void __launch_bounds__(VL_SCAN_THREADS, VL_SCAN_CTAS) k_substr_scan(const __grid_constant__ DevProgram P, const __grid_constant__ BatchView B, int slot, const __grid_constant__ ScanParams sp,
-                                                                                      const ScanTile* __restrict__ tiles, const uint32_t* __restrict__ work_count,
-                                                                                      const uint32_t* __restrict__ row_off8, uint64_t* __restrict__ leaf_bm) {
+                                                                                      const ScanTile* __restrict__ tiles, uint32_t* __restrict__ work_count,
+                                                                                      const uint32_t* __restrict__ row_off8, uint64_t* __restrict__ leaf_bm,
+                                                                                      unsigned long long* __restrict__ cta_done) {
     __shared__ ScanCand s_q[VL_SCAN_QCAP];
-    __shared__ uint32_t s_cnt, s_t, s_ntiles;
+    __shared__ uint32_t s_cnt, s_ntiles, s_k, s_claim[2];
     __shared__ ScanTile s_next;
     if (threadIdx.x == 0) s_cnt = 0;
     __syncthreads();
@@ -857,7 +866,9 @@
     uint4 v[VL_SCAN_STAGES][VL_SCAN_UNROLL];
 #pragma unroll
     for (int s = 0; s < VL_SCAN_STAGES - 1; s++) scan_load_round(v[s], B, cur, s);
-    for (uint32_t t = blockIdx.x; t < ntiles; t += gridDim.x) {
+    for (uint32_t k = 0; cur.bytes; k ^= 1) {
+        uint32_t claim = ntiles;
+        if (threadIdx.x == 0 && next.bytes) claim = 2 * gridDim.x + atomicAdd(&work_count[WC_TILE_CLAIM], 1u);
         bool overflow = false;
 #pragma unroll
         for (int r = 0; r < VL_SCAN_ROUNDS; r++) {
@@ -866,22 +877,24 @@
             else scan_load_round(v[ahead % VL_SCAN_STAGES], B, next, ahead - VL_SCAN_ROUNDS);
             overflow |= scan_round<MASKED>(v[r % VL_SCAN_STAGES], sp, cur.block, (uint32_t)cur.off + (uint32_t)r * VL_SCAN_ROUND_BYTES + threadIdx.x * 16, s_q, &s_cnt);
         }
+        if (threadIdx.x == 0) s_claim[k] = claim;
         if (__syncthreads_or((threadIdx.x == 0 && s_cnt >= VL_SCAN_QFLUSH) || overflow)) {
-            if (threadIdx.x == 0) { s_t = t; s_ntiles = ntiles; s_next = next; }
+            if (threadIdx.x == 0) { s_ntiles = ntiles; s_next = next; s_k = k; }
             if (__syncthreads_or(overflow)) scan_tile_inplace<MASKED>(P, B, slot, sp, cur, row_off8, leaf_bm);
             scan_drain<MASKED>(P, B, slot, sp, row_off8, leaf_bm, s_q, min(s_cnt, (uint32_t)VL_SCAN_QCAP));
             __syncthreads();
             if (threadIdx.x == 0) s_cnt = 0;
-            t = s_t; ntiles = s_ntiles; next = s_next;
+            ntiles = s_ntiles; next = s_next; k = s_k;
             __syncthreads();
 #pragma unroll
             for (int s = 0; s < VL_SCAN_STAGES - 1; s++) scan_load_round(v[s], B, next, s);
         }
         cur = next;
-        next = scan_tile_at(tiles, t + 2 * gridDim.x, ntiles);
+        next = scan_tile_at(tiles, s_claim[k], ntiles);
     }
     __syncthreads();
     scan_drain<MASKED>(P, B, slot, sp, row_off8, leaf_bm, s_q, min(s_cnt, (uint32_t)VL_SCAN_QCAP));
+    if (cta_done && threadIdx.x == 0) { unsigned long long ns; asm volatile("mov.u64 %0, %%globaltimer;" : "=l"(ns)); cta_done[blockIdx.x] = ns; }
 }
 
 static __global__ void k_word_match(DevProgram P, BatchView B, uint32_t leaf_idx, int slot, const uint8_t* __restrict__ action, const uint64_t* __restrict__ payload, const uint64_t* __restrict__ reg,
@@ -1002,16 +1015,24 @@
     reg[gw] = act == ACT_NONE ? 0 : (reg[gw] & leaf_bm[gw]);
 }
 
-static __global__ void __launch_bounds__(256) k_finalize(BatchView B, const uint64_t* __restrict__ reg, uint32_t* __restrict__ counts, unsigned long long* __restrict__ stats,
-                           unsigned long long* __restrict__ totals4) {
+static __global__ void __launch_bounds__(256) k_finish(BatchView B, const uint8_t* __restrict__ action, const uint64_t* __restrict__ leaf_bm, const uint64_t* __restrict__ init,
+                                                       uint64_t* __restrict__ reg, uint32_t* __restrict__ counts, unsigned long long* __restrict__ stats,
+                                                       unsigned long long* __restrict__ totals4) {
     __shared__ unsigned long long s_acc[8][4];
     const uint32_t warp = threadIdx.x >> 5;
     const uint32_t b = blockIdx.x * 8 + warp;
     unsigned long long rows = 0, matched = 0, blocks = 0, bm_bytes = 0;
     if (b < B.nblocks) {
         uint64_t lo = B.blk_word_off[b], hi = B.blk_word_off[b + 1];
+        const uint8_t act = action ? action[b] : ACT_ALL;
         uint32_t n = 0;
-        for (uint64_t w = lo + lane_id(); w < hi; w += 32) n += __popcll(reg[w]);
+        for (uint64_t w = lo + lane_id(); w < hi; w += 32) {
+            uint64_t x;
+            if (init) { if (act == ACT_ALL) reg[w] = x = init[w]; else x = reg[w]; }
+            else if (act == ACT_ALL) x = reg[w];
+            else reg[w] = x = act == ACT_NONE ? 0 : (reg[w] & leaf_bm[w]);
+            n += __popcll(x);
+        }
 #pragma unroll
         for (int d = 16; d; d >>= 1) n += __shfl_xor_sync(0xffffffffu, n, d);
         if (lane_id() == 0) counts[b] = n;
```

After: 22.18 billion (median of 6 runs). 1.02x the previous value.
